# bblinn2017/inverse_path_tracer

Hardware: AMD Instinct MI355X
Metric: Msamples/sec fwd + grad-Msamples/sec, 512² Cornell 64spp, 1/2/4/8 GPU (higher is better)
Workload: dtype f32; 1 GPU; C2: CornellBox-Empty-CO.obj, 512x512, 64 spp, max_bounces=4; one frame per step tiled over the ranks as interleaved rows (fwd); adjoint dL/dKd of the rank's rows + RCCL all-reduce of the gradient (grad, --full); 3 frames in flight (consecutive steps round-robin over 3 HIP streams; one stream: secondary.serial); streams=3, width=512, height=512, spp=64, max_bounces=4, triangles=18, parallelism=interleaved row tiles x1

## Files before the change

include/ipt.h:

```cpp
#ifndef IPT_H
#define IPT_H
#include <stdint.h>

#ifdef __cplusplus
extern "C" {
#endif


int loadScene(float **poss, float **oris, float **scls, char **obj_fs, char **mtl_fs, int n,
              void **scenePtr);

void freeScene(void *scenePtr);

void createImage(void *scenePtr, char *img_file);

void createGraph(void *scenePtr, char *imgFile, float *data);

void getMaterials(void *scenePtr, float *materials);
void setMaterials(void *scenePtr, float *materials);


typedef struct ipt_params {
  int32_t width, height, spp, max_bounces;
  uint64_t seed;
  int32_t row_begin, row_end;
  int32_t row_step;
} ipt_params_t;

const char *ipt_last_error(void);
void ipt_clear_error(void);
int ipt_abi_version(void);
int ipt_device_count(void);
int ipt_selftest_math(uint64_t n, uint64_t seed, uint64_t *counts);
void ipt_debug_fail_launches(int n);
void ipt_debug_adju_ring(int pool_chunks, int lds_slots);

void ipt_legacy_config(int width, int height, int spp, int max_bounces, int64_t seed);

int ipt_load_scene(int n, const float *pos, const float *ori, const float *scl, const char **obj_files,
                   const char **mtl_files, void **scenePtr);
int ipt_load_scene_host(int n, const float *pos, const float *ori, const float *scl, const char **obj_files,
                        const char **mtl_files, void **scenePtr);
int ipt_scene_num_triangles(void *scene);
int ipt_scene_num_emissives(void *scene);
int ipt_scene_export_triangles(void *scene, float *out);
int ipt_scene_get_materials(void *scene, float *kd);
int ipt_scene_set_materials(void *scene, const float *kd);
int ipt_scene_camera(void *scene, float *out16);

#define IPT_ACCEL_AUTO 0
#define IPT_ACCEL_BRUTE 1
#define IPT_ACCEL_BVH 2
int ipt_scene_set_accel(void *scene, int mode);
int ipt_scene_bvh_info(void *scene, int32_t *info8);
int ipt_scene_export_bvh(void *scene, float *nodes, float *pairs, int32_t *big_idx);
int ipt_scene_export_wide(void *scene, float *wide);
int ipt_scene_shadow_masks(void *scene, uint32_t *masks);
int ipt_closest_hit_host(void *scene, int64_t n, const float *origins, const float *dirs, const int32_t *targets,
                         float *t, int32_t *idx);
int ipt_closest_hit_dev(void *scene, int64_t n, const float *origins_dev, const float *dirs_dev,
                        const int32_t *targets_dev, float *t_dev, int32_t *idx_dev, void *stream);
int ipt_shadow_hit_host(void *scene, int64_t n, const float *origins, const float *dirs, const int32_t *targets,
                        const int32_t *sources, float *t, int32_t *idx);

int ipt_render_samples_host(void *scene, const ipt_params_t *p, float *samples);
int ipt_render_host(void *scene, const ipt_params_t *p, float *hdr, uint8_t *ldr);
int ipt_adjoint_host(void *scene, const ipt_params_t *p, const float *adj , double *grad );
int ipt_graph_host(void *scene, const ipt_params_t *p, const uint8_t *target ,
                   double *acc , float *data );
int ipt_compress(int nT, const double *acc, float *data);

int ipt_render_dev(void *scene, const ipt_params_t *p, const float *kd_dev, float *hdr_dev, uint8_t *ldr_dev,
                   void *stream);
int ipt_render_samples_dev(void *scene, const ipt_params_t *p, const float *kd_dev, float *samples_dev,
                           void *stream);
int ipt_pixel_mean_dev(const float *samples_dev, int64_t npix, int spp, float *hdr_dev, uint8_t *ldr_dev,
                       void *stream);
int ipt_render_samples_sm_dev(void *scene, const ipt_params_t *p, const float *kd_dev, float *samples_dev,
                              void *stream);
int ipt_pixel_mean_sm_dev(const float *samples_dev, int64_t npix, int spp, float *hdr_dev, uint8_t *ldr_dev,
                          void *stream);
int ipt_adjoint_dev(void *scene, const ipt_params_t *p, const float *kd_dev, const float *adj_dev, double *grad_dev,
                    void *stream);
int ipt_graph_dev(void *scene, const ipt_params_t *p, const uint8_t *target_dev, double *acc_dev, void *stream);

int ipt_render_batch_dev(void *scene, const ipt_params_t *p, int n_scenes, uint64_t seed_stride, const float *kd_dev,
                         float *hdr_dev, void *stream);
int ipt_adjoint_batch_dev(void *scene, const ipt_params_t *p, int n_scenes, uint64_t seed_stride, const float *kd_dev,
                          const float *adj_dev, double *grad_dev, void *stream);

int ipt_scene_get_material_params(void *scene, float *kd, float *ks, float *ke, float *ns);
int ipt_scene_set_material_params(void *scene, const float *kd, const float *ks, const float *ke);
int ipt_render_mat_dev(void *scene, const ipt_params_t *p, const float *kd_dev, const float *ks_dev,
                       const float *ke_dev, float *hdr_dev, uint8_t *ldr_dev, void *stream);
int ipt_adjoint_mat_dev(void *scene, const ipt_params_t *p, const float *kd_dev, const float *ks_dev,
                        const float *ke_dev, const float *adj_dev, double *grad_dev, void *stream);
int ipt_adjoint_mat_host(void *scene, const ipt_params_t *p, const float *adj , double *grad );
int ipt_adjoint_mat_unbounded_dev(void *scene, const ipt_params_t *p, const float *kd_dev, const float *ks_dev,
                                  const float *ke_dev, const float *adj_dev, double *grad_dev, void *stream);
int ipt_adjoint_mat_unbounded_host(void *scene, const ipt_params_t *p, const float *adj ,
                                   double *grad );
int ipt_render_mat_batch_dev(void *scene, const ipt_params_t *p, int n_scenes, uint64_t seed_stride,
                             const float *kd_dev, const float *ks_dev, const float *ke_dev, float *hdr_dev,
                             void *stream);
int ipt_adjoint_mat_batch_dev(void *scene, const ipt_params_t *p, int n_scenes, uint64_t seed_stride,
                              const float *kd_dev, const float *ks_dev, const float *ke_dev, const float *adj_dev,
                              double *grad_dev, void *stream);

int ipt_camera_look_at(const float eye[3], const float look[3], const float up[3], float fov_deg, float aspect,
                       float *out16);
int ipt_scene_camera_bound(void *scene, float *bound);
int ipt_views_create(void *scene, int n_views, const float *cams , void **views);
void ipt_views_free(void *views);
int ipt_views_count(void *views);
int ipt_render_views_dev(void *scene, void *views, const ipt_params_t *p, uint64_t seed_stride, const float *kd_dev,
                         const float *ks_dev, const float *ke_dev, float *hdr_dev, void *stream);
int ipt_adjoint_views_dev(void *scene, void *views, const ipt_params_t *p, uint64_t seed_stride, const float *kd_dev,
                          const float *ks_dev, const float *ke_dev, const float *adj_dev, double *grad_dev,
                          void *stream);
int ipt_render_views_batch_dev(void *scene, void *views, const ipt_params_t *p, int n_sets, uint64_t seed_stride,
                               const float *kd_dev, const float *ks_dev, const float *ke_dev,
                               float *hdr_dev , void *stream);
int ipt_adjoint_views_batch_dev(void *scene, void *views, const ipt_params_t *p, int n_sets, uint64_t seed_stride,
                                const float *kd_dev, const float *ks_dev, const float *ke_dev,
                                const float *adj_dev ,
                                double *grad_dev , void *stream);
int ipt_render_views_batch_unbounded_dev(void *scene, void *views, const ipt_params_t *p, int n_sets,
                                         uint64_t seed_stride, const float *kd_dev, const float *ks_dev,
                                         const float *ke_dev,
                                         float *hdr_dev , void *stream);
int ipt_adjoint_views_batch_unbounded_dev(void *scene, void *views, const ipt_params_t *p, int n_sets,
                                          uint64_t seed_stride, const float *kd_dev, const float *ks_dev,
                                          const float *ke_dev,
                                          const float *adj_dev ,
                                          double *grad_dev ,
                                          void *stream);
int ipt_render_views_host(void *scene, void *views, const ipt_params_t *p, uint64_t seed_stride,
                          float *hdr );
int ipt_adjoint_views_host(void *scene, void *views, const ipt_params_t *p, uint64_t seed_stride,
                           const float *adj , double *grad );
int ipt_views_rays_host(void *scene, void *views, int view, const ipt_params_t *p, int64_t n,
                        const int64_t *sample_index, float *org , float *dir );

int ipt_png_write(const char *path, int width, int height, const uint8_t *rgb);
int ipt_png_read(const char *path, int *width, int *height, uint8_t *rgb, int64_t capacity);

#ifdef __cplusplus
}
#endif
#endif
```

inverse_path_tracer_amd/_native.py:

```python
from __future__ import annotations

import ctypes as C
import os

_HERE = os.path.dirname(os.path.abspath(__file__))
LIB_PATH = os.environ.get("IPT_AMD_LIB") or os.path.join(_HERE, "lib", "libipt_amd.so")
HEADER_PATH = os.path.join(os.path.dirname(_HERE), "include", "ipt.h")
TRI_EXPORT_STRIDE = 57
ACC_WIDTH = 8
ABI_VERSION = 5
ACCEL_AUTO, ACCEL_BRUTE, ACCEL_BVH = 0, 1, 2


class NativeError(RuntimeError):
    """A C-ABI call failed; the message is ipt_last_error()."""


class Params(C.Structure):

    _fields_ = [
        ("width", C.c_int32),
        ("height", C.c_int32),
        ("spp", C.c_int32),
        ("max_bounces", C.c_int32),
        ("seed", C.c_uint64),
        ("row_begin", C.c_int32),
        ("row_end", C.c_int32),
        ("row_step", C.c_int32),
    ]

    @property
    def rows(self) -> int:
        n = self.row_end - self.row_begin
        return max(0, -(-n // max(1, self.row_step)))


def make_params(width, height, spp, max_bounces=None, seed=0, row_begin=0, row_end=None, row_step=1) -> Params:
    return Params(int(width), int(height), int(spp), -1 if max_bounces is None else int(max_bounces),
                  int(seed) & 0xFFFFFFFFFFFFFFFF, int(row_begin), int(height if row_end is None else row_end),
                  int(row_step))


_lib = None

vp = C.c_void_p
fp = C.POINTER(C.c_float)
dp = C.POINTER(C.c_double)
u8p = C.POINTER(C.c_uint8)
pp = C.POINTER(Params)

SIGNATURES = {
    "loadScene": (C.c_int, [C.POINTER(fp), C.POINTER(fp), C.POINTER(fp), C.POINTER(C.c_char_p),
                            C.POINTER(C.c_char_p), C.c_int, C.POINTER(vp)]),
    "freeScene": (None, [vp]),
    "createImage": (None, [vp, C.c_char_p]),
    "createGraph": (None, [vp, C.c_char_p, fp]),
    "getMaterials": (None, [vp, fp]),
    "setMaterials": (None, [vp, fp]),
    "ipt_last_error": (C.c_char_p, []),
    "ipt_clear_error": (None, []),
    "ipt_abi_version": (C.c_int, []),
    "ipt_device_count": (C.c_int, []),
    "ipt_selftest_math": (C.c_int, [C.c_uint64, C.c_uint64, C.POINTER(C.c_uint64)]),
    "ipt_debug_fail_launches": (None, [C.c_int]),
    "ipt_debug_adju_ring": (None, [C.c_int, C.c_int]),
    "ipt_legacy_config": (None, [C.c_int, C.c_int, C.c_int, C.c_int, C.c_int64]),
    "ipt_load_scene": (C.c_int, [C.c_int, fp, fp, fp, C.POINTER(C.c_char_p), C.POINTER(C.c_char_p), C.POINTER(vp)]),
    "ipt_load_scene_host": (C.c_int, [C.c_int, fp, fp, fp, C.POINTER(C.c_char_p), C.POINTER(C.c_char_p),
                                      C.POINTER(vp)]),
    "ipt_scene_num_triangles": (C.c_int, [vp]),
    "ipt_scene_num_emissives": (C.c_int, [vp]),
    "ipt_scene_export_triangles": (C.c_int, [vp, fp]),
    "ipt_scene_camera": (C.c_int, [vp, fp]),
    "ipt_scene_get_materials": (C.c_int, [vp, fp]),
    "ipt_scene_set_materials": (C.c_int, [vp, fp]),
    "ipt_render_samples_host": (C.c_int, [vp, pp, fp]),
    "ipt_render_host": (C.c_int, [vp, pp, fp, u8p]),
    "ipt_adjoint_host": (C.c_int, [vp, pp, fp, dp]),
    "ipt_graph_host": (C.c_int, [vp, pp, u8p, dp, fp]),
    "ipt_compress": (C.c_int, [C.c_int, dp, fp]),
    "ipt_render_dev": (C.c_int, [vp, pp, vp, vp, vp, vp]),
    "ipt_render_samples_dev": (C.c_int, [vp, pp, vp, vp, vp]),
    "ipt_pixel_mean_dev": (C.c_int, [vp, C.c_int64, C.c_int, vp, vp, vp]),
    "ipt_render_samples_sm_dev": (C.c_int, [vp, pp, vp, vp, vp]),
    "ipt_pixel_mean_sm_dev": (C.c_int, [vp, C.c_int64, C.c_int, vp, vp, vp]),
    "ipt_adjoint_dev": (C.c_int, [vp, pp, vp, vp, vp, vp]),
    "ipt_graph_dev": (C.c_int, [vp, pp, vp, vp, vp]),
    "ipt_render_batch_dev": (C.c_int, [vp, pp, C.c_int, C.c_uint64, vp, vp, vp]),
    "ipt_adjoint_batch_dev": (C.c_int, [vp, pp, C.c_int, C.c_uint64, vp, vp, vp, vp]),
    "ipt_scene_get_material_params": (C.c_int, [vp, fp, fp, fp, fp]),
    "ipt_scene_set_material_params": (C.c_int, [vp, fp, fp, fp]),
    "ipt_render_mat_dev": (C.c_int, [vp, pp, vp, vp, vp, vp, vp, vp]),
    "ipt_adjoint_mat_dev": (C.c_int, [vp, pp, vp, vp, vp, vp, vp, vp]),
    "ipt_adjoint_mat_host": (C.c_int, [vp, pp, fp, dp]),
    "ipt_adjoint_mat_unbounded_dev": (C.c_int, [vp, pp, vp, vp, vp, vp, vp, vp]),
    "ipt_adjoint_mat_unbounded_host": (C.c_int, [vp, pp, fp, dp]),
    "ipt_render_mat_batch_dev": (C.c_int, [vp, pp, C.c_int, C.c_uint64, vp, vp, vp, vp, vp]),
    "ipt_adjoint_mat_batch_dev": (C.c_int, [vp, pp, C.c_int, C.c_uint64, vp, vp, vp, vp, vp, vp]),
    "ipt_camera_look_at": (C.c_int, [fp, fp, fp, C.c_float, C.c_float, fp]),
    "ipt_scene_camera_bound": (C.c_int, [vp, fp]),
    "ipt_views_create": (C.c_int, [vp, C.c_int, fp, C.POINTER(vp)]),
    "ipt_views_free": (None, [vp]),
    "ipt_views_count": (C.c_int, [vp]),
    "ipt_render_views_dev": (C.c_int, [vp, vp, pp, C.c_uint64, vp, vp, vp, vp, vp]),
    "ipt_adjoint_views_dev": (C.c_int, [vp, vp, pp, C.c_uint64, vp, vp, vp, vp, vp, vp]),
    "ipt_render_views_batch_dev": (C.c_int, [vp, vp, pp, C.c_int, C.c_uint64, vp, vp, vp, vp, vp]),
    "ipt_adjoint_views_batch_dev": (C.c_int, [vp, vp, pp, C.c_int, C.c_uint64, vp, vp, vp, vp, vp, vp]),
    "ipt_render_views_batch_unbounded_dev": (C.c_int, [vp, vp, pp, C.c_int, C.c_uint64, vp, vp, vp, vp, vp]),
    "ipt_adjoint_views_batch_unbounded_dev": (C.c_int, [vp, vp, pp, C.c_int, C.c_uint64, vp, vp, vp, vp, vp, vp]),
    "ipt_render_views_host":(C.c_int, [vp, vp, pp, C.c_uint64, fp]),
    "ipt_adjoint_views_host": (C.c_int, [vp, vp, pp, C.c_uint64, fp, dp]),
    "ipt_views_rays_host": (C.c_int, [vp, vp, C.c_int, pp, C.c_int64, C.POINTER(C.c_int64), fp, fp]),
    "ipt_scene_set_accel": (C.c_int, [vp, C.c_int]),
    "ipt_scene_bvh_info": (C.c_int, [vp, C.POINTER(C.c_int32)]),
    "ipt_scene_export_bvh": (C.c_int, [vp, fp, fp, C.POINTER(C.c_int32)]),
    "ipt_scene_export_wide": (C.c_int, [vp, fp]),
    "ipt_closest_hit_host": (C.c_int, [vp, C.c_int64, fp, fp, C.POINTER(C.c_int32), fp, C.POINTER(C.c_int32)]),
    "ipt_closest_hit_dev": (C.c_int, [vp, C.c_int64, vp, vp, vp, vp, vp, vp]),
    "ipt_scene_shadow_masks": (C.c_int, [vp, C.POINTER(C.c_uint32)]),
    "ipt_shadow_hit_host": (C.c_int, [vp, C.c_int64, fp, fp, C.POINTER(C.c_int32), C.POINTER(C.c_int32), fp,
                                      C.POINTER(C.c_int32)]),
    "ipt_png_write": (C.c_int, [C.c_char_p, C.c_int, C.c_int, u8p]),
    "ipt_png_read": (C.c_int, [C.c_char_p, C.POINTER(C.c_int), C.POINTER(C.c_int), u8p, C.c_int64]),
}


def lib():
    global _lib
    if _lib is None:
        if not os.path.exists(LIB_PATH):
            raise NativeError(
                "native library %s is missing: build it with `make -C inverse_path_tracer_amd/csrc` "
                "(there is no CPU fallback)" % LIB_PATH)
        L = C.CDLL(LIB_PATH)
        for name, (res, args) in SIGNATURES.items():
            f = getattr(L, name)
            f.restype = res
            f.argtypes = args
        v = L.ipt_abi_version()
        if v != ABI_VERSION:
            raise NativeError("%s has ABI %d, this binding needs %d: rebuild it" % (LIB_PATH, v, ABI_VERSION))
        _lib = L
    return _lib


def last_error() -> str:
    return (lib().ipt_last_error() or b"").decode(errors="replace")


def check(rc, what="native call"):
    if rc is not None and rc < 0:
        raise NativeError("%s failed: %s" % (what, last_error()))
    return rc


def device_count() -> int:
    return lib().ipt_device_count()
```

inverse_path_tracer_amd/csrc/capi.cpp:

```cpp
#include <cmath>
#include <cstdlib>
#include <algorithm>
#include <cstring>
#include <ctime>
#include <mutex>
#include <set>
#include <string>
#include <vector>

#include "../../include/ipt.h"
#include "gpu_api.h"
#include "png_io.h"
#include "scene_io.h"
#include "bvh.h"

using ipt::GpuScene;

namespace {

thread_local std::string g_err;

void fail(const std::string &e) { g_err = e; }

struct LegacyConfig {
  int width = 500, height = 500, spp = 100, max_bounces = -1;
  int64_t seed = -1;
} g_legacy;

ipt::RenderParams to_params(const ipt_params_t *p) {
  ipt::RenderParams r;
  r.width = p->width;
  r.height = p->height;
  r.spp = p->spp;
  r.max_bounces = p->max_bounces;
  r.seed = p->seed;
  r.row_begin = p->row_begin;
  r.row_end = p->row_end;
  r.row_step = p->row_step;
  return r;
}

ipt::RenderParams legacy_params() {
  ipt::RenderParams r;
  r.width = g_legacy.width;
  r.height = g_legacy.height;
  r.spp = g_legacy.spp;
  r.max_bounces = g_legacy.max_bounces;
  r.seed = g_legacy.seed >= 0 ? (uint64_t)g_legacy.seed : (uint64_t)time(nullptr);
  r.row_begin = 0;
  r.row_end = r.height;
  return r;
}

int gpu_status(int rc) {
  if (rc) fail(ipt::gpu_last_error());
  return rc;
}

GpuScene *as_scene(void *p) {
  if (!p) fail("null scene handle");
  return static_cast<GpuScene *>(p);
}

void compress(int nT, const double *acc, float *data) {
  const size_t sz = (size_t)(nT + 1) * nT;
  float *wts = data, *pix = data + sz, *lig = data + 4 * sz;
  std::vector<float> ws((size_t)nT);
  for (int dst = 0; dst <= nT; ++dst) {
    float total = 0.f;
    for (int src = 0; src < nT; ++src) {
      const double *e = acc + ((size_t)dst * nT + src) * 8;
      const float w = logf((float)e[0] + 1);
      ws[(size_t)src] = w;
      total += w;
      const float fs = (float)e[1];
      const float den = (fs != 0.f) ? fs : 1.f;
      for (int i = 0; i < 3; ++i) {
        pix[((size_t)dst * nT + src) * 3 + i] = (float)e[2 + i] / den;
        lig[((size_t)dst * nT + src) * 3 + i] = (float)e[5 + i] / den;
      }
    }
    for (int src = 0; src < nT; ++src)
      wts[(size_t)dst * nT + src] = (total != 0.f) ? ws[(size_t)src] / total : 0.f;
  }
}

}

extern "C" {

const char *ipt_last_error(void) { return g_err.c_str(); }
void ipt_clear_error(void) { g_err.clear(); }
int ipt_abi_version(void) { return 5; }
int ipt_device_count(void) { return ipt::gpu_device_count(); }
int ipt_selftest_math(uint64_t n, uint64_t seed, uint64_t *counts) {
  if (!counts) return -1;
  return gpu_status(ipt::gpu_selftest_math(n, seed, counts));
}
void ipt_debug_fail_launches(int n) { ipt::gpu_debug_fail_launches(n); }
void ipt_debug_adju_ring(int pool_chunks, int lds_slots) { ipt::gpu_debug_adju_ring(pool_chunks, lds_slots); }

void ipt_legacy_config(int width, int height, int spp, int max_bounces, int64_t seed) {
  g_legacy.width = width;
  g_legacy.height = height;
  g_legacy.spp = spp;
  g_legacy.max_bounces = max_bounces;
  g_legacy.seed = seed;
}

static int load_scene_impl(int n, const float *pos, const float *ori, const float *scl, const char **obj_files,
                           const char **mtl_files, void **scenePtr, bool device) {
  if (scenePtr) *scenePtr = nullptr;
  if (n < 0 || !scenePtr || (n > 0 && (!pos || !ori || !scl || !obj_files || !mtl_files))) {
    fail("ipt_load_scene: bad arguments");
    return -1;
  }
  std::vector<ipt::ObjectRecord> recs((size_t)n);
  for (int i = 0; i < n; ++i) {
    for (int k = 0; k < 3; ++k) {
      recs[(size_t)i].pos[k] = pos[3 * i + k];
      recs[(size_t)i].ori[k] = ori[3 * i + k];
      recs[(size_t)i].scl[k] = scl[3 * i + k];
    }
    if (!obj_files[i] || !mtl_files[i]) {
      fail("ipt_load_scene: null file name");
      return -1;
    }
    recs[(size_t)i].obj_file = obj_files[i];
    recs[(size_t)i].mtl_file = mtl_files[i];
  }
  ipt::HostScene host;
  std::string err;
  if (!ipt::build_scene(recs, &host, &err)) {
    fail(err);
    return -1;
  }
  GpuScene *s = device ? ipt::gpu_upload(host, &err) : ipt::gpu_host_only(host);
  if (!s) {
    fail(err);
    return -1;
  }
  *scenePtr = s;
  return host.nT;
}

int ipt_load_scene(int n, const float *pos, const float *ori, const float *scl, const char **obj_files,
                   const char **mtl_files, void **scenePtr) {
  return load_scene_impl(n, pos, ori, scl, obj_files, mtl_files, scenePtr, true);
}
int ipt_load_scene_host(int n, const float *pos, const float *ori, const float *scl, const char **obj_files,
                        const char **mtl_files, void **scenePtr) {
  return load_scene_impl(n, pos, ori, scl, obj_files, mtl_files, scenePtr, false);
}

int loadScene(float **poss, float **oris, float **scls, char **obj_fs, char **mtl_fs, int n, void **scenePtr) {
  if (n < 0 || !poss || !oris || !scls) {
    if (scenePtr) *scenePtr = nullptr;
    fail("loadScene: bad arguments");
    return -1;
  }
  std::vector<float> pos((size_t)n * 3), ori((size_t)n * 3), scl((size_t)n * 3);
  for (int i = 0; i < n; ++i)
    for (int k = 0; k < 3; ++k) {
      pos[(size_t)(3 * i + k)] = poss[i][k];
      ori[(size_t)(3 * i + k)] = oris[i][k];
      scl[(size_t)(3 * i + k)] = scls[i][k];
    }
  return ipt_load_scene(n, pos.data(), ori.data(), scl.data(), const_cast<const char **>(obj_fs),
                        const_cast<const char **>(mtl_fs), scenePtr);
}

void freeScene(void *scenePtr) { ipt::gpu_free(static_cast<GpuScene *>(scenePtr)); }

int ipt_scene_num_triangles(void *scene) {
  GpuScene *s = as_scene(scene);
  return s ? ipt::gpu_host(s).nT : -1;
}
int ipt_scene_num_emissives(void *scene) {
  GpuScene *s = as_scene(scene);
  return s ? ipt::gpu_host(s).nE : -1;
}
int ipt_scene_export_triangles(void *scene, float *out) {
  GpuScene *s = as_scene(scene);
  if (!s || !out) return -1;
  ipt::export_triangles(ipt::gpu_host(s), out);
  return 0;
}
int ipt_scene_camera(void *scene, float *out16) {
  GpuScene *s = as_scene(scene);
  if (!s || !out16) return -1;
  std::memcpy(out16, ipt::gpu_host(s).cam, 16 * sizeof(float));
  return 0;
}

int ipt_scene_bvh_info(void *scene, int32_t *info8) {
  GpuScene *s = as_scene(scene);
  if (!s || !info8) return -1;
  const ipt::HostScene &h = ipt::gpu_host(s);
  info8[0] = (int32_t)h.bvh_nodes.size();
  info8[1] = (int32_t)h.bvh_pairs.size();
  info8[2] = h.bvh_depth;
  info8[3] = ipt::gpu_accel_in_use(s);
  info8[4] = (int32_t)h.bvh_big_pairs.size();
  info8[5] = (int32_t)h.bvh_wide.size();
  info8[6] = h.bvh_wdepth;
  info8[7] = (int32_t)h.bvh_wtris.size();
  if (h.bvh_nodes.empty()) fail("no BVH: " + h.bvh_status);
  return h.bvh_nodes.empty() ? 0 : 1;
}
int ipt_scene_export_bvh(void *scene, float *nodes, float *pairs, int32_t *big_idx) {
  GpuScene *s = as_scene(scene);
  if (!s) return -1;
  const ipt::HostScene &h = ipt::gpu_host(s);
  if (big_idx && !h.bvh_big_idx.empty())
    std::memcpy(big_idx, h.bvh_big_idx.data(), h.bvh_big_idx.size() * sizeof(int32_t));
  if (nodes && !h.bvh_nodes.empty()) std::memcpy(nodes, h.bvh_nodes.data(), h.bvh_nodes.size() * sizeof(ipt::BvhNode));
  if (pairs && !h.bvh_pairs.empty()) std::memcpy(pairs, h.bvh_pairs.data(), h.bvh_pairs.size() * sizeof(ipt::BvhPair));
  return 0;
}
int ipt_scene_export_wide(void *scene, float *wide) {
  GpuScene *s = as_scene(scene);
  if (!s) return -1;
  const ipt::HostScene &h = ipt::gpu_host(s);
  if (wide && !h.bvh_wide.empty()) std::memcpy(wide, h.bvh_wide.data(), h.bvh_wide.size() * sizeof(ipt::WideNode));
  return 0;
}
int ipt_scene_shadow_masks(void *scene, uint32_t *masks) {
  GpuScene *s = as_scene(scene);
  if (!s || !masks) return -1;
  const std::vector<uint32_t> m = ipt::shadow_occluder_masks(ipt::gpu_host(s));
  std::memcpy(masks, m.data(), m.size() * sizeof(uint32_t));
  return 0;
}
int ipt_scene_set_accel(void *scene, int mode) {
  GpuScene *s = as_scene(scene);
  if (!s) return -1;
  return gpu_status(ipt::gpu_set_accel(s, mode));
}
static bool probe_ids_ok(GpuScene *s, int64_t n, const int32_t *targets, const int32_t *sources, const char *who) {
  const ipt::HostScene &h = ipt::gpu_host(s);
  for (int64_t i = 0; i < n; ++i) {
    if (targets && targets[i] >= 0 &&
        std::find(h.emit_tri.begin(), h.emit_tri.end(), targets[i]) == h.emit_tri.end()) {
      fail(std::string(who) + ": target " + std::to_string(targets[i]) + " is not an emitter triangle");
      return false;
    }
    if (sources && (sources[i] < -1 || sources[i] >= h.nT)) {
      fail(std::string(who) + ": source " + std::to_string(sources[i]) + " outside [-1, nT)");
      return false;
    }
  }
  return true;
// ... 521 lines not shown
```

inverse_path_tracer_amd/csrc/gpu_api.h:

```cpp
#pragma once
#include <stdint.h>

#include <string>

#include "../../include/ipt.h"
#include "scene_io.h"

namespace ipt {

struct GpuScene;

GpuScene *gpu_upload(const HostScene &host, std::string *err);
GpuScene *gpu_host_only(const HostScene &host);
bool gpu_on_device(const GpuScene *s);
void gpu_free(GpuScene *s);
const HostScene &gpu_host(const GpuScene *s);
HostScene &gpu_host_mut(GpuScene *s);
int gpu_set_kd(GpuScene *s, const float *kd_host);

int gpu_render_samples(GpuScene *s, const RenderParams &p, const float *kd_dev, float *samples_dev,
                       void *stream);
int gpu_pixel_mean(const float *samples_dev, int64_t npix, int spp, float *hdr_dev, uint8_t *ldr_dev,
                   void *stream);
int gpu_render_samples_sm(GpuScene *s, const RenderParams &p, const float *kd_dev, float *samples_dev,
                          void *stream);
int gpu_pixel_mean_sm(const float *samples_dev, int64_t npix, int spp, float *hdr_dev, uint8_t *ldr_dev,
                      void *stream);
int gpu_render(GpuScene *s, const RenderParams &p, const float *kd_dev, float *hdr_dev, uint8_t *ldr_dev,
               void *stream);
int gpu_adjoint(GpuScene *s, const RenderParams &p, const float *kd_dev, const float *adj_dev,
                double *grad_dev, void *stream);
int gpu_graph(GpuScene *s, const RenderParams &p, const uint8_t *target_dev, double *acc_dev, void *stream);

int gpu_set_material_params(GpuScene *s, const float *kd, const float *ks, const float *ke);
int gpu_render_mat(GpuScene *s, const RenderParams &p, const float *kd_dev, const float *ks_dev, const float *ke_dev,
                   float *hdr_dev, uint8_t *ldr_dev, void *stream);
int gpu_adjoint_mat(GpuScene *s, const RenderParams &p, const float *kd_dev, const float *ks_dev, const float *ke_dev,
                    const float *adj_dev, double *grad_dev, void *stream);
int gpu_adjoint_mat_host(GpuScene *s, const RenderParams &p, const float *adj, double *grad);
int gpu_adjoint_mat_unbounded(GpuScene *s, const RenderParams &p, const float *kd_dev, const float *ks_dev,
                              const float *ke_dev, const float *adj_dev, double *grad_dev, void *stream);
int gpu_adjoint_mat_unbounded_host(GpuScene *s, const RenderParams &p, const float *adj, double *grad);
int gpu_render_mat_batch(GpuScene *s, const RenderParams &p, const float *kd_dev, const float *ks_dev,
                         const float *ke_dev, float *hdr_dev, void *stream);
int gpu_adjoint_mat_batch(GpuScene *s, const RenderParams &p, const float *kd_dev, const float *ks_dev,
                          const float *ke_dev, const float *adj_dev, double *grad_dev, void *stream);

struct GpuViews;
GpuViews *gpu_views_create(GpuScene *s, int n, const float *cams);
void gpu_views_free(GpuViews *v);
int gpu_views_count(const GpuViews *v);
float gpu_camera_bound(const GpuScene *s);
int gpu_render_views(GpuScene *s, const GpuViews *v, RenderParams p, const float *kd_dev, const float *ks_dev,
                     const float *ke_dev, float *hdr_dev, void *stream);
int gpu_adjoint_views(GpuScene *s, const GpuViews *v, RenderParams p, const float *kd_dev, const float *ks_dev,
                      const float *ke_dev, const float *adj_dev, double *grad_dev, void *stream);
int gpu_render_views_batch(GpuScene *s, const GpuViews *v, RenderParams p, int n_sets, const float *kd_dev,
                           const float *ks_dev, const float *ke_dev, float *hdr_dev, void *stream);
int gpu_adjoint_views_batch(GpuScene *s, const GpuViews *v, RenderParams p, int n_sets, const float *kd_dev,
                            const float *ks_dev, const float *ke_dev, const float *adj_dev, double *grad_dev,
                            void *stream);
int gpu_render_views_batch_unbounded(GpuScene *s, const GpuViews *v, RenderParams p, int n_sets, const float *kd_dev,
                                     const float *ks_dev, const float *ke_dev, float *hdr_dev, void *stream);
int gpu_adjoint_views_batch_unbounded(GpuScene *s, const GpuViews *v, RenderParams p, int n_sets, const float *kd_dev,
                                      const float *ks_dev, const float *ke_dev, const float *adj_dev,
                                      double *grad_dev, void *stream);
int gpu_render_views_host(GpuScene *s, const GpuViews *v, const RenderParams &p, float *hdr);
int gpu_adjoint_views_host(GpuScene *s, const GpuViews *v, const RenderParams &p, const float *adj, double *grad);
int gpu_views_rays_host(GpuScene *s, const GpuViews *v, int view, RenderParams p, int64_t n, const int64_t *index,
                        float *org, float *dir);

int gpu_render_samples_host(GpuScene *s, const RenderParams &p, float *samples);
int gpu_render_host(GpuScene *s, const RenderParams &p, float *hdr, uint8_t *ldr);
int gpu_adjoint_host(GpuScene *s, const RenderParams &p, const float *adj, double *grad);
int gpu_graph_host(GpuScene *s, const RenderParams &p, const uint8_t *target, double *acc);

int gpu_set_accel(GpuScene *s, int mode);
int gpu_accel_in_use(const GpuScene *s);
int gpu_closest_hit(GpuScene *s, int64_t n, const float *org_dev, const float *dir_dev, const int *targets_dev,
                    const int *sources_dev, float *t_dev, int *idx_dev, void *stream);
int gpu_closest_hit_host(GpuScene *s, int64_t n, const float *org, const float *dir, const int *targets,
                         const int *sources, float *t, int *idx);

int gpu_device_count();
int gpu_selftest_math(uint64_t n, uint64_t seed, uint64_t *counts);
void gpu_debug_fail_launches(int n);
void gpu_debug_adju_ring(int pool_chunks, int lds_slots);
const char *gpu_last_error();
void gpu_set_error(const std::string &e);

}
```

inverse_path_tracer_amd/csrc/ipt_device.h:

```cpp
#pragma once
#include <hip/hip_runtime.h>
#include <stdint.h>

#include "scene_layout.h"

namespace ipt {
namespace dev {

typedef __attribute__((address_space(3))) float lds_f32;
typedef __attribute__((address_space(3))) double lds_f64;
typedef __attribute__((address_space(1))) float gbl_f32;
typedef __attribute__((address_space(1))) double gbl_f64;
typedef float v4f __attribute__((ext_vector_type(4)));
typedef __attribute__((address_space(3))) v4f lds_v4;
typedef __attribute__((address_space(1))) v4f gbl_v4;

constexpr float kMinDotUp = 0x1.a36e30p-14f;
constexpr float kEpsUp = 0x1.47ae16p-7f;
constexpr float kPRR = 0.9f;
constexpr float kPiF = 3.14159265358979323846f;
constexpr float kInvPiF = (float)(1.0 / 3.14159265358979323846);
constexpr double kPi = 3.14159265358979323846;

#ifndef IPT_DIV_CONST
// ... 924 lines not shown
  const float s2 = fmaf(qz, T.e2[2], fmaf(qy, T.e2[1], fmaf(qx, T.e2[0], T.e2[3])));
  const bool ok = !(fabsf(denom) < kMinDotUp) && t >= kEpsUp && !(s0 > 0.f) && !(s1 > 0.f) && !(s2 > 0.f);
  return ok ? t : __builtin_inff();
}

template <bool SHADOW>
__device__ __forceinline__ void coop_traverse(const CoopView &C, V3 gp, V3 gd, float &gt, int &gi) {
  const int lane = (int)__lane_id();
  const int g = lane >> 3, j = lane & 7;
  const int target = gi;
  const SlabRay r = slab_ray(gp, gd);
  const int oct = (gd.x < 0.f ? 1 : 0) | (gd.y < 0.f ? 2 : 0) | (gd.z < 0.f ? 4 : 0);
  uint32_t *stk = C.stk + g * C.stride;
  int node = 0, sp = 0;
#ifdef IPT_BVH_STATS
  uint32_t st_nodes = 0, st_leaves = 0;
#endif
  for (;;) {
    if (node >= 0) {
#ifdef IPT_BVH_STATS
      ++st_nodes;
#endif
      float4 a, b;
      uint32_t rw;
      if (C.wn_lds) {
        const lds_f32 *pw = (const lds_f32 *)C.wn + 4 * (2 * (8 * node + oct) + 1) + 3;
        const lds_v4 *q = (const lds_v4 *)C.wn + 2 * (8 * node + j);
        rw = __float_as_uint(*pw);
        const v4f qa = q[0], qb = q[1];
        a = make_float4(qa.x, qa.y, qa.z, qa.w);
        b = make_float4(qb.x, qb.y, qb.z, qb.w);
      } else {
        const gbl_f32 *pw = (const gbl_f32 *)C.wn + 4 * (2 * (8 * node + oct) + 1) + 3;
        const gbl_v4 *q = (const gbl_v4 *)C.wn + 2 * (8 * node + j);
        rw = __float_as_uint(*pw);
        const v4f qa = q[0], qb = q[1];
        a = make_float4(qa.x, qa.y, qa.z, qa.w);
        b = make_float4(qb.x, qb.y, qb.z, qb.w);
      }
      const uint32_t rj = (rw >> (3 * j)) & 7u;
      const int ref = __float_as_int(b.z);
      const float tx0 = fmaf(a.x, r.ix.x, r.ox.x), tx1 = fmaf(a.w, r.ix.x, r.ox.x);
      const float ty0 = fmaf(a.y, r.iy.x, r.oy.x), ty1 = fmaf(b.x, r.iy.x, r.oy.x);
      const float tz0 = fmaf(a.z, r.iz.x, r.oz.x), tz1 = fmaf(b.y, r.iz.x, r.oz.x);
      const float en = fmaxf(fmaxf(fminf(tx0, tx1), fminf(ty0, ty1)), fmaxf(fminf(tz0, tz1), 0.f));
      const float ex = fminf(fminf(fmaxf(tx0, tx1), fmaxf(ty0, ty1)), fminf(fmaxf(tz0, tz1), gt));
      const bool h = en <= ex && ref != kWideEmpty;
      const uint32_t hm = group_or_u32(h ? 1u << rj : 0u);
      if (hm == 0) {
        node = sp > 0 ? (int)stk[--sp] : kBvhDone;
      } else {
        const uint32_t f = (uint32_t)__builtin_ctz(hm);
        const int nx = group_min_i32(h && rj == f ? ref : 0x7fffffff);
        const uint32_t others = hm & (hm - 1u);
        if ((others >> rj) & 1u) stk[sp + __popc(others >> (rj + 1))] = (uint32_t)ref;
        sp += __popc(others);
        node = nx;
      }
    } else {
#ifdef IPT_BVH_STATS
      ++st_leaves;
#endif
      const int code = ~node;
      const int first = code >> 4, cnt = (code & 15) + 1;
#ifdef IPT_BVH_STATS
      if (j == 0) atomicAdd(&g_bvh_stats[4], (unsigned long long)cnt);
#endif
      for (int base = 0; base < cnt; base += 8) {
        float tj = __builtin_inff();
        int ij = 0x7fffffff;
        if (base + j < cnt) {
          const TriIsect &T = C.wt[first + base + j];
          tj = tri_accept_t(T, gp, gd);
          ij = __float_as_int(T.pad[0]);
        }
        group_lexmin(tj, ij);
        const bool take = (tj < gt) | ((tj == gt) & (ij < gi));
        gt = take ? tj : gt;
        gi = take ? ij : gi;
      }
      node = (SHADOW && gi != target) ? kBvhDone : (sp > 0 ? (int)stk[--sp] : kBvhDone);
    }
    if (node == kBvhDone) break;
  }
#ifdef IPT_BVH_STATS
  if (j == 0) {
    atomicAdd(&g_bvh_stats[0], 1ull);
    atomicAdd(&g_bvh_stats[1], (unsigned long long)st_nodes);
    atomicAdd(&g_bvh_stats[2], (unsigned long long)st_leaves);
    if (SHADOW && gi != target) atomicAdd(&g_bvh_stats[3], 1ull);
  }
#endif
}

template <bool SHADOW>
__device__ __forceinline__ void coop_cast(const CoopView &C, bool need, V3 p, V3 d, float &bt, int &bi) {
  const int lane = (int)__lane_id();
  const int g = lane >> 3;
  uint64_t M = __ballot(need);
#ifdef IPT_BVH_STATS
  if (M && lane == (int)__builtin_ctzll(__ballot(1))) atomicAdd(&g_bvh_stats[5], 1ull);
#endif
  while (M) {
#ifdef IPT_BVH_STATS
    if (lane == (int)__builtin_ctzll(__ballot(1))) atomicAdd(&g_bvh_stats[6], 1ull);
#endif
    uint64_t Mr = M;
    int src = -1;
#pragma unroll
    for (int k = 0; k < 8; ++k) {
      if (Mr) {
        const int idx = __builtin_ctzll(Mr);
        Mr &= Mr - 1;
        src = (g == k) ? idx : src;
      }
    }
    const uint64_t taken = M & ~Mr;
    M = Mr;
    const int sa = (src < 0 ? lane : src) << 2;
    const V3 gp = mk(bperm_f(sa, p.x), bperm_f(sa, p.y), bperm_f(sa, p.z));
    const V3 gd = mk(bperm_f(sa, d.x), bperm_f(sa, d.y), bperm_f(sa, d.z));
    float gt = bperm_f(sa, bt);
    int gi = __builtin_amdgcn_ds_bpermute(sa, bi);
    if (src >= 0) {
      coop_traverse<SHADOW>(C, gp, gd, gt, gi);
    }
    const int ra = (8 * lane_rank64(taken)) << 2;
    const float rt = bperm_f(ra, gt);
    const int ri = __builtin_amdgcn_ds_bpermute(ra, gi);
    if ((taken >> lane) & 1ull) {
      bt = rt;
      bi = ri;
    }
  }
}

__device__ __forceinline__ V3 shading_normal(const TriGeom &g, V3 q) {
  if (g.flags & GEOM_AXIS_FLAT) return mk(g.vn[0][0], g.vn[0][1], g.vn[0][2]);
  const V3 v0 = mk(g.v[0][0], g.v[0][1], g.v[0][2]);
  const V3 v1 = mk(g.v[1][0], g.v[1][1], g.v[1][2]);
  const V3 v2 = mk(g.v[2][0], g.v[2][1], g.v[2][2]);
  const V3 c0 = cross3(sub(v1, q), sub(v2, q));
  const V3 c1 = cross3(sub(v2, q), sub(v0, q));
  const V3 c2 = cross3(sub(v0, q), sub(v1, q));
  const float w0 = (0.5f * sqrtf(dot3(c0, c0))) / g.area;
  const float w1 = (0.5f * sqrtf(dot3(c1, c1))) / g.area;
  const float w2 = (0.5f * sqrtf(dot3(c2, c2))) / g.area;
  const V3 n = mk(fmaf(g.vn[2][0], w2, fmaf(g.vn[1][0], w1, g.vn[0][0] * w0)),
                  fmaf(g.vn[2][1], w2, fmaf(g.vn[1][1], w1, g.vn[0][1] * w0)),
                  fmaf(g.vn[2][2], w2, fmaf(g.vn[1][2], w1, g.vn[0][2] * w0)));
  return unit(n);
}

__device__ __forceinline__ V3 camera_local(float u0, float u1, float cf, float rf, int W, int H, float rcW, float rcH) {
  const float nx = 2.f * (cf + u0), ny = 2.f * (rf + u1);
  const float x = (rcW != 0.f ? nx * rcW : div_inrange(nx, (float)W)) - 1.f;
  const float y = 1.f - (rcH != 0.f ? ny * rcH : div_inrange(ny, (float)H));
  return unit_in_range(mk(x, y, 1.f));
}
__device__ __forceinline__ V3 rotate3(const float *R0, const float *R1, const float *R2, V3 h) {
  return mk(fmaf(R0[2], h.z, fmaf(R0[1], h.y, R0[0] * h.x)), fmaf(R1[2], h.z, fmaf(R1[1], h.y, R1[0] * h.x)),
            fmaf(R2[2], h.z, fmaf(R2[1], h.y, R2[0] * h.x)));
}
__device__ __forceinline__ V3 camera_w0(const float *cam, V3 v) {
  return mk(fmaf(cam[3], 0.f, v.x), fmaf(cam[7], 0.f, v.y), fmaf(cam[11], 0.f, v.z));
}
__device__ __forceinline__ void camera_ray_f(const float *cam, const float *org, Rng &st, float rf, float cf, int W, int H,
                                             float rcW, float rcH, V3 &p, V3 &d) {
  const float u0 = uniform(st), u1 = uniform(st);
  const V3 d0 = camera_local(u0, u1, cf, rf, W, H, rcW, rcH);
  p = mk(org[0], org[1], org[2]);
  d = unit(camera_w0(cam, rotate3(cam, cam + 4, cam + 8, d0)));
}
__device__ __forceinline__ void camera_ray(const float *cam, const float *org, Rng &st, int r, int c, int W, int H,
                                           float rcW, float rcH, V3 &p, V3 &d) {
  camera_ray_f(cam, org, st, (float)r, (float)c, W, H, rcW, rcH, p, d);
}

__device__ inline float phong(float shin, V3 nrm, V3 w, V3 wi) {
  const float dn = dot3(nrm, wi);
  const V3 refl = mk(fmaf(2.f * dn, nrm.x, -wi.x), fmaf(2.f * dn, nrm.y, -wi.y), fmaf(2.f * dn, nrm.z, -wi.z));
  const float pw = pow_f(dot3(refl, w), shin);
  const float mx = pw > 0.f ? pw : 0.f;
  return (float)((((double)(shin + 2.f)) / 2.0 / kPi) * (double)mx);
}

}
}
```

inverse_path_tracer_amd/csrc/ipt_hip.hip:

```cpp
#include <hip/hip_runtime.h>

#include <algorithm>
#include <atomic>
#include <cmath>
#include <cstdio>
#include <cstdlib>
#include <cstring>
#include <mutex>
#include <string>
#include <type_traits>
#include <vector>

#include "bvh.h"
#include "gpu_api.h"
#include "ipt_device.h"

namespace ipt {

static thread_local std::string g_gpu_err;
void gpu_set_error(const std::string &e) { g_gpu_err = e; }
const char *gpu_last_error() { return g_gpu_err.c_str(); }
static std::atomic<int> g_fail_launches{0};
void gpu_debug_fail_launches(int n) { g_fail_launches.store(n > 0 ? n : 0); }
static std::atomic<int> g_adju_pool{0}, g_adju_lds{0};
void gpu_debug_adju_ring(int pool_chunks, int lds_slots) {
  g_adju_pool.store(pool_chunks > 0 ? std::min(pool_chunks, 63) : 0);
  g_adju_lds.store(lds_slots > 0 ? lds_slots : 0);
}

#define HIP_TRY(expr)                                                                        \
  do {                                                                                       \
    hipError_t e_ = (expr);                                                                  \
    if (e_ != hipSuccess) {                                                                  \
      gpu_set_error(std::string(#expr) + ": " + hipGetErrorString(e_));                      \
      return -1;                                                                             \
    }                                                                                        \
  } while (0)

enum { MODE_FWD = 0, MODE_ADJ = 1, MODE_GRAPH = 2, MODE_ADJU = 3, MODE_FWDM = 4, MODE_ADJW = 5 };
template <int MODE>
constexpr bool is_badj() {
  return MODE == MODE_ADJ || MODE == MODE_ADJW;
}
template <int MODE>
constexpr bool is_adj() {
  return is_badj<MODE>() || MODE == MODE_ADJU;
}
template <int MODE>
constexpr bool is_fwd() {
  return MODE == MODE_FWD || MODE == MODE_FWDM;
}
constexpr int kBlock = 256;
constexpr int kRecSD = 3;
constexpr int kRecFieldsDiffuse = 3;
constexpr int kRecFieldsSpec = kRecFieldsDiffuse + 2;
constexpr int kMaxAdjTris = 65535;
constexpr int kEdgeW = 8;
constexpr int kEdgeL = 5;
__host__ __device__ inline size_t graph_lds_doubles(int nT, int nE) {
  return (size_t)(nT + 1) * nT * kEdgeL + (size_t)(nT + 1) * (nE > 0 ? nE : 0) * 3;
}
__host__ __device__ inline size_t mat_lds_doubles(int grad_slots, int nE, bool spec) {
  return (size_t)grad_slots * 3 * (spec ? 2 : 1) + (size_t)(nE > 0 ? nE : 0) * 3;
}
constexpr int kCarryWords = 9;
__host__ __device__ inline size_t mat_carry_bytes(bool bvh) {
  return bvh ? 0 : (size_t)kCarryWords * kBlock * sizeof(uint32_t);
}
constexpr int kMaxAdjBounces = 62;
#ifndef IPT_CHAIN_DPP
#define IPT_CHAIN_DPP 1
#endif
#ifndef IPT_ADJU_SHIFTED_CHAIN
#define IPT_ADJU_SHIFTED_CHAIN 0
#endif
#ifndef IPT_ADJU_RING
#define IPT_ADJU_RING 63
#endif
constexpr int kPoolSlots = 16, kPoolMaxChunks = 4;
#ifndef IPT_ADJU_POOL_MB
#define IPT_ADJU_POOL_MB 64
#endif
#ifndef IPT_ADJU_LDS_CAP
#define IPT_ADJU_LDS_CAP (31 * 1024)
#endif
#ifndef IPT_ADJU_LDS_SLOTS
#define IPT_ADJU_LDS_SLOTS 8
#endif
#ifndef IPT_ADJU_LDS_SLOTS_BVH
#define IPT_ADJU_LDS_SLOTS_BVH 6
#endif
#ifndef IPT_ADJU_LDS_SLOTS_FIXED
#define IPT_ADJU_LDS_SLOTS_FIXED -1
#endif
constexpr int kAdjuRing = IPT_ADJU_RING;
#ifndef IPT_ADJU_SUB
#define IPT_ADJU_SUB 0
#endif
constexpr int kSub = IPT_ADJU_SUB;
constexpr int kMrEnt = kSub > 0 ? (kAdjuRing + kSub - 1) / kSub : 1;
#ifndef IPT_DYN_CHUNKS
#define IPT_DYN_CHUNKS 1
#endif
#ifndef IPT_DYN_CHUNKS_PER_WAVE
#define IPT_DYN_CHUNKS_PER_WAVE 32
#endif
#ifndef IPT_DYN_MIN_CHUNK
#define IPT_DYN_MIN_CHUNK 128
#endif
constexpr int kMaxTableTris = 512;
#ifndef IPT_LDS_GRAD_KB
#define IPT_LDS_GRAD_KB 12
#endif
constexpr int kLdsGradBytes = IPT_LDS_GRAD_KB * 1024;
#ifndef IPT_BVH_MIN_TRIS
#define IPT_BVH_MIN_TRIS 64
#endif
constexpr int kBvhMinTris = IPT_BVH_MIN_TRIS;
#ifndef IPT_BVH_LDS_KB
#define IPT_BVH_LDS_KB 32
#endif
constexpr int kBvhLdsNodeBytes = IPT_BVH_LDS_KB * 1024;

struct TraceArgs {
  int W, H, spp, max_bounces;
  uint64_t seed;
  uint64_t n_samples;
  int nT, nE;
  int lds_edges;
  int sample_major;
  int kd_tables;
  const float *kdpi_g;
  int small_pairs;
  uint64_t npix;
  int row0, row_step;
  int idx32;
  uint64_t m_spp, m_W, m_npix;
  int bvh_nbig;
  const float4 *bvh_wide;
  const TriIsect *bvh_wtris;
  int bvh_wide_lds, coop_stride;
  int bvh_big_lds;
  float root_box[6];
  float tree_sphere[4];
  const float4 *src_cull;
  const TriPair *bvh_big;
  const int32_t *bvh_big_idx;
  const PairBox2 *bvh_big_boxes;
  int grad_slots;
  const int *grad_map;
  const int *slot_tri;
  float cam[16];
  float cam_org[3];
  const double *emit_pmfr;
  float rc_spp;
  float rc_W, rc_H;
  int rec_cap;
  int rec_lds;
  float *grec;
  uint64_t grec_stride;
  int pool_chunks;
  float *mring;
  int nscenes, bps;
  uint64_t seed_stride, out_stride, adj_stride;
  uint32_t chunk;
  uint32_t chunk_small, chunk_big_n;
  uint32_t mat_stride;
  uint32_t *chunk_ctr;
  uint32_t grabs;
  const PairBox2 *pboxes;
  const uint32_t *pomask;
  const uint32_t *big_pomask;
  int fused;
  uint32_t group;
  uint32_t mean_off, mean_wstride;
  int nslots;
  uint8_t *ldr;
};
static_assert(alignof(TraceArgs) == 8, "TraceArgs sits right after the ten 8-B scene pointers in the kernarg segment");
static_assert(offsetof(TraceArgs, chunk_ctr) == offsetof(TraceArgs, mat_stride) + sizeof(uint32_t), "mat_stride fills the padding");

__device__ __forceinline__ uint32_t udiv32(uint32_t n, uint64_t m, uint32_t d) {
  return d == 1u ? n : (uint32_t)__umul64hi(m, (uint64_t)n);
}

__device__ __forceinline__ void item_split(const TraceArgs &a, uint64_t w, uint64_t &lp, uint64_t &sj) {
  if (a.idx32) {
    if (a.sample_major) {
      const uint32_t q = udiv32((uint32_t)w, a.m_npix, (uint32_t)a.npix);
      sj = q;
      lp = (uint32_t)w - q * (uint32_t)a.npix;
    } else {
      const uint32_t q = udiv32((uint32_t)w, a.m_spp, (uint32_t)a.spp);
      lp = q;
      sj = (uint32_t)w - q * (uint32_t)a.spp;
    }
  } else if (a.sample_major) {
    sj = w / a.npix;
    lp = w - sj * a.npix;
  } else {
    lp = w / (uint64_t)a.spp;
    sj = w - lp * (uint64_t)a.spp;
  }
}
__device__ __forceinline__ void local_rc(const TraceArgs &a, uint64_t lp, int &r, int &c) {
  uint64_t lr;
  if (a.idx32) {
    const uint32_t q = udiv32((uint32_t)lp, a.m_W, (uint32_t)a.W);
    lr = q;
    c = (int)((uint32_t)lp - q * (uint32_t)a.W);
  } else {
    lr = lp / (uint64_t)a.W;
    c = (int)(lp - lr * (uint64_t)a.W);
  }
  r = a.row0 + (int)lr * a.row_step;
}

#ifndef IPT_BF_BIG
#define IPT_BF_BIG 2
#endif
#ifndef IPT_BF_TAIL
#define IPT_BF_TAIL 4
#endif
#ifndef IPT_CTR_STRIDE
#define IPT_CTR_STRIDE 32
#endif
constexpr int kCtrStride = IPT_CTR_STRIDE;
constexpr int kViewFloats = 20;
template <bool BVH>
constexpr bool kGuided() {
  return BVH || IPT_BF_BIG > 1;
}
template <bool GUIDED>
__device__ __forceinline__ void chunk_range(const TraceArgs &a, uint64_t g, uint64_t units, uint64_t &start,
                                            uint64_t &end) {
  const uint64_t nb = a.chunk_big_n;
  uint64_t len;
  if (!GUIDED || g < nb) {
    start = g * a.chunk;
    len = a.chunk;
  } else {
    start = nb * a.chunk + (g - nb) * a.chunk_small;
    len = a.chunk_small;
  }
  end = start + len < units ? start + len : units;
}

__device__ __forceinline__ void grab_failed(uint32_t *word, uint32_t c, uint32_t grabs) {
  if (c + 1u == grabs) __hip_atomic_store(word, 0u, __ATOMIC_RELAXED, __HIP_MEMORY_SCOPE_AGENT);
}

__device__ __forceinline__ uint64_t item_pixel(const TraceArgs &a, uint64_t w) {
  uint64_t lp, sj;
  item_split(a, w, lp, sj);
  int r, c;
  local_rc(a, lp, r, c);
  if (a.idx32) return (uint32_t)r * (uint32_t)a.W + (uint32_t)c;
  return (uint64_t)r * (uint64_t)a.W + (uint64_t)c;
}

using namespace dev;
typedef __attribute__((address_space(3))) uint32_t lds_u32;

__device__ __forceinline__ void item_ray_ls(const TraceArgs &a, uint64_t seed, uint64_t lp, uint64_t sj, Rng &st, V3 &p,
                                            V3 &d, int &r, int &c) {
  local_rc(a, lp, r, c);
  uint64_t g;
  if (a.idx32) {
    const uint32_t pixel = (uint32_t)r * (uint32_t)a.W + (uint32_t)c;
    g = (uint64_t)pixel * (uint32_t)a.spp + sj;
  } else {
    g = ((uint64_t)r * (uint64_t)a.W + (uint64_t)c) * (uint64_t)a.spp + sj;
  }
  rng_init(st, seed + g);
  camera_ray(a.cam, a.cam_org, st, r, c, a.W, a.H, a.rc_W, a.rc_H, p, d);
}
__device__ __forceinline__ void item_ray(const TraceArgs &a, uint64_t seed, uint64_t w, Rng &st, V3 &p, V3 &d, int &r,
                                         int &c) {
  uint64_t lp, sj;
  item_split(a, w, lp, sj);
  item_ray_ls(a, seed, lp, sj, st, p, d, r, c);
}

#ifndef IPT_INPHASE_REFILL
#define IPT_INPHASE_REFILL 1
#endif
#ifndef IPT_INPHASE_MERGE
#define IPT_INPHASE_MERGE 1
#endif
#ifndef IPT_INPHASE_PACK
#define IPT_INPHASE_PACK 0
#endif
template <int MODE, bool BVH>
constexpr bool kInphase() {
  return IPT_INPHASE_REFILL && MODE == MODE_FWDM && !BVH;
}
constexpr int kEntryWords = 4;
static inline uint32_t fused_entry_words(uint32_t group, bool bvh) {
  return (IPT_INPHASE_REFILL && !bvh) ? kEntryWords * group : 0u;
}
__device__ __forceinline__ void pixel_entry(const TraceArgs &a, uint64_t seed, uint64_t lp, uint32_t e[kEntryWords]) {
  int r, c;
  local_rc(a, lp, r, c);
  uint64_t g0;
  if (a.idx32) {
    const uint32_t pixel = (uint32_t)r * (uint32_t)a.W + (uint32_t)c;
    g0 = (uint64_t)pixel * (uint32_t)a.spp;
  } else {
    g0 = ((uint64_t)r * (uint64_t)a.W + (uint64_t)c) * (uint64_t)a.spp;
  }
  g0 += seed;
  e[0] = (uint32_t)g0;
  e[1] = (uint32_t)(g0 >> 32);
  e[2] = __float_as_uint((float)c);
  e[3] = __float_as_uint((float)r);
}
#ifndef IPT_REFILL_ABLATE
#define IPT_REFILL_ABLATE 0
#endif

#ifndef IPT_MIN_BLOCKS_FWD
#define IPT_MIN_BLOCKS_FWD 5
#endif
#ifndef IPT_MIN_BLOCKS_ADJ
#define IPT_MIN_BLOCKS_ADJ 5
#endif
#ifndef IPT_MIN_BLOCKS_ADJU
#define IPT_MIN_BLOCKS_ADJU 5
#endif
#ifndef IPT_MIN_BLOCKS_ADJW
#define IPT_MIN_BLOCKS_ADJW 6
#endif
#ifndef IPT_ADJW_LANE_LDS
#define IPT_ADJW_LANE_LDS 1
#endif
#ifndef IPT_MIN_BLOCKS_GRAPH
#define IPT_MIN_BLOCKS_GRAPH 0
#endif
#ifndef IPT_MIN_BLOCKS_BVH
#define IPT_MIN_BLOCKS_BVH 4
#endif
#ifndef IPT_MIN_BLOCKS_BVH_ADJ
#define IPT_MIN_BLOCKS_BVH_ADJ 2
#endif
#ifndef IPT_MIN_BLOCKS_BVH_ADJU
#define IPT_MIN_BLOCKS_BVH_ADJU 4
#endif
#ifndef IPT_MIN_BLOCKS_BVH_FWD
#define IPT_MIN_BLOCKS_BVH_FWD 5
#endif
template <int MODE, bool BVH>
constexpr int min_blocks() {
  return BVH ? (MODE == MODE_ADJU ? IPT_MIN_BLOCKS_BVH_ADJU
                                  : (is_adj<MODE>() ? IPT_MIN_BLOCKS_BVH_ADJ
                                                    : (is_fwd<MODE>() ? IPT_MIN_BLOCKS_BVH_FWD : IPT_MIN_BLOCKS_BVH)))
             : (is_fwd<MODE>() ? IPT_MIN_BLOCKS_FWD
                                : (MODE == MODE_ADJU   ? IPT_MIN_BLOCKS_ADJU
                                   : MODE == MODE_ADJW ? IPT_MIN_BLOCKS_ADJW
                                                       : (is_adj<MODE>() ? IPT_MIN_BLOCKS_ADJ : IPT_MIN_BLOCKS_GRAPH)));
}
#ifndef IPT_GRAPH_LDS_KB
#define IPT_GRAPH_LDS_KB 64
#endif
#ifndef IPT_ADJ_PIXEL_MAJOR
#define IPT_ADJ_PIXEL_MAJOR 1
#endif
#ifndef IPT_GRAPH_PIXEL_MAJOR
#define IPT_GRAPH_PIXEL_MAJOR 1
#endif
#define IPT_TRACE_BOUNDS __attribute__((amdgpu_flat_work_group_size(1, kBlock), amdgpu_waves_per_eu(min_blocks<MODE, BVH>() ? min_blocks<MODE, BVH>() : 1)))
#ifdef IPT_PHASE_TIMING
constexpr int kPhaseWords = 26;
__device__ unsigned long long g_phase_cycles[kPhaseWords];
#define PHASE_LANES(i, cond)                             \
  {                                                      \
    const uint64_t b_ = __ballot(cond);                  \
    if (b_) {                                            \
      tacc[i] += (uint64_t)__popcll(b_);                 \
      tacc[(i) + 1] += 1;                                \
    }                                                    \
  }
#define SUBPHASE_BEGIN const uint64_t ts_ = __builtin_amdgcn_s_memtime();
#define SUBPHASE_END(i) tacc[i] += __builtin_amdgcn_s_memtime() - ts_;
#define PHASE(i)                                     \
  {                                                  \
    const uint64_t tn_ = __builtin_amdgcn_s_memtime(); \
    tacc[i] += tn_ - tp_;                            \
    tp_ = tn_;                                       \
  }
#else
#define PHASE(i)
#define SUBPHASE_BEGIN
#define SUBPHASE_END(i)
#define PHASE_LANES(i, cond)
#endif

__device__ __forceinline__ int cast_bf(const TriPair *__restrict__ pairs, const f2 *e3, int nT, V3 p, V3 d, float &t) {
  if (e3) return closest_hit_pairs_small(pairs, e3, nT, p, d, t);
  return closest_hit_pairs(pairs, nT, p, d, t);
}

__device__ __forceinline__ float small_table_entry(const TriPair *__restrict__ pairs, int i) {
  const int j = i / kE3Floats, k = i % kE3Floats, h = k & 1;
  return pairs[j].f[9 + 4 * (k >> 1)][h];
}

__host__ __device__ inline size_t bvh_lds_offset(size_t base) { return (base + 15) & ~(size_t)15; }
constexpr int kEmitLdsMax = 16;
__host__ __device__ inline size_t emit_lds_bytes(int nE) {
  return nE > 0 && nE <= kEmitLdsMax ? (size_t)nE * sizeof(TriIsect) : 0;
}
__host__ __device__ inline size_t big_lds_bytes(int nbig) {
  return IPT_PATH_CULL && nbig > 0 ? 12 + (size_t)nbig * (sizeof(TriPair) + 2 * sizeof(int32_t)) : 0;
}
__device__ __forceinline__ float *big_lds_copy(const TraceArgs &a, float *at, float *base, int tid, int nthr,
                                               BvhView &bv) {
  if (!(IPT_PATH_CULL && a.bvh_nbig > 0 && a.bvh_big_lds)) return at;
  float *pl = at + ((4 - (int)((at - base) & 3)) & 3);
  const float *g = reinterpret_cast<const float *>(a.bvh_big);
  for (int i = tid; i < 36 * a.bvh_nbig; i += nthr) pl[i] = g[i];
  int32_t *il = reinterpret_cast<int32_t *>(pl + 36 * a.bvh_nbig);
  for (int i = tid; i < 2 * a.bvh_nbig; i += nthr) il[i] = a.bvh_big_idx[i];
  bv.big_lds = pl;
  return at + big_lds_bytes(a.bvh_nbig) / sizeof(float);
}

template <int CTRL, int ROW, int BANK>
__device__ __forceinline__ int dpp0(int v) {
  return __builtin_amdgcn_update_dpp(0, v, CTRL, ROW, BANK, true);
}
__device__ __forceinline__ int wave_scan_add(int v) {
  int s = v + dpp0<0x111, 0xf, 0xf>(v);
  s += dpp0<0x112, 0xf, 0xf>(v);
  s += dpp0<0x113, 0xf, 0xf>(v);
  s += dpp0<0x114, 0xf, 0xe>(s);
  s += dpp0<0x118, 0xf, 0xc>(s);
  s += dpp0<0x142, 0xa, 0xf>(s);
  s += dpp0<0x143, 0xc, 0xf>(s);
  return s;
}
__device__ __forceinline__ uint32_t wave_scan_max(uint32_t v) {
  v = max(v, (uint32_t)dpp0<0x111, 0xf, 0xf>((int)v));
  v = max(v, (uint32_t)dpp0<0x112, 0xf, 0xf>((int)v));
  v = max(v, (uint32_t)dpp0<0x114, 0xf, 0xf>((int)v));
  v = max(v, (uint32_t)dpp0<0x118, 0xf, 0xf>((int)v));
  v = max(v, (uint32_t)dpp0<0x142, 0xa, 0xf>((int)v));
  v = max(v, (uint32_t)dpp0<0x143, 0xc, 0xf>((int)v));
  return v;
}

struct TraceKernArgs {
  TraceArgs a;
  const TriIsect *isect;
  const TriPair *pairs;
  const TriGeom *geom;
  const TriMat *mat;
  const float *kd;
  const int *emit_tri;
  const float *emit_cdf;
  const float *emit_pmf;
  float *out_samples;
  const float *adj;
  double *grad;
  const uint8_t *target;
  double *edges;
};
static_assert(offsetof(TraceKernArgs, isect) == sizeof(TraceArgs), "pointers follow TraceArgs");
template <typename T>
__device__ __forceinline__ T karg(size_t off) {
#if defined(__HIP_DEVICE_COMPILE__)
  typedef __attribute__((address_space(4))) const char cst_char;
  typedef __attribute__((address_space(4))) const T cst_t;
  const cst_char *k = (const cst_char *)__builtin_amdgcn_kernarg_segment_ptr();
  asm volatile("" : "+s"(k));
  return *(const cst_t *)(k + off);
#else
  (void)off;
  return T();
#endif
}
template <int MODE, bool SPEC, bool BVH>
__global__ IPT_TRACE_BOUNDS void trace_kernel(
    const TraceArgs a, const TriIsect *__restrict__ isect, const TriPair *__restrict__ pairs,
    const TriGeom *__restrict__ geom, const TriMat *__restrict__ mat, const float *__restrict__ kd,
    const int *__restrict__ emit_tri, const float *__restrict__ emit_cdf, const float *__restrict__ emit_pmf,
    float *__restrict__ out_samples, const float *__restrict__ adj, double *__restrict__ grad,
    const uint8_t *__restrict__ target, double *__restrict__ edges) {
  constexpr bool MATG = false;
  constexpr bool MATB = false;
  constexpr bool VIEWS = false;
  constexpr bool VSETS = false;
  const int *const tri_emit = nullptr;
#include "trace_body.h"
}

template <int MODE, bool SPEC, bool BVH>
__global__ IPT_TRACE_BOUNDS void trace_fwd_mat_kernel(
    const TraceArgs a, const TriIsect *__restrict__ isect, const TriPair *__restrict__ pairs,
    const TriGeom *__restrict__ geom, const TriMat *__restrict__ mat, const float *__restrict__ kd,
    const int *__restrict__ emit_tri, const float *__restrict__ emit_cdf, const float *__restrict__ emit_pmf,
    float *__restrict__ out_samples, const float *__restrict__ adj, double *__restrict__ grad,
    const uint8_t *__restrict__ target, double *__restrict__ edges) {
  static_assert(is_fwd<MODE>(), "forward instances only");
  constexpr bool MATG = false;
  constexpr bool MATB = true;
  constexpr bool VIEWS = false;
  constexpr bool VSETS = false;
  const int *const tri_emit = nullptr;
#include "trace_body.h"
}

template <bool SPEC, bool BVH>
__global__ __attribute__((amdgpu_flat_work_group_size(1, kBlock),
                          amdgpu_waves_per_eu(min_blocks<MODE_ADJ, BVH>()))) void
trace_mat_kernel(const TraceArgs a, const TriIsect *__restrict__ isect, const TriPair *__restrict__ pairs,
                 const TriGeom *__restrict__ geom, const TriMat *__restrict__ mat, const float *__restrict__ kd,
                 const int *__restrict__ emit_tri, const float *__restrict__ emit_cdf,
                 const float *__restrict__ emit_pmf, float *__restrict__ out_samples, const float *__restrict__ adj,
                 double *__restrict__ grad, const uint8_t *__restrict__ target, double *__restrict__ edges,
                 const int *__restrict__ tri_emit) {
  constexpr int MODE = MODE_ADJ;
  constexpr bool MATG = true;
  constexpr bool MATB = false;
  constexpr bool VIEWS = false;
  constexpr bool VSETS = false;
#include "trace_body.h"
}

template <bool SPEC, bool BVH>
__global__ __attribute__((amdgpu_flat_work_group_size(1, kBlock),
                          amdgpu_waves_per_eu(min_blocks<MODE_ADJU, BVH>()))) void
trace_matu_kernel(const TraceArgs a, const TriIsect *__restrict__ isect, const TriPair *__restrict__ pairs,
                  const TriGeom *__restrict__ geom, const TriMat *__restrict__ mat, const float *__restrict__ kd,
                  const int *__restrict__ emit_tri, const float *__restrict__ emit_cdf,
                  const float *__restrict__ emit_pmf, float *__restrict__ out_samples, const float *__restrict__ adj,
                  double *__restrict__ grad, const uint8_t *__restrict__ target, double *__restrict__ edges,
                  const int *__restrict__ tri_emit) {
  constexpr int MODE = MODE_ADJU;
  constexpr bool MATG = true;
  constexpr bool MATB = false;
  constexpr bool VIEWS = false;
  constexpr bool VSETS = false;
#include "trace_body.h"
}

template <int MODE, bool SPEC, bool BVH>
__global__ IPT_TRACE_BOUNDS void trace_fwd_views_kernel(
    const TraceArgs a, const TriIsect *__restrict__ isect, const TriPair *__restrict__ pairs,
    const TriGeom *__restrict__ geom, const TriMat *__restrict__ mat, const float *__restrict__ kd,
    const int *__restrict__ emit_tri, const float *__restrict__ emit_cdf, const float *__restrict__ emit_pmf,
    float *__restrict__ out_samples, const float *__restrict__ adj, double *__restrict__ grad,
    const uint8_t *__restrict__ target, double *__restrict__ edges, const float *__restrict__ views) {
  static_assert(is_fwd<MODE>(), "forward instances only");
  constexpr bool MATG = false;
  constexpr bool MATB = false;
  constexpr bool VIEWS = true;
  constexpr bool VSETS = false;
  const int *const tri_emit = nullptr;
#include "trace_body.h"
}
template <bool SPEC, bool BVH>
__global__ __attribute__((amdgpu_flat_work_group_size(1, kBlock),
                          amdgpu_waves_per_eu(min_blocks<MODE_ADJ, BVH>()))) void
trace_mat_views_kernel(const TraceArgs a, const TriIsect *__restrict__ isect, const TriPair *__restrict__ pairs,
                       const TriGeom *__restrict__ geom, const TriMat *__restrict__ mat,
                       const float *__restrict__ kd, const int *__restrict__ emit_tri,
                       const float *__restrict__ emit_cdf, const float *__restrict__ emit_pmf,
                       float *__restrict__ out_samples, const float *__restrict__ adj, double *__restrict__ grad,
                       const uint8_t *__restrict__ target, double *__restrict__ edges,
                       const int *__restrict__ tri_emit, const float *__restrict__ views) {
  constexpr int MODE = MODE_ADJ;
  constexpr bool MATG = true;
  constexpr bool MATB = false;
  constexpr bool VIEWS = true;
  constexpr bool VSETS = false;
#include "trace_body.h"
}

template <int MODE, bool SPEC, bool BVH>
__global__ IPT_TRACE_BOUNDS void trace_fwd_views_batch_kernel(
    const TraceArgs a, const TriIsect *__restrict__ isect, const TriPair *__restrict__ pairs,
    const TriGeom *__restrict__ geom, const TriMat *__restrict__ mat, const float *__restrict__ kd,
    const int *__restrict__ emit_tri, const float *__restrict__ emit_cdf, const float *__restrict__ emit_pmf,
    float *__restrict__ out_samples, const float *__restrict__ adj, double *__restrict__ grad,
    const uint8_t *__restrict__ target, double *__restrict__ edges, const float *__restrict__ views,
    const int nviews) {
  static_assert(is_fwd<MODE>(), "forward instances only");
  constexpr bool MATG = false;
  constexpr bool MATB = false;
  constexpr bool VIEWS = true;
  constexpr bool VSETS = true;
  const int *const tri_emit = nullptr;
#include "trace_body.h"
}
template <bool SPEC, bool BVH>
__global__ __attribute__((amdgpu_flat_work_group_size(1, kBlock),
                          amdgpu_waves_per_eu(min_blocks<MODE_ADJ, BVH>()))) void
trace_mat_views_batch_kernel(const TraceArgs a, const TriIsect *__restrict__ isect, const TriPair *__restrict__ pairs,
                             const TriGeom *__restrict__ geom, const TriMat *__restrict__ mat,
                             const float *__restrict__ kd, const int *__restrict__ emit_tri,
                             const float *__restrict__ emit_cdf, const float *__restrict__ emit_pmf,
                             float *__restrict__ out_samples, const float *__restrict__ adj,
                             double *__restrict__ grad, const uint8_t *__restrict__ target,
                             double *__restrict__ edges, const int *__restrict__ tri_emit,
                             const float *__restrict__ views, const int nviews) {
  constexpr int MODE = MODE_ADJ;
  constexpr bool MATG = true;
  constexpr bool MATB = false;
  constexpr bool VIEWS = true;
  constexpr bool VSETS = true;
#include "trace_body.h"
}

template <bool SPEC, bool BVH>
__global__ __attribute__((amdgpu_flat_work_group_size(1, kBlock),
                          amdgpu_waves_per_eu(min_blocks<MODE_ADJU, BVH>()))) void
trace_matu_views_batch_kernel(const TraceArgs a, const TriIsect *__restrict__ isect, const TriPair *__restrict__ pairs,
                              const TriGeom *__restrict__ geom, const TriMat *__restrict__ mat,
                              const float *__restrict__ kd, const int *__restrict__ emit_tri,
                              const float *__restrict__ emit_cdf, const float *__restrict__ emit_pmf,
                              float *__restrict__ out_samples, const float *__restrict__ adj,
                              double *__restrict__ grad, const uint8_t *__restrict__ target,
                              double *__restrict__ edges, const int *__restrict__ tri_emit,
                              const float *__restrict__ views, const int nviews) {
  constexpr int MODE = MODE_ADJU;
  constexpr bool MATG = true;
  constexpr bool MATB = false;
  constexpr bool VIEWS = true;
  constexpr bool VSETS = true;
#include "trace_body.h"
}

__global__ __launch_bounds__(kBlock) void view_rays_kernel(const float *__restrict__ views, int view, int W, int H,
                                                           int spp, float rcW, float rcH, uint64_t seed, int64_t n,
                                                           const int64_t *__restrict__ index,
                                                           float *__restrict__ org, float *__restrict__ dir) {
  const int64_t i = (int64_t)blockIdx.x * kBlock + threadIdx.x;
  if (i >= n) return;
  const uint64_t g = (uint64_t)index[i], pixel = g / (uint64_t)spp;
  const float *cam = views + (size_t)view * kViewFloats;
  Rng st;
  rng_init(st, seed + g);
  V3 p, d;
  camera_ray(cam, cam + 16, st, (int)(pixel / (uint64_t)W), (int)(pixel % (uint64_t)W), W, H, rcW, rcH, p, d);
  org[3 * i] = p.x, org[3 * i + 1] = p.y, org[3 * i + 2] = p.z;
  dir[3 * i] = d.x, dir[3 * i + 1] = d.y, dir[3 * i + 2] = d.z;
}

__global__ __launch_bounds__(kBlock) void pack_mat_kernel(const TriMat *__restrict__ src, const float *__restrict__ ks,
                                                          const float *__restrict__ ke,
                                                          const int *__restrict__ tri_emit, int nT,
                                                          TriMat *__restrict__ out) {
  const int i = blockIdx.x * kBlock + threadIdx.x;
  if (i >= nT) return;
  const size_t row = (size_t)blockIdx.y * (size_t)nT + (size_t)i;
  TriMat m = src[i];
  if (ks) {
    const bool lobe = (m.flags & MAT_HAS_KS) != 0;
    for (int c = 0; c < 3; ++c) m.ks[c] = lobe ? ks[3 * row + c] : 0.f;
  }
  if (ke) {
    const bool em = tri_emit[i] >= 0;
    for (int c = 0; c < 3; ++c) m.ke[c] = em ? ke[3 * row + c] : 0.f;
  }
  out[row] = m;
}

__global__ __launch_bounds__(kBlock) void replicate_kernel(const float *__restrict__ src, int n, size_t total,
                                                           float *__restrict__ out) {
  const size_t i = (size_t)blockIdx.x * kBlock + threadIdx.x;
  if (i < total) out[i] = src[i % (size_t)n];
}

__global__ __launch_bounds__(kBlock) void pixel_mean_sm_kernel(const float *__restrict__ samples, int64_t npix,
                                                               int spp, float *__restrict__ hdr,
                                                               uint8_t *__restrict__ ldr) {
  const int64_t px = (int64_t)blockIdx.x * kBlock + threadIdx.x;
  if (px >= npix) return;
  samples += (size_t)blockIdx.y * (size_t)npix * spp * 3;
  hdr += (size_t)blockIdx.y * (size_t)npix * 3;
  if (ldr) ldr += (size_t)blockIdx.y * (size_t)npix * 3;
  float tx = 0.f, ty = 0.f, tz = 0.f;
  const float fs = (float)spp;
  if ((spp & (spp - 1)) == 0 && spp <= (1 << 24)) {
    const float rc = 1.0f / fs;
    int i = 0;
    for (; i + 16 <= spp; i += 16) {
      float v[48];
#pragma unroll
      for (int u = 0; u < 16; ++u) {
        const float *s = samples + ((int64_t)(i + u) * npix + px) * 3;
        v[3 * u] = s[0];
        v[3 * u + 1] = s[1];
        v[3 * u + 2] = s[2];
      }
#pragma unroll
      for (int u = 0; u < 16; ++u) {
        tx += v[3 * u] * rc;
        ty += v[3 * u + 1] * rc;
        tz += v[3 * u + 2] * rc;
      }
    }
    for (; i < spp; ++i) {
      const float *s = samples + ((int64_t)i * npix + px) * 3;
      tx += s[0] * rc;
      ty += s[1] * rc;
      tz += s[2] * rc;
    }
  } else {
    for (int i = 0; i < spp; ++i) {
      const float *s = samples + ((int64_t)i * npix + px) * 3;
      tx += s[0] / fs;
      ty += s[1] / fs;
      tz += s[2] / fs;
    }
  }
  hdr[px * 3] = tx;
  hdr[px * 3 + 1] = ty;
  hdr[px * 3 + 2] = tz;
  if (ldr) {
    ldr[px * 3] = (uint8_t)(255.f * tx / (1 + tx));
    ldr[px * 3 + 1] = (uint8_t)(255.f * ty / (1 + ty));
    ldr[px * 3 + 2] = (uint8_t)(255.f * tz / (1 + tz));
  }
}

__global__ __launch_bounds__(kBlock) void pixel_mean_kernel(const float *__restrict__ samples, int64_t npix,
                                                            int spp, float *__restrict__ hdr,
                                                            uint8_t *__restrict__ ldr) {
  const int64_t px = (int64_t)blockIdx.x * kBlock + threadIdx.x;
  if (px >= npix) return;
  const float *s = samples + px * spp * 3;
  float tx = 0.f, ty = 0.f, tz = 0.f;
  const float fs = (float)spp;
  for (int i = 0; i < spp; ++i) {
    tx += s[3 * i] / fs;
    ty += s[3 * i + 1] / fs;
    tz += s[3 * i + 2] / fs;
  }
  hdr[px * 3] = tx;
  hdr[px * 3 + 1] = ty;
  hdr[px * 3 + 2] = tz;
  if (ldr) {
    ldr[px * 3] = (uint8_t)(255.f * tx / (1 + tx));
    ldr[px * 3 + 1] = (uint8_t)(255.f * ty / (1 + ty));
    ldr[px * 3 + 2] = (uint8_t)(255.f * tz / (1 + tz));
  }
}

static std::vector<double> pmf_reciprocals(const std::vector<float> &pmf) {
  std::vector<double> r(pmf.size(), 0.0);
  for (size_t e = 0; e < pmf.size(); ++e) {
    int ex = 0;
    const double m = std::frexp((double)pmf[e], &ex);
    if (pmf[e] > 0.f && m == 0.5 && ex > -1000) r[e] = std::ldexp(1.0, 1 - ex);
  }
  return r;
}

enum { KIND_TRACE = 0, KIND_MATG = 1, KIND_FWDB = 2, KIND_VFWD = 3, KIND_VMAT = 4, KIND_VBFWD = 5, KIND_VBMAT = 6 };
constexpr int kKindLast = KIND_VBMAT;
constexpr bool kind_views(int kind) { return kind == KIND_VFWD || kind == KIND_VMAT; }
constexpr bool kind_view_sets(int kind) { return kind == KIND_VBFWD || kind == KIND_VBMAT; }
constexpr bool inst_valid(int mode, int kind) {
  return kind == KIND_TRACE  ? mode >= MODE_FWD && mode <= MODE_ADJW
         : kind == KIND_MATG ? mode == MODE_ADJ || mode == MODE_ADJU
         : kind == KIND_VMAT ? mode == MODE_ADJ
         : kind == KIND_VBMAT ? mode == MODE_ADJ || mode == MODE_ADJU
                             : mode == MODE_FWD || mode == MODE_FWDM;
}
constexpr int inst_slot(int mode, bool spec, bool bvh, int kind) {
  return (kind == KIND_MATG   ? (mode == MODE_ADJU ? 36 : 24)
          : kind == KIND_FWDB ? 28 + (mode == MODE_FWDM ? 4 : 0)
          : kind == KIND_VFWD ? 40 + (mode == MODE_FWDM ? 4 : 0)
          : kind == KIND_VMAT ? 48
          : kind == KIND_VBFWD ? 52 + (mode == MODE_FWDM ? 4 : 0)
          : kind == KIND_VBMAT ? (mode == MODE_ADJU ? 64 : 60)
                              : mode * 4) +
         (spec ? 2 : 0) + (bvh ? 1 : 0);
}
constexpr int inst_slot_count() {
  bool seen[128] = {};
  int n = 0;
  for (int kind = KIND_TRACE; kind <= kKindLast; ++kind)
    for (int mode = MODE_FWD; mode <= MODE_ADJW; ++mode)
      for (int sb = 0; sb < 4 && inst_valid(mode, kind); ++sb) {
        const int slot = inst_slot(mode, (sb & 2) != 0, (sb & 1) != 0, kind);
        if (slot < 0 || slot >= 128 || seen[slot]) return -1;
        seen[slot] = true;
        n = slot + 1 > n ? slot + 1 : n;
      }
  return n;
}
constexpr int kInstSlots = inst_slot_count();
static_assert(kInstSlots > 0, "two instances share a slot of GpuScene::inst (inst_slot)");

struct InstCache {
  int grid = 0;
  size_t grid_lds = 0;
  size_t pick_base = 0;
  size_t pick_tail = 0;
  int pick_opt = -1;
};

struct GpuScene {
  HostScene host;
  int device = 0;
  bool on_device = false;
  TriIsect *isect = nullptr;
  TriPair *pairs = nullptr;
  TriGeom *geom = nullptr;
  TriMat *mat = nullptr;
  float *kd = nullptr;
  int *emit_tri = nullptr;
  float *emit_cdf = nullptr, *emit_pmf = nullptr;
  double *emit_pmfr = nullptr;
  bool has_ks = false;
  TriPair *big_pairs = nullptr;
  int32_t *big_idx = nullptr;
  PairBox2 *big_boxes = nullptr;
  float4 *wide = nullptr;
  float4 *src_cull = nullptr;
  TriIsect *wtris = nullptr;
  PairBox2 *pboxes = nullptr;
  uint32_t *pomask = nullptr;
  uint32_t *big_pomask = nullptr;
  int accel = IPT_ACCEL_AUTO;
  size_t adju_base = 0;
  int adju_nl = 0;
  size_t matu_base = 0;
  int matu_nl = 0;
  size_t vbmatu_base = 0;
  int vbmatu_nl = 0;
  int *grad_map = nullptr, *slot_tri = nullptr;
  int *tri_emit = nullptr;
  InstCache inst[kInstSlots];
  struct Counters {
    hipStream_t stream;
    int words;
    uint32_t *dev;
  };
  std::vector<Counters> counters;
  std::vector<uint32_t *> counters_retired;
  std::mutex counters_mu;
};

#ifdef IPT_PHASE_TIMING
extern "C" int ipt_debug_phase_cycles(unsigned long long *out) {
  if (hipMemcpyFromSymbol(out, HIP_SYMBOL(g_phase_cycles), kPhaseWords * sizeof(unsigned long long)) != hipSuccess)
    return -1;
  unsigned long long z[kPhaseWords] = {};
  return hipMemcpyToSymbol(HIP_SYMBOL(g_phase_cycles), z, sizeof z) == hipSuccess ? 0 : -1;
}
#endif

#ifdef IPT_BVH_STATS
extern "C" int ipt_debug_bvh_stats(unsigned long long *out) {
  if (hipMemcpyFromSymbol(out, HIP_SYMBOL(g_bvh_stats), kBvhStats * sizeof(unsigned long long)) != hipSuccess)
    return -1;
  unsigned long long z[kBvhStats] = {0};
  return hipMemcpyToSymbol(HIP_SYMBOL(g_bvh_stats), z, sizeof z) == hipSuccess ? 0 : -1;
}
#endif

const HostScene &gpu_host(const GpuScene *s) { return s->host; }
HostScene &gpu_host_mut(GpuScene *s) { return s->host; }

template <typename T>
static int upload(T **dst, const std::vector<T> &v) {
  const size_t n = std::max<size_t>(v.size(), 1) * sizeof(T);
  HIP_TRY(hipMalloc(reinterpret_cast<void **>(dst), n));
  if (!v.empty()) HIP_TRY(hipMemcpy(*dst, v.data(), v.size() * sizeof(T), hipMemcpyHostToDevice));
  return 0;
}

template <typename T>
static int upload_as_f4(float4 **dst, const std::vector<T> &v) {
  static_assert(sizeof(T) % sizeof(float4) == 0, "record is not a whole number of float4");
  HIP_TRY(hipMalloc(reinterpret_cast<void **>(dst), std::max<size_t>(v.size(), 1) * sizeof(T)));
  if (!v.empty()) HIP_TRY(hipMemcpy(*dst, v.data(), v.size() * sizeof(T), hipMemcpyHostToDevice));
  return 0;
}

static std::vector<float4> src_cull_f4(const HostScene &host) {
  std::vector<float4> v(host.bvh_src_cull.size() / 4);
  for (size_t i = 0; i < v.size(); ++i)
    v[i] = make_float4(host.bvh_src_cull[4 * i], host.bvh_src_cull[4 * i + 1], host.bvh_src_cull[4 * i + 2],
                       host.bvh_src_cull[4 * i + 3]);
  return v;
}

GpuScene *gpu_upload(const HostScene &host, std::string *err) {
  GpuScene *s = new GpuScene();
  s->host = host;
  if (hipGetDevice(&s->device) != hipSuccess) {
    *err = "no HIP device available";
    delete s;
    return nullptr;
  }
  std::vector<TriPair> pairs((host.isect.size() + 1) / 2);
  pack_pairs(host.isect.data(), (int)host.isect.size(), pairs.data());
  std::vector<TriGeom> geom(host.geom);
  geom.resize((size_t)host.nT + 1, TriGeom());
  for (int i = 0; i < 3; ++i)
    for (int j = 0; j < 3; ++j) geom[(size_t)host.nT].R[i][j] = host.cam[4 * i + j];
  if (upload(&s->isect, host.isect) || upload(&s->pairs, pairs) || upload(&s->geom, geom) || upload(&s->mat, host.mat) ||
      upload(&s->kd, host.kd) || upload(&s->emit_tri, host.emit_tri) || upload(&s->emit_cdf, host.emit_cdf) ||
      upload(&s->emit_pmf, host.emit_pmf) || upload(&s->emit_pmfr, pmf_reciprocals(host.emit_pmf)) ||
      upload(&s->big_pairs, host.bvh_big_pairs) || upload(&s->big_idx, host.bvh_big_idx) ||
      upload(&s->big_boxes, host.bvh_big_boxes) ||
      upload_as_f4(&s->wide, host.bvh_wide) || upload(&s->src_cull, src_cull_f4(host)) ||
      upload(&s->wtris, host.bvh_wtris) || upload(&s->pboxes, pair_boxes(host)) ||
      upload(&s->pomask, shadow_occluder_masks(host)) ||
      upload(&s->big_pomask, host.bvh_big_idx.empty()
                                 ? std::vector<uint32_t>()
                                 : shadow_occluder_masks(host, std::vector<int>(host.bvh_big_idx.begin(),
                                                                                host.bvh_big_idx.end())))) {
    *err = gpu_last_error();
    gpu_free(s);
    return nullptr;
  }
  for (const TriMat &m : host.mat) s->has_ks |= (m.flags & MAT_HAS_KS) != 0;
  {
    std::vector<int> te((size_t)host.nT, -1);
    for (int e = 0; e < host.nE; ++e) te[(size_t)host.emit_tri[(size_t)e]] = e;
    if (upload(&s->tri_emit, te)) {
      *err = gpu_last_error();
      gpu_free(s);
      return nullptr;
    }
  }
  {
    hipMemPool_t pool;
    if (hipDeviceGetDefaultMemPool(&pool, s->device) == hipSuccess) {
      uint64_t keep = ~0ull;
      (void)hipMemPoolSetAttribute(pool, hipMemPoolAttrReleaseThreshold, &keep);
    }
  }
  if ((size_t)host.nT * 3 * sizeof(double) > (size_t)kLdsGradBytes) {
    const int slots = kLdsGradBytes / (3 * (int)sizeof(double));
    std::vector<int> order(host.nT), map(host.nT, -1), inv(slots);
    for (int i = 0; i < host.nT; ++i) order[i] = i;
    std::stable_sort(order.begin(), order.end(),
                     [&](int x, int y) { return host.geom[(size_t)x].area > host.geom[(size_t)y].area; });
    for (int k = 0; k < slots; ++k) {
      map[(size_t)order[(size_t)k]] = k;
      inv[(size_t)k] = order[(size_t)k];
    }
    if (upload(&s->grad_map, map) || upload(&s->slot_tri, inv)) {
      *err = gpu_last_error();
      gpu_free(s);
      return nullptr;
    }
  }
  s->on_device = true;
  return s;
}

GpuScene *gpu_host_only(const HostScene &host) {
  GpuScene *s = new GpuScene();
  s->host = host;
  return s;
}
bool gpu_on_device(const GpuScene *s) { return s->on_device; }

void gpu_free(GpuScene *s) {
  if (!s) return;
  if (!s->on_device) {
    delete s;
    return;
  }
  (void)hipFree(s->isect);
  (void)hipFree(s->pairs);
  (void)hipFree(s->geom);
  (void)hipFree(s->mat);
  (void)hipFree(s->kd);
  (void)hipFree(s->emit_tri);
  (void)hipFree(s->emit_cdf);
  (void)hipFree(s->emit_pmf);
  (void)hipFree(s->emit_pmfr);
  (void)hipFree(s->big_pairs);
  (void)hipFree(s->big_idx);
  (void)hipFree(s->big_boxes);
  (void)hipFree(s->wide);
  (void)hipFree(s->src_cull);
  (void)hipFree(s->wtris);
  (void)hipFree(s->pboxes);
  (void)hipFree(s->pomask);
  (void)hipFree(s->big_pomask);
  (void)hipFree(s->grad_map);
  (void)hipFree(s->slot_tri);
  (void)hipFree(s->tri_emit);
  for (auto &c : s->counters) (void)hipFree(c.dev);
  for (uint32_t *p : s->counters_retired) (void)hipFree(p);
  delete s;
}

int gpu_set_kd(GpuScene *s, const float *kd_host) {
  std::memcpy(s->host.kd.data(), kd_host, s->host.kd.size() * sizeof(float));
  if (!s->on_device) return 0;
  HIP_TRY(hipMemcpy(s->kd, kd_host, s->host.kd.size() * sizeof(float), hipMemcpyHostToDevice));
  return 0;
}

int gpu_device_count() {
  int n = 0;
  if (hipGetDeviceCount(&n) != hipSuccess) return 0;
  return n;
}

static int check_params(const GpuScene *s, const RenderParams &p) {
  if (!s->on_device) {
    gpu_set_error("scene was loaded host-only (ipt_load_scene_host); it cannot be rendered");
    return -1;
  }
  if (p.width <= 0 || p.height <= 0 || p.spp <= 0 || p.row_begin < 0 || p.row_end > p.height ||
      p.row_begin > p.row_end || p.row_step < 1) {
    gpu_set_error("invalid render parameters (width/height/spp > 0, 0 <= row_begin <= row_end <= height, row_step >= 1)");
    return -1;
  }
  if ((uint64_t)p.width * (uint64_t)p.height * (uint64_t)p.spp >= (1ull << 40)) {
    gpu_set_error("too many samples (width*height*spp must be < 2^40)");
    return -1;
  }
  if (s->host.nT <= 0) {
    gpu_set_error("scene has no triangles");
    return -1;
  }
  if (p.nscenes < 1) {
    gpu_set_error("scene batch needs n_scenes >= 1");
    return -1;
  }
  return 0;
}

#ifndef IPT_DEBUG_GRID
#define IPT_DEBUG_GRID 0
#endif
template <int MODE, bool SPEC, bool BVH, int KIND>
constexpr auto kernel_of() {
  if constexpr (KIND == KIND_VBMAT) {
    static_assert(MODE == MODE_ADJ || MODE == MODE_ADJU, "the view sets' adjoint is the material adjoint, MODE_ADJ or MODE_ADJU");
    if constexpr (MODE == MODE_ADJU) return &trace_matu_views_batch_kernel<SPEC, BVH>;
    else return &trace_mat_views_batch_kernel<SPEC, BVH>;
  } else if constexpr (KIND == KIND_VBFWD) {
    static_assert(is_fwd<MODE>(), "the view sets' forward: forward instances only");
    return &trace_fwd_views_batch_kernel<MODE, SPEC, BVH>;
  } else if constexpr (KIND == KIND_VMAT) {
    static_assert(MODE == MODE_ADJ, "the views' adjoint is the bounded material adjoint");
    return &trace_mat_views_kernel<SPEC, BVH>;
  } else if constexpr (KIND == KIND_VFWD) {
    static_assert(is_fwd<MODE>(), "the views' forward: forward instances only");
    return &trace_fwd_views_kernel<MODE, SPEC, BVH>;
  } else if constexpr (KIND == KIND_MATG) {
    static_assert(MODE == MODE_ADJ || MODE == MODE_ADJU, "the material adjoint is MODE_ADJ or MODE_ADJU");
    if constexpr (MODE == MODE_ADJU) return &trace_matu_kernel<SPEC, BVH>;
    else return &trace_mat_kernel<SPEC, BVH>;
  } else if constexpr (KIND == KIND_FWDB) {
    static_assert(is_fwd<MODE>(), "the batch forward: forward instances only");
    return &trace_fwd_mat_kernel<MODE, SPEC, BVH>;
  } else {
    return &trace_kernel<MODE, SPEC, BVH>;
  }
}
constexpr const char *kernel_name(int mode, int kind) {
  return kind == KIND_VBFWD  ? "trace_fwd_views_batch_kernel"
         : kind == KIND_VBMAT ? (mode == MODE_ADJU ? "trace_matu_views_batch_kernel" : "trace_mat_views_batch_kernel")
         : kind == KIND_VFWD ? "trace_fwd_views_kernel"
         : kind == KIND_VMAT ? "trace_mat_views_kernel"
         : kind == KIND_MATG ? (mode == MODE_ADJU ? "trace_matu_kernel" : "trace_mat_kernel")
         : kind == KIND_FWDB ? "trace_fwd_mat_kernel"
                             : "trace_kernel";
}
template <int MODE, bool SPEC, bool BVH, int KIND>
static int resident_grid(GpuScene *s, size_t lds_bytes, int *grid) {
  InstCache &c = s->inst[inst_slot(MODE, SPEC, BVH, KIND)];
  if (c.grid == 0 || c.grid_lds != lds_bytes) {
    int per_cu = 0, cus = 0;
    HIP_TRY(hipOccupancyMaxActiveBlocksPerMultiprocessor(&per_cu, kernel_of<MODE, SPEC, BVH, KIND>(), kBlock, lds_bytes));
    HIP_TRY(hipDeviceGetAttribute(&cus, hipDeviceAttributeMultiprocessorCount, s->device));
    if (per_cu <= 0) {
      gpu_set_error("trace kernel cannot be resident (LDS request too large?)");
      return -1;
    }
    c.grid = per_cu * cus;
    c.grid_lds = lds_bytes;
    if (IPT_DEBUG_GRID)
      std::fprintf(stderr, "[ipt] %s<%d,%d,%d>: %zu B LDS/block, %d blocks/CU x %d CUs\n", kernel_name(MODE, KIND), MODE,
                   (int)SPEC, (int)BVH, lds_bytes, per_cu, cus);
  }
  *grid = c.grid;
  return 0;
}

static void camera_origin(const float *cam, float *org) {
  for (int i = 0; i < 3; ++i) {
    const float *M = cam + 4 * i;
    org[i] = std::fmaf(M[3], 1.f, std::fmaf(M[2], 0.f, std::fmaf(M[1], 0.f, M[0] * 0.f)));
  }
}

static TraceArgs make_args(const GpuScene *s, const RenderParams &p);
static TraceArgs make_args_scene(const GpuScene *s) {
  RenderParams p;
  p.width = p.height = p.spp = 1;
  p.max_bounces = 0;
  p.seed = 0;
  p.row_begin = 0;
  p.row_end = 1;
  return make_args(s, p);
}
static TraceArgs make_args(const GpuScene *s, const RenderParams &p) {
  TraceArgs a = TraceArgs();
  a.W = p.width;
  a.H = p.height;
  a.spp = p.spp;
  a.max_bounces = p.max_bounces < 0 ? -1 : p.max_bounces;
  a.seed = p.seed;
  const int rows = band_rows(p);
  a.n_samples = (uint64_t)rows * p.width * p.spp;
  a.nT = s->host.nT;
  a.nE = s->host.nE;
  a.kd_tables = s->host.nT <= kMaxTableTris ? 1 : 0;
  a.small_pairs = s->host.nT <= 2 * kSmallPairs ? 1 : 0;
  a.npix = (uint64_t)rows * p.width;
  a.row0 = p.row_begin;
  a.row_step = p.row_step > 1 ? p.row_step : 1;
  const uint64_t total = (uint64_t)p.height * p.width * p.spp;
  a.idx32 = total <= 0xffffffffull ? 1 : 0;
  a.m_spp = p.spp > 1 ? ~0ull / (uint64_t)p.spp + 1 : 0;
  a.m_W = p.width > 1 ? ~0ull / (uint64_t)p.width + 1 : 0;
  a.m_npix = a.npix > 1 ? ~0ull / a.npix + 1 : 0;
  for (int k = 0; k < 6; ++k) a.root_box[k] = s->host.bvh_root_box[k];
  for (int k = 0; k < 4; ++k) a.tree_sphere[k] = s->host.bvh_sphere[k];
  a.src_cull = s->src_cull;
  std::memcpy(a.cam, s->host.cam, sizeof a.cam);
  a.emit_pmfr = s->emit_pmfr;
  camera_origin(a.cam, a.cam_org);
  a.rec_cap = p.max_bounces >= 0 ? p.max_bounces + 1 : 0;
  a.pboxes = s->pboxes;
  a.pomask = s->host.nE > 0 ? s->pomask : nullptr;
  a.nscenes = p.nscenes > 1 ? p.nscenes : 1;
  a.bps = 1;
  a.seed_stride = p.seed_stride;
  a.out_stride = a.n_samples * 3;
  a.adj_stride = (uint64_t)p.width * p.height * 3;
  a.rc_spp = (p.spp > 0 && p.spp <= (1 << 24) && (p.spp & (p.spp - 1)) == 0) ? 1.0f / (float)p.spp : 0.f;
  a.rc_W = (p.width > 0 && (p.width & (p.width - 1)) == 0) ? 1.0f / (float)p.width : 0.f;
  a.rc_H = (p.height > 0 && (p.height & (p.height - 1)) == 0) ? 1.0f / (float)p.height : 0.f;
  return a;
}

static bool use_bvh(const GpuScene *s) {
  if (s->host.bvh_nodes.empty()) return false;
  if (s->accel == IPT_ACCEL_BVH) return true;
  if (s->accel == IPT_ACCEL_BRUTE) return false;
  return s->host.nT >= kBvhMinTris;
}

constexpr size_t kLaneWsBytes = (size_t)6 * kBlock * sizeof(uint32_t);

static size_t bvh_lds(const GpuScene *s, TraceArgs &a, size_t base, bool stage = true, bool big_copy = true,
                      bool lane_words = false) {
  const size_t nw = s->host.bvh_wide.size();
  a.bvh_wide = s->wide;
  a.bvh_wtris = s->wtris;
  a.bvh_wide_lds = (stage && nw * kWideF4 * sizeof(float4) <= (size_t)kBvhLdsNodeBytes) ? (int)nw : 0;
  a.bvh_big_lds = big_copy && IPT_PATH_CULL ? 1 : 0;
  a.big_pomask = (IPT_SHADOW_PO && s->host.nE > 0 && !s->host.bvh_big_idx.empty()) ? s->big_pomask : nullptr;
  a.coop_stride = 7 * s->host.bvh_wdepth + 8;
  a.bvh_nbig = (int)s->host.bvh_big_pairs.size();
  a.bvh_big = s->big_pairs;
  a.bvh_big_idx = s->big_idx;
  a.bvh_big_boxes = s->big_boxes;
  const size_t head = bvh_lds_offset(base) + (size_t)a.bvh_wide_lds * kWideF4 * sizeof(float4) +
                      (size_t)a.bvh_nbig * 6 * sizeof(float) + (a.bvh_big_lds ? big_lds_bytes(a.bvh_nbig) : 0) +
                      emit_lds_bytes(s->host.nE);
  return head + (size_t)(kBlock / 64) * 8 * a.coop_stride * sizeof(uint32_t) + (lane_words ? kLaneWsBytes : 0);
}

static size_t table_bytes(const TraceArgs &a) {
  return (a.kd_tables ? (size_t)6 * a.nT * sizeof(float) : 0) +
         (a.small_pairs ? (size_t)kE3Floats * ((a.nT + 1) / 2) * sizeof(float) + 12 + (size_t)a.nT * kIsectLdsFloats * sizeof(float) +
                              (IPT_PATH_CULL ? (size_t)((a.nT + 1) / 2) * sizeof(TriPair) : 0) +
                              (IPT_SHADOW_PO && a.pomask ? (size_t)a.nT * a.nE * sizeof(uint32_t) : 0)
                        : 0);
}

struct StreamScratch {
  void *p = nullptr;
  hipStream_t st = nullptr;
  int alloc(size_t bytes, hipStream_t stream) {
    st = stream;
    HIP_TRY(hipMallocAsync(&p, std::max<size_t>(bytes, 16), st));
    return 0;
  }
  ~StreamScratch() {
    if (p) (void)hipFreeAsync(p, st);
  }
};

static int stream_counters(GpuScene *s, hipStream_t st, int words, uint32_t **out, void **scratch) {
  const size_t bytes = (size_t)words * sizeof(uint32_t);
  hipStreamCaptureStatus cap = hipStreamCaptureStatusNone;
  HIP_TRY(hipStreamIsCapturing(st, &cap));
  if (cap != hipStreamCaptureStatusNone) {
    HIP_TRY(hipMallocAsync(scratch, bytes, st));
    HIP_TRY(hipMemsetAsync(*scratch, 0, bytes, st));
    *out = (uint32_t *)*scratch;
    return 0;
  }
  std::lock_guard<std::mutex> lk(s->counters_mu);
  GpuScene::Counters *c = nullptr;
  for (auto &e : s->counters)
    if (e.stream == st) c = &e;
  if (c && c->words < words) {
    s->counters_retired.push_back(c->dev);
    c->dev = nullptr;
    c->words = 0;
  }
  if (!c || c->dev == nullptr) {
    const int w = std::max(words, 16);
    uint32_t *dev = nullptr;
    HIP_TRY(hipMalloc(reinterpret_cast<void **>(&dev), (size_t)w * sizeof(uint32_t)));
    HIP_TRY(hipMemsetAsync(dev, 0, (size_t)w * sizeof(uint32_t), st));
    if (c) {
      c->dev = dev;
      c->words = w;
    } else {
      s->counters.push_back({st, w, dev});
      c = &s->counters.back();
    }
  }
  *out = c->dev;
  return 0;
}

#ifndef IPT_GUIDED_TAIL
#define IPT_GUIDED_TAIL 4
#endif

static uint32_t launch_grabs(bool guided, uint64_t units, uint64_t c, uint64_t small, uint64_t nb, uint64_t rw) {
  const uint64_t chunks = guided ? nb + (units - nb * c + small - 1) / small : (units + c - 1) / c;
  return (uint32_t)((chunks > rw ? chunks - rw : 0) + rw);
}
#ifndef IPT_DYN_SMALL_CHUNK
#define IPT_DYN_SMALL_CHUNK 64
#endif

struct LaunchIO {
  const float *kd = nullptr;
  float *out = nullptr;
  const float *adj = nullptr;
  double *grad = nullptr;
  const uint8_t *target = nullptr;
  double *edges = nullptr;
  const TriMat *mat = nullptr;
  const float *views = nullptr;
  int nviews = 0;
  hipStream_t stream = nullptr;
  size_t tail = 0;
};

template <int MODE, bool SPEC, bool BVH, int KIND>
static int launch_inst(GpuScene *s, const TraceArgs &a, size_t lds, const LaunchIO &io) {
  const hipStream_t st = io.stream;
  int grid = 0;
  if (lds > 160 * 1024) {
    gpu_set_error("LDS footprint of the launch exceeds 160 KiB");
    return -1;
  }
  if (resident_grid<MODE, SPEC, BVH, KIND>(s, lds, &grid)) return -1;
  if (a.n_samples == 0) return 0;
  TraceArgs b = a;
  if (a.nscenes > 1) {
    b.bps = std::max(1, grid / a.nscenes);
    grid = b.bps * a.nscenes;
  }
  b.chunk = 0;
  b.chunk_ctr = nullptr;
  StreamScratch cap_ctr;
  if (IPT_DYN_CHUNKS) {
    const uint64_t waves = (uint64_t)(a.nscenes > 1 ? b.bps : grid) * (kBlock / 64);
    uint64_t c = (a.n_samples / (waves * IPT_DYN_CHUNKS_PER_WAVE) + 63) / 64 * 64;
    c = std::min<uint64_t>(std::max<uint64_t>(c, IPT_DYN_MIN_CHUNK), 4096);
    uint64_t units = a.n_samples, small = std::min<uint64_t>(c, IPT_DYN_SMALL_CHUNK);
    if (a.fused) {
      c = a.chunk;
      while (c > 1 && (a.npix + c - 1) / c < waves && (c / 2) * (uint64_t)a.spp >= 64) c /= 2;
      b.group = std::min<uint32_t>(a.group, (uint32_t)c);
      small = std::min<uint64_t>(c, std::max<uint64_t>(1, 64 / (uint64_t)a.spp));
      units = a.npix;
    }
    if (!BVH) {
      small = c;
      c *= IPT_BF_BIG;
    }
    b.chunk = (uint32_t)c;
    b.chunk_small = (uint32_t)small;
    const uint64_t rw = waves;
    constexpr bool guided = kGuided<BVH>();
    const uint64_t tail = guided ? rw * (uint64_t)(BVH ? IPT_GUIDED_TAIL : IPT_BF_TAIL) * small : 0;
    const uint64_t nb = guided ? (units > tail ? (units - tail) / c : 0) : 0;
    b.chunk_big_n = (uint32_t)nb;
    b.grabs = launch_grabs(guided, units, c, small, nb, rw);
    cap_ctr.st = st;
    const int words = a.nscenes * kCtrStride;
    if (stream_counters(s, st, words, &b.chunk_ctr, &cap_ctr.p)) return -1;
  }
  StreamScratch grec, mring;
  if (MODE == MODE_ADJU) {
    const size_t fields = SPEC ? kRecFieldsSpec : kRecFieldsDiffuse;
    const size_t waves = (size_t)grid * (kBlock / 64), chunk = (size_t)kPoolSlots * fields * sizeof(float);
    b.pool_chunks = (int)std::max<size_t>(16, std::min<size_t>(63, ((size_t)IPT_ADJU_POOL_MB << 20) / (waves * chunk)));
    if (g_adju_pool.load() > 0) b.pool_chunks = g_adju_pool.load();
    b.grec_stride = (uint64_t)b.pool_chunks * kPoolSlots * fields;
    b.rec_cap = std::min(kAdjuRing, a.rec_lds + kPoolMaxChunks * kPoolSlots);
    if (grec.alloc(waves * b.grec_stride * sizeof(float), st)) return -1;
    b.grec = (float *)grec.p;
    if (kSub > 0) {
      if (mring.alloc(waves * (size_t)kMrEnt * 64 * 3 * sizeof(float), st)) return -1;
      b.mring = (float *)mring.p;
    }
  }
  if (g_fail_launches.load() > 0 && g_fail_launches.fetch_sub(1) > 0) {
    gpu_set_error("launch failed on request (ipt_debug_fail_launches)");
    return -1;
  }
  if (IPT_DEBUG_GRID)
    std::fprintf(stderr,
                 "[ipt] launch %s<%d,%d,%d> grid=%d lds=%zu bps=%d chunk=%u chunk_small=%u chunk_big_n=%u grabs=%u group=%u "
                 "rec_cap=%d rec_lds=%d pool_chunks=%d grec_stride=%llu grad_slots=%d bvh_wide_lds=%d bvh_big_lds=%d "
                 "coop_stride=%d mean_off=%u mean_wstride=%u nslots=%d mat_stride=%u kd_tables=%d small_pairs=%d "
                 "sample_major=%d\n",
                 kernel_name(MODE, KIND), MODE, (int)SPEC, (int)BVH, grid, lds, b.bps, b.chunk, b.chunk_small,
                 b.chunk_big_n, b.grabs, b.group, b.rec_cap, b.rec_lds, b.pool_chunks, (unsigned long long)b.grec_stride,
                 b.grad_slots, b.bvh_wide_lds, b.bvh_big_lds, b.coop_stride, b.mean_off, b.mean_wstride, b.nslots,
                 b.mat_stride, b.kd_tables, b.small_pairs, b.sample_major);
  auto enqueue = [&](auto... trailing) {
    hipLaunchKernelGGL((kernel_of<MODE, SPEC, BVH, KIND>()), dim3(grid), dim3(kBlock), lds, st, b, s->isect, s->pairs,
                       s->geom, io.mat ? io.mat : s->mat, io.kd ? io.kd : s->kd, s->emit_tri, s->emit_cdf, s->emit_pmf,
                       io.out, io.adj, io.grad, io.target, io.edges, trailing...);
  };
  if constexpr (KIND == KIND_VBMAT) enqueue(s->tri_emit, io.views, io.nviews);
  else if constexpr (KIND == KIND_VBFWD) enqueue(io.views, io.nviews);
  else if constexpr (KIND == KIND_VMAT) enqueue(s->tri_emit, io.views);
  else if constexpr (KIND == KIND_VFWD) enqueue(io.views);
  else if constexpr (KIND == KIND_MATG) enqueue(s->tri_emit);
  else enqueue();
  HIP_TRY(hipGetLastError());
  return 0;
}

__global__ __launch_bounds__(kBlock) void kdpi_kernel(const float *__restrict__ kd, int n, float *__restrict__ out) {
  const int i = blockIdx.x * kBlock + threadIdx.x;
  if (i < n) out[i] = kd[i] / kPiF;
}

template <int MODE, bool SPEC, int KIND>
static int launch_bvh_pick(GpuScene *s, TraceArgs &a, size_t *lds, size_t tail) {
  InstCache &c = s->inst[inst_slot(MODE, SPEC, false, KIND)];
  const bool opt[4][2] = {{true, true}, {true, false}, {false, true}, {false, false}};
  const size_t base = *lds;
  if (c.pick_opt < 0 || c.pick_base != base || c.pick_tail != tail) {
    int best = -1, best_per_cu = 0;
    for (int k = 0; k < 4; ++k) {
      TraceArgs b = a;
      const size_t l = bvh_lds_offset(bvh_lds(s, b, base, opt[k][0], opt[k][1], is_fwd<MODE>())) + tail;
      if (l > 160 * 1024) continue;
      int per_cu = 0;
      HIP_TRY(hipOccupancyMaxActiveBlocksPerMultiprocessor(&per_cu, kernel_of<MODE, SPEC, true, KIND>(), kBlock, l));
      if (per_cu > best_per_cu) {
        best = k;
        best_per_cu = per_cu;
      }
    }
    if (best < 0) {
      gpu_set_error("BVH trace kernel cannot be resident (LDS request too large?)");
      return -1;
    }
    c.pick_opt = best;
    c.pick_base = base;
    c.pick_tail = tail;
  }
  const int k = c.pick_opt;
  *lds = bvh_lds(s, a, base, opt[k][0], opt[k][1], is_fwd<MODE>());
  return 0;
}

template <int MODE, int KIND = KIND_TRACE>
static int launch(GpuScene *s, TraceArgs a, size_t lds, const LaunchIO &io) {
  const hipStream_t st = io.stream;
  const int msets = kind_views(KIND) ? 1 : kind_view_sets(KIND) ? a.nscenes / io.nviews : a.nscenes;
  a.mat_stride = (io.mat && msets > 1) ? (uint32_t)a.nT : 0u;
  if constexpr (is_fwd<MODE>() && KIND == KIND_TRACE) {
    if (a.mat_stride) return launch<MODE, KIND_FWDB>(s, a, lds, io);
  }
  StreamScratch kdpi;
  if (MODE != MODE_GRAPH && !a.kd_tables && a.n_samples > 0) {
    const int n = 3 * s->host.nT * msets;
    if (kdpi.alloc((size_t)n * sizeof(float), st)) return -1;
    hipLaunchKernelGGL(kdpi_kernel, dim3((n + kBlock - 1) / kBlock), dim3(kBlock), 0, st, io.kd ? io.kd : s->kd, n,
                       (float *)kdpi.p);
    HIP_TRY(hipGetLastError());
    a.kdpi_g = (const float *)kdpi.p;
  }
  auto run = [&](auto spec, auto bvh) {
    constexpr bool SPEC = decltype(spec)::value, BVH = decltype(bvh)::value;
    if constexpr (BVH) {
      if (launch_bvh_pick<MODE, SPEC, KIND>(s, a, &lds, io.tail)) return -1;
    }
    if (io.tail) {
      a.mean_off = (uint32_t)bvh_lds_offset(lds);
      lds = a.mean_off + io.tail;
    }
    return launch_inst<MODE, SPEC, BVH, KIND>(s, a, lds, io);
  };
  constexpr std::true_type yes;
  constexpr std::false_type no;
  if constexpr (MODE == MODE_ADJW) return run(no, no);
  else if (use_bvh(s)) return s->has_ks ? run(yes, yes) : run(no, yes);
  else return s->has_ks ? run(yes, no) : run(no, no);
}

int gpu_render_samples(GpuScene *s, const RenderParams &p, const float *kd_dev, float *samples_dev, void *stream) {
  if (check_params(s, p)) return -1;
  const TraceArgs a = make_args(s, p);
  LaunchIO io;
  io.kd = kd_dev, io.out = samples_dev, io.stream = (hipStream_t)stream;
  return launch<MODE_FWD>(s, a, table_bytes(a), io);
}

int gpu_pixel_mean(const float *samples_dev, int64_t npix, int spp, float *hdr_dev, uint8_t *ldr_dev, void *stream) {
  if (npix <= 0) return 0;
  const int blocks = (int)((npix + kBlock - 1) / kBlock);
  hipLaunchKernelGGL(pixel_mean_kernel, dim3(blocks), dim3(kBlock), 0, (hipStream_t)stream, samples_dev, npix, spp,
                     hdr_dev, ldr_dev);
  HIP_TRY(hipGetLastError());
  return 0;
}

template <int KIND = KIND_TRACE>
static int render_samples_sm(GpuScene *s, const RenderParams &p, const float *kd_dev, float *samples_dev,
                             void *stream, const TriMat *mat_dev, const float *views_dev = nullptr,
                             int nviews = 0) {
  if (check_params(s, p)) return -1;
  TraceArgs a = make_args(s, p);
  a.sample_major = 1;
  LaunchIO io;
  io.kd = kd_dev, io.out = samples_dev, io.mat = mat_dev, io.views = views_dev, io.nviews = nviews;
  io.stream = (hipStream_t)stream;
  return launch<MODE_FWD, KIND>(s, a, table_bytes(a), io);
}
int gpu_render_samples_sm(GpuScene *s, const RenderParams &p, const float *kd_dev, float *samples_dev,
                          void *stream) {
  return render_samples_sm(s, p, kd_dev, samples_dev, stream, nullptr);
}

static int pixel_mean_sm_sets(const float *samples_dev, int64_t npix, int spp, int nsets, float *hdr_dev,
                              uint8_t *ldr_dev, void *stream) {
  if (npix <= 0 || nsets <= 0) return 0;
  const int blocks = (int)((npix + kBlock - 1) / kBlock);
  hipLaunchKernelGGL(pixel_mean_sm_kernel, dim3(blocks, nsets), dim3(kBlock), 0, (hipStream_t)stream, samples_dev,
                     npix, spp, hdr_dev, ldr_dev);
  HIP_TRY(hipGetLastError());
  return 0;
}

int gpu_pixel_mean_sm(const float *samples_dev, int64_t npix, int spp, float *hdr_dev, uint8_t *ldr_dev,
                      void *stream) {
  return pixel_mean_sm_sets(samples_dev, npix, spp, 1, hdr_dev, ldr_dev, stream);
}

#ifndef IPT_FUSED_MEAN
#define IPT_FUSED_MEAN 1
#endif
#ifndef IPT_FUSED_GRAB_SAMPLES
#define IPT_FUSED_GRAB_SAMPLES 256
#endif
#ifndef IPT_FUSED_WAVE_BYTES
#define IPT_FUSED_WAVE_BYTES 6144
#endif
struct FusedShape {
  int slots, group, per_grab;
};
#ifndef IPT_FUSED_BVH
#define IPT_FUSED_BVH 0
#endif
#ifndef IPT_FUSED_BVH_WAVE_BYTES
#define IPT_FUSED_BVH_WAVE_BYTES 3072
#endif
static FusedShape fused_shape(const RenderParams &p, bool bvh) {
  const FusedShape none = {0, 0, 0};
  if (!IPT_FUSED_MEAN || !IPT_DYN_CHUNKS) return none;
  if ((uint64_t)p.width * (uint64_t)p.height * (uint64_t)p.spp > 0xffffffffull || p.spp > 256) return none;
  int bytes = IPT_FUSED_WAVE_BYTES;
  if (bvh) {
    if (!IPT_FUSED_BVH) return none;
    bytes = IPT_FUSED_BVH_WAVE_BYTES;
  }
  const int slots = std::min(16, bytes / (12 * p.spp));
  const bool long_paths = p.max_bounces < 0 || p.max_bounces > 8;
  const int cap = slots / (long_paths ? 4 : 2);
  if (cap < 1) return none;
  int g = 1;
  while (2 * g <= cap && 2 * g * p.spp <= 256) g *= 2;
  if (g * p.spp < 32) return none;
  const int per_grab = std::min(8, (IPT_FUSED_GRAB_SAMPLES + g * p.spp - 1) / (g * p.spp));
  return {slots, g, per_grab};
}

template <int KIND = KIND_TRACE>
static int render_impl(GpuScene *s, const RenderParams &p, const float *kd_dev, float *hdr_dev, uint8_t *ldr_dev,
                       void *stream, const TriMat *mat_dev, const float *views_dev = nullptr, int nviews = 0) {
  if (check_params(s, p)) return -1;
  const int64_t npix = (int64_t)band_rows(p) * p.width;
  const int sets = p.nscenes > 1 ? p.nscenes : 1;
  const FusedShape fs = fused_shape(p, use_bvh(s));
  if (fs.group > 0) {
    TraceArgs a = make_args(s, p);
    a.fused = 1;
    a.group = (uint32_t)fs.group;
    a.chunk = (uint32_t)(fs.group * fs.per_grab);
    a.nslots = fs.slots;
    a.mean_wstride = (uint32_t)(((2 * fs.slots + 3) & ~3) + fused_entry_words((uint32_t)fs.group, use_bvh(s)) +
                                3 * fs.slots * p.spp + 3) & ~3u;
    a.ldr = ldr_dev;
    a.out_stride = (uint64_t)npix * 3;
    LaunchIO io;
    io.kd = kd_dev, io.out = hdr_dev, io.mat = mat_dev, io.views = views_dev, io.nviews = nviews;
    io.stream = (hipStream_t)stream;
    io.tail = (size_t)(kBlock / 64) * a.mean_wstride * sizeof(float);
    return launch<MODE_FWDM, KIND>(s, a, table_bytes(a), io);
  }
  StreamScratch ws;
  if (ws.alloc((size_t)sets * npix * p.spp * 3 * sizeof(float), (hipStream_t)stream)) return -1;
  if (render_samples_sm<KIND>(s, p, kd_dev, (float *)ws.p, stream, mat_dev, views_dev, nviews)) return -1;
  return pixel_mean_sm_sets((const float *)ws.p, npix, p.spp, sets, hdr_dev, ldr_dev, stream);
}
int gpu_render(GpuScene *s, const RenderParams &p, const float *kd_dev, float *hdr_dev, uint8_t *ldr_dev,
               void *stream) {
  return render_impl(s, p, kd_dev, hdr_dev, ldr_dev, stream, nullptr);
}

int gpu_set_material_params(GpuScene *s, const float *kd, const float *ks, const float *ke) {
  HostScene &h = s->host;
  if (kd) std::memcpy(h.kd.data(), kd, h.kd.size() * sizeof(float));
  std::vector<char> em((size_t)h.nT, 0);
  for (int e : h.emit_tri) em[(size_t)e] = 1;
  for (int i = 0; i < h.nT; ++i) {
    TriMat &m = h.mat[(size_t)i];
    for (int c = 0; c < 3; ++c) {
      if (ks) m.ks[c] = (m.flags & MAT_HAS_KS) ? ks[3 * i + c] : 0.f;
      if (ke) m.ke[c] = em[(size_t)i] ? ke[3 * i + c] : 0.f;
    }
  }
  if (!s->on_device) return 0;
  if (kd) HIP_TRY(hipMemcpy(s->kd, h.kd.data(), h.kd.size() * sizeof(float), hipMemcpyHostToDevice));
  if (ks || ke) HIP_TRY(hipMemcpy(s->mat, h.mat.data(), h.mat.size() * sizeof(TriMat), hipMemcpyHostToDevice));
  return 0;
}

static int pack_materials(GpuScene *s, const float *ks_dev, const float *ke_dev, int sets, hipStream_t st,
                          StreamScratch &buf, const TriMat **mat) {
  *mat = nullptr;
  if (!ks_dev && !ke_dev) return 0;
  const int nT = s->host.nT;
  if (buf.alloc((size_t)sets * nT * sizeof(TriMat), st)) return -1;
  hipLaunchKernelGGL(pack_mat_kernel, dim3((nT + kBlock - 1) / kBlock, sets), dim3(kBlock), 0, st, s->mat, ks_dev,
                     ke_dev, s->tri_emit, nT, (TriMat *)buf.p);
  HIP_TRY(hipGetLastError());
  *mat = (const TriMat *)buf.p;
  return 0;
}

static int batch_kd(GpuScene *s, const float **kd_dev, int sets, hipStream_t st, StreamScratch &buf) {
  if (*kd_dev || sets <= 1) return 0;
  const int n = 3 * s->host.nT;
  const size_t total = (size_t)sets * n;
  if (buf.alloc(total * sizeof(float), st)) return -1;
  hipLaunchKernelGGL(replicate_kernel, dim3((unsigned)((total + kBlock - 1) / kBlock)), dim3(kBlock), 0, st, s->kd, n,
                     total, (float *)buf.p);
  HIP_TRY(hipGetLastError());
  *kd_dev = (const float *)buf.p;
  return 0;
}

struct LaunchMaterials {
  StreamScratch tab, kdrep;
  const TriMat *mat = nullptr;
  int fill(GpuScene *s, const float **kd_dev, const float *ks_dev, const float *ke_dev, int sets, void *stream) {
    if (batch_kd(s, kd_dev, sets, (hipStream_t)stream, kdrep)) return -1;
    return pack_materials(s, ks_dev, ke_dev, sets, (hipStream_t)stream, tab, &mat);
  }
};

static int check_sets(int n_scenes) {
  if (n_scenes > 65535) {
    gpu_set_error("material overrides: at most 65535 material sets per launch");
    return -1;
  }
  return 0;
}

static int render_mat_impl(GpuScene *s, const RenderParams &p, const float *kd_dev, const float *ks_dev,
                           const float *ke_dev, float *hdr_dev, uint8_t *ldr_dev, void *stream) {
  const int sets = p.nscenes > 1 ? p.nscenes : 1;
  LaunchMaterials m;
  if (m.fill(s, &kd_dev, ks_dev, ke_dev, sets, stream)) return -1;
  return render_impl(s, p, kd_dev, hdr_dev, ldr_dev, stream, m.mat);
}

int gpu_render_mat(GpuScene *s, const RenderParams &p, const float *kd_dev, const float *ks_dev, const float *ke_dev,
                   float *hdr_dev, uint8_t *ldr_dev, void *stream) {
  if (check_params(s, p)) return -1;
  if (p.nscenes > 1) {
    gpu_set_error("material overrides do not support the scene batch (n_scenes > 1)");
    return -1;
  }
  return render_mat_impl(s, p, kd_dev, ks_dev, ke_dev, hdr_dev, ldr_dev, stream);
}

int gpu_render_mat_batch(GpuScene *s, const RenderParams &p, const float *kd_dev, const float *ks_dev,
                         const float *ke_dev, float *hdr_dev, void *stream) {
  if (check_params(s, p) || check_sets(p.nscenes)) return -1;
  if (p.max_bounces < 0 || p.max_bounces > kMaxAdjBounces) {
    gpu_set_error("material batch: give max_bounces in 0..62 (the unbounded estimator is not supported; one material set: ipt_adjoint_mat_unbounded_dev)");
    return -1;
  }
  if (s->host.nT > kMaxAdjTris) {
    gpu_set_error("material batch supports at most 65535 triangles");
    return -1;
  }
  return render_mat_impl(s, p, kd_dev, ks_dev, ke_dev, hdr_dev, nullptr, stream);
}

static TraceArgs adjoint_args(const GpuScene *s, const RenderParams &p) {
  TraceArgs a = make_args(s, p);
  a.sample_major = IPT_ADJ_PIXEL_MAJOR ? 0 : 1;
  if (s->grad_map) {
    a.grad_slots = kLdsGradBytes / (3 * (int)sizeof(double));
    a.grad_map = s->grad_map;
    a.slot_tri = s->slot_tri;
  } else {
    a.grad_slots = s->host.nT;
  }
  return a;
}

template <int KIND>
static int ring_lds_slots(GpuScene *s, size_t base, size_t per, bool bvh, size_t *cached_base, int *cached_nl,
                          int *rec_lds) {
  int nl = bvh ? IPT_ADJU_LDS_SLOTS_BVH : IPT_ADJU_LDS_SLOTS;
  if (IPT_ADJU_LDS_SLOTS_FIXED >= 0) {
    nl = IPT_ADJU_LDS_SLOTS_FIXED;
  } else if (!bvh) {
    if (*cached_base != base) {
      auto occ = [&](size_t bytes, int *o) {
        return s->has_ks ? hipOccupancyMaxActiveBlocksPerMultiprocessor(o, kernel_of<MODE_ADJU, true, false, KIND>(), kBlock, bytes)
                         : hipOccupancyMaxActiveBlocksPerMultiprocessor(o, kernel_of<MODE_ADJU, false, false, KIND>(), kBlock, bytes);
      };
      int occ0 = 0, best = 0;
      HIP_TRY(occ(base, &occ0));
      for (int k = nl; k > 0 && best == 0; --k) {
        int o = 0;
        HIP_TRY(occ(base + k * per, &o));
        if (o >= occ0 && base + k * per <= IPT_ADJU_LDS_CAP) best = k;
      }
      *cached_base = base;
      *cached_nl = best;
    }
    nl = *cached_nl;
  }
// ... 208 lines not shown
    gpu_set_error("ipt_views_rays_host: view outside [0, n_views)");
    return -1;
  }
  const uint64_t total = (uint64_t)p.width * (uint64_t)p.height * (uint64_t)p.spp;
  for (int64_t i = 0; i < n; ++i)
    if (index[i] < 0 || (uint64_t)index[i] >= total) {
      gpu_set_error("ipt_views_rays_host: a sample index outside [0, width*height*spp)");
      return -1;
    }
  if (n <= 0) return 0;
  const TraceArgs a = make_args(s, p);
  struct Buf {
    void *p = nullptr;
    ~Buf() {
      if (p) (void)hipFree(p);
    }
  } ix, o, d;
  const size_t n3 = (size_t)n * 3 * sizeof(float);
  HIP_TRY(hipMalloc(&ix.p, (size_t)n * sizeof(int64_t)));
  HIP_TRY(hipMalloc(&o.p, n3));
  HIP_TRY(hipMalloc(&d.p, n3));
  HIP_TRY(hipMemcpy(ix.p, index, (size_t)n * sizeof(int64_t), hipMemcpyHostToDevice));
  hipLaunchKernelGGL(view_rays_kernel, dim3((unsigned)((n + kBlock - 1) / kBlock)), dim3(kBlock), 0, nullptr, v->dev,
                     view, p.width, p.height, p.spp, a.rc_W, a.rc_H, p.seed, n, (const int64_t *)ix.p, (float *)o.p,
                     (float *)d.p);
  HIP_TRY(hipGetLastError());
  HIP_TRY(hipMemcpy(org, o.p, n3, hipMemcpyDeviceToHost));
  HIP_TRY(hipMemcpy(dir, d.p, n3, hipMemcpyDeviceToHost));
  return 0;
}

static size_t matu_lds_base(const GpuScene *s, const TraceArgs &a, size_t *per) {
  *per = (size_t)(s->has_ks ? kRecFieldsSpec : kRecFieldsDiffuse) * kBlock * sizeof(float);
  return mat_lds_doubles(a.grad_slots, s->host.nE, s->has_ks) * sizeof(double) + table_bytes(a) +
         mat_carry_bytes(use_bvh(s)) + (size_t)kBlock * sizeof(uint32_t);
}

template <int KIND>
static int matu_ring(GpuScene *s, TraceArgs &a, size_t *cached_base, int *cached_nl, size_t *lds) {
  size_t per = 0;
  const size_t base = matu_lds_base(s, a, &per);
  a.rec_cap = kAdjuRing;
  if (ring_lds_slots<KIND>(s, base, per, use_bvh(s), cached_base, cached_nl, &a.rec_lds)) return -1;
  a.rec_lds = (int)std::min<size_t>((size_t)a.rec_lds, (160 * 1024 - base) / per);
  *lds = base + (size_t)a.rec_lds * per;
  return 0;
}

static int check_unbounded(const RenderParams &p) {
  if (p.max_bounces >= 0) {
    gpu_set_error("unbounded material adjoint: max_bounces must be -1 (no bounce cap); ipt_adjoint_mat_dev takes max_bounces in 0..62");
    return -1;
  }
  return 0;
}
int gpu_adjoint_mat_unbounded(GpuScene *s, const RenderParams &p, const float *kd_dev, const float *ks_dev,
                              const float *ke_dev, const float *adj_dev, double *grad_dev, void *stream) {
  if (check_unbounded(p) || check_params(s, p)) return -1;
  if (p.nscenes > 1) {
    gpu_set_error("unbounded material adjoint: the scene batch (n_scenes > 1) is not supported");
    return -1;
  }
  if (s->host.nT > kMaxAdjTris) {
    gpu_set_error("adjoint supports at most 65535 triangles");
    return -1;
  }
  TraceArgs a = adjoint_args(s, p);
  size_t per = 0, lds = 0;
  if (matu_lds_base(s, a, &per) + per > 160 * 1024) {
    gpu_set_error("unbounded material adjoint: the Kd/Ks/Ke bins and the scene's LDS tables plus one record slot per lane exceed 160 KiB");
    return -1;
  }
  if (matu_ring<KIND_MATG>(s, a, &s->matu_base, &s->matu_nl, &lds)) return -1;
  LaunchMaterials m;
  if (m.fill(s, &kd_dev, ks_dev, ke_dev, 1, stream)) return -1;
  LaunchIO io;
  io.kd = kd_dev, io.adj = adj_dev, io.grad = grad_dev, io.mat = m.mat, io.stream = (hipStream_t)stream;
  return launch<MODE_ADJU, KIND_MATG>(s, a, lds, io);
}

static int view_sets_unbounded_params(GpuScene *s, const GpuViews *v, RenderParams &p, int n_sets) {
  if (p.max_bounces >= 0) {
    gpu_set_error("unbounded views batch: max_bounces must be -1 (no bounce cap); ipt_render_views_batch_dev and ipt_adjoint_views_batch_dev take max_bounces in 0..62");
    return -1;
  }
  if (n_sets < 1) {
    gpu_set_error("unbounded views batch: n_sets must be >= 1");
    return -1;
  }
  if ((int64_t)n_sets * v->n > 65535) {
    gpu_set_error("unbounded views batch: at most 65535 (material set, view) pairs per launch (n_sets * n_views)");
    return -1;
  }
  if (s->host.nT > kMaxAdjTris) {
    gpu_set_error("unbounded views batch supports at most 65535 triangles");
    return -1;
  }
  if (v->scene != s) {
    gpu_set_error("views: the handle was created for another scene");
    return -1;
  }
  p.nscenes = n_sets * v->n;
  if (check_params(s, p)) return -1;
  size_t per = 0;
  const size_t base = matu_lds_base(s, adjoint_args(s, p), &per);
  if (base + per > 160 * 1024) {
    gpu_set_error("unbounded views batch: the Kd/Ks/Ke bins and the scene's LDS tables plus one record slot per lane exceed 160 KiB");
    return -1;
  }
  return 0;
}

int gpu_render_views_batch_unbounded(GpuScene *s, const GpuViews *v, RenderParams p, int n_sets, const float *kd_dev,
                                     const float *ks_dev, const float *ke_dev, float *hdr_dev, void *stream) {
  if (view_sets_unbounded_params(s, v, p, n_sets)) return -1;
  LaunchMaterials m;
  if (m.fill(s, &kd_dev, ks_dev, ke_dev, n_sets, stream)) return -1;
  return render_impl<KIND_VBFWD>(s, p, kd_dev, hdr_dev, nullptr, stream, m.mat, v->dev, v->n);
}

int gpu_adjoint_views_batch_unbounded(GpuScene *s, const GpuViews *v, RenderParams p, int n_sets, const float *kd_dev,
                                      const float *ks_dev, const float *ke_dev, const float *adj_dev,
                                      double *grad_dev, void *stream) {
  if (view_sets_unbounded_params(s, v, p, n_sets)) return -1;
  TraceArgs a = adjoint_args(s, p);
  size_t lds = 0;
  if (matu_ring<KIND_VBMAT>(s, a, &s->vbmatu_base, &s->vbmatu_nl, &lds)) return -1;
  LaunchMaterials m;
  if (m.fill(s, &kd_dev, ks_dev, ke_dev, n_sets, stream)) return -1;
  LaunchIO io;
  io.kd = kd_dev, io.adj = adj_dev, io.grad = grad_dev, io.mat = m.mat, io.views = v->dev, io.nviews = v->n;
  io.stream = (hipStream_t)stream;
  return launch<MODE_ADJU, KIND_VBMAT>(s, a, lds, io);
}

#ifndef IPT_ADJW_MIN_SAMPLES
#define IPT_ADJW_MIN_SAMPLES (8ull << 20)
#endif
int gpu_adjoint(GpuScene *s, const RenderParams &p, const float *kd_dev, const float *adj_dev, double *grad_dev,
                void *stream) {
  if (check_params(s, p)) return -1;
  if (p.max_bounces > kMaxAdjBounces) {
    gpu_set_error("adjoint requires max_bounces <= 62 (vertex records live in LDS); -1 = unbounded");
    return -1;
  }
  const bool unbounded = p.max_bounces < 0;
  if (s->host.nT > kMaxAdjTris) {
    gpu_set_error("adjoint supports at most 65535 triangles");
    return -1;
  }
  TraceArgs a = adjoint_args(s, p);
  const size_t fields = (size_t)(s->has_ks ? kRecFieldsSpec : kRecFieldsDiffuse);
  const size_t per = fields * kBlock * sizeof(float);
  const size_t base = (size_t)a.grad_slots * 3 * sizeof(double) + table_bytes(a) +
                      (size_t)kBlock * sizeof(uint32_t);
  if (unbounded) {
    a.rec_cap = kAdjuRing;
    if (ring_lds_slots<KIND_TRACE>(s, base, per, use_bvh(s), &s->adju_base, &s->adju_nl, &a.rec_lds)) return -1;
  }
  const size_t lds = base + (size_t)(unbounded ? a.rec_lds : a.rec_cap) * per;
  if (lds > 160 * 1024) {
    gpu_set_error(unbounded ? "unbounded adjoint: the scene's LDS tables plus one record slot per lane exceed 160 KiB"
                            : "adjoint LDS footprint exceeds 160 KiB; lower max_bounces");
    return -1;
  }
  LaunchIO io;
  io.kd = kd_dev, io.adj = adj_dev, io.grad = grad_dev, io.stream = (hipStream_t)stream;
  if (unbounded) return launch<MODE_ADJU>(s, a, lds, io);
  const size_t lane_words = IPT_ADJW_LANE_LDS ? kLaneWsBytes : 0;
  bool wide = !use_bvh(s) && !s->has_ks && 6 * (lds + lane_words) <= 160 * 1024 &&
              (uint64_t)a.n_samples * (uint64_t)std::max(1, a.nscenes) >= IPT_ADJW_MIN_SAMPLES;
  if (const char *e = std::getenv("IPT_ADJW")) wide = std::atoi(e) != 0 && !use_bvh(s) && !s->has_ks;
  if (wide) return launch<MODE_ADJW>(s, a, lds + lane_words, io);
  return launch<MODE_ADJ>(s, a, lds, io);
}

int gpu_graph(GpuScene *s, const RenderParams &p, const uint8_t *target_dev, double *acc_dev, void *stream) {
  if (check_params(s, p)) return -1;
  TraceArgs a = make_args(s, p);
  const size_t bins = graph_lds_doubles(s->host.nT, s->host.nE) * sizeof(double);
  a.lds_edges = bins <= (size_t)IPT_GRAPH_LDS_KB * 1024 ? 1 : 0;
  a.kd_tables = 0;
  a.sample_major = IPT_GRAPH_PIXEL_MAJOR ? 0 : 1;
  LaunchIO io;
  io.target = target_dev, io.edges = acc_dev, io.stream = (hipStream_t)stream;
  return launch<MODE_GRAPH>(s, a, (a.lds_edges ? bins : 0) + table_bytes(a), io);
}

__device__ __forceinline__ uint64_t mix64(uint64_t z) {
  z += 0x9e3779b97f4a7c15ull;
  z = (z ^ (z >> 30)) * 0xbf58476d1ce4e5b9ull;
  z = (z ^ (z >> 27)) * 0x94d049bb133111ebull;
  return z ^ (z >> 31);
}
__device__ __forceinline__ float rand_exp_float(uint64_t r, int emin, int emax) {
  const int e = emin + (int)((r >> 23) % (uint64_t)(emax - emin + 1));
  const uint32_t m = (uint32_t)r & 0x7fffffu;
  const uint32_t sgn = (uint32_t)(r >> 63) << 31;
  return __uint_as_float(sgn | ((uint32_t)(e + 127) << 23) | m);
}
__global__ __launch_bounds__(kBlock) void math_selftest_kernel(uint64_t n, uint64_t seed,
                                                               unsigned long long *counts) {
  unsigned long long c[8] = {0, 0, 0, 0, 0, 0, 0, 0};
  const uint64_t stride = (uint64_t)gridDim.x * kBlock;
  for (uint64_t i = (uint64_t)blockIdx.x * kBlock + threadIdx.x; i < n; i += stride) {
    const uint64_t r0 = mix64(seed ^ (i * 8 + 0)), r1 = mix64(seed ^ (i * 8 + 1)), r2 = mix64(seed ^ (i * 8 + 2));
    const uint64_t r3 = mix64(seed ^ (i * 8 + 3)), r4 = mix64(seed ^ (i * 8 + 4));
    {
      const float x = fabsf(rand_exp_float(r0, -96, 127));
      c[0] += __float_as_uint(sqrt_core(x)) != __float_as_uint(sqrtf(x));
    }
    {
      const int e = -767 + (int)((r1 >> 52) % 1768u);
      const double x = __longlong_as_double((long long)(((uint64_t)(e + 1023) << 52) | (r1 & 0xfffffffffffffull)));
      c[1] += __double_as_longlong(dsqrt_core(x)) != __double_as_longlong(sqrt(x));
    }
    {
      const float a = rand_exp_float(r2, -100, 60);
      const float b = rand_exp_float(r3, -60, 60);
      const float q = a / b;
      if (fabsf(q) >= 0x1p-120f && fabsf(q) <= 0x1p120f)
        c[2] += __float_as_uint(div_inrange(a, b)) != __float_as_uint(q);
    }
    {
      const float a = rand_exp_float(r4, -40, 20);
      const float b = (r0 & 1 ? 1.f : -1.f) * (kMinDotUp + (1.f - kMinDotUp) * (float)(r3 >> 40) * 0x1p-24f);
      c[3] += __float_as_uint(div_inrange(a, b)) != __float_as_uint(a / b);
    }
    {
      V3 v;
      float comp[3];
      for (int k = 0; k < 3; ++k) {
        const uint64_t rk = mix64(r4 ^ (uint64_t)(k + 11));
        const int kind = (int)(rk & 15);
        if (kind == 0) comp[k] = 0.f;
        else if (kind == 1) comp[k] = (rk & 16) ? -0.f : 0.f;
        else if (kind == 2) comp[k] = rand_exp_float(rk, -149 + 23, -85);
        else if (kind == 3) comp[k] = rand_exp_float(rk, 25, 35);
        else if (kind == 4) comp[k] = rand_exp_float(rk, -6, -2);
        else comp[k] = rand_exp_float(rk, -30, 3);
      }
      v = mk(comp[0], comp[1], comp[2]);
      const V3 u = unit(v), w = unit_ieee(v);
      c[5] += (__float_as_uint(u.x) != __float_as_uint(w.x)) || (__float_as_uint(u.y) != __float_as_uint(w.y)) ||
              (__float_as_uint(u.z) != __float_as_uint(w.z));
      const float n2 = dot3(v, v);
      const uint32_t m = min(min((__float_as_uint(v.x) << 1) - 1u, (__float_as_uint(v.y) << 1) - 1u),
                             (__float_as_uint(v.z) << 1) - 1u);
      const bool fast = n2 >= 0x1p-6f && n2 <= 0x1p60f && m >= ((0x25u << 24) - 1u);
      c[6] += fast;
      if (fast) {
        const float sq = sqrtf(n2);
        const V3 q = div3_core(v, sq);
        c[4] += (__float_as_uint(q.x) != __float_as_uint(v.x / sq)) || (__float_as_uint(q.y) != __float_as_uint(v.y / sq)) ||
                (__float_as_uint(q.z) != __float_as_uint(v.z / sq));
      }
    }
    {
      const int W = 1 + (int)(r0 % 65536u), cc = (int)(r1 % (uint64_t)W);
      const float u0 = (float)(uint32_t)r2 * 2.3283064e-10f + 1.1641532e-10f;
      const float a = 2.f * ((float)cc + u0);
      c[7] += __float_as_uint(div_inrange(a, (float)W)) != __float_as_uint(a / (float)W);
    }
  }
  for (int k = 0; k < 8; ++k)
    if (c[k]) atomicAdd(&counts[k], c[k]);
}

int gpu_selftest_math(uint64_t n, uint64_t seed, uint64_t *counts_host) {
  unsigned long long *d = nullptr;
  HIP_TRY(hipMalloc(reinterpret_cast<void **>(&d), 8 * sizeof(unsigned long long)));
  int rc = 0;
  if (hipMemset(d, 0, 8 * sizeof(unsigned long long)) != hipSuccess) rc = -1;
  if (!rc) {
    hipLaunchKernelGGL(math_selftest_kernel, dim3(2048), dim3(kBlock), 0, 0, n, seed, d);
    if (hipGetLastError() != hipSuccess || hipDeviceSynchronize() != hipSuccess) rc = -1;
  }
  if (!rc && hipMemcpy(counts_host, d, 8 * sizeof(unsigned long long), hipMemcpyDeviceToHost) != hipSuccess) rc = -1;
  (void)hipFree(d);
  if (rc) gpu_set_error("math self-test failed to run");
  return rc;
}

__device__ __forceinline__ uint32_t probe_allow(const uint32_t *masks, const int *emit_tri, int nE, int nT, int src,
                                                int target) {
  if (!masks || src < 0 || src >= nT) return 0xffffffffu;
  for (int e = 0; e < nE; ++e)
    if (emit_tri[e] == target) return masks[src * nE + e];
  return 0xffffffffu;
}

template <bool BVH>
__global__ __launch_bounds__(kBlock) void closest_hit_kernel(const TriIsect *__restrict__ isect,
                                                             const TriPair *__restrict__ pairs, const TraceArgs a,
                                                             int small, int64_t n, const float *__restrict__ org,
                                                             const float *__restrict__ dir,
                                                             const int *__restrict__ targets,
                                                             const int *__restrict__ sources,
                                                             const int *__restrict__ emit_tri, float *__restrict__ t_out,
                                                             int *__restrict__ i_out) {
  extern __shared__ double lds[];
  const int tid = threadIdx.x;
  const int nT = a.nT;
  const int nP = (nT + 1) >> 1;
  float *lds_e3 = reinterpret_cast<float *>(lds);
  const f2 *e3 = nullptr;
  if (small) {
    for (int i = tid; i < kE3Floats * nP; i += kBlock) lds_e3[i] = small_table_entry(pairs, i);
    e3 = reinterpret_cast<const f2 *>(lds_e3);
  }
  float *lds_is = lds_e3 + kE3Floats * nP;
  lds_is += (4 - (int)((lds_is - lds_e3) & 3)) & 3;
  float *lds_pr = lds_is + kIsectLdsFloats * nT;
  if (!BVH && small) {
    const float *g = reinterpret_cast<const float *>(isect);
    for (int i = tid; i < kIsectLdsFloats * nT; i += kBlock) lds_is[i] = g[i];
    if (IPT_PATH_CULL) {
      const float *gp = reinterpret_cast<const float *>(pairs);
      for (int i = tid; i < 36 * nP; i += kBlock) lds_pr[i] = gp[i];
    }
  }
  BvhView bv;
  bv.isect = isect;
  bv.big = nullptr;
  bv.big_idx = nullptr;
// ... 245 lines not shown
```

inverse_path_tracer_amd/csrc/scene_layout.h:

```cpp
#pragma once
#include <stdint.h>

namespace ipt {

struct TriIsect {
  float c[3];
  float n[3];
  float e0[4];
  float e1[4];
  float e2[4];
  float pad[2];
};
static_assert(sizeof(TriIsect) == 80, "TriIsect layout");

struct TriPair {
  float f[18][2];
};
static_assert(sizeof(TriPair) == 144, "TriPair layout");
inline void pack_pairs(const TriIsect *t, int nT, TriPair *out) {
  for (int j = 0; 2 * j < nT; ++j) {
    for (int h = 0; h < 2; ++h) {
      const int i = 2 * j + h;
      float src[18] = {0.f};
      if (i < nT) {
        const TriIsect &T = t[i];
        const float v[18] = {T.c[0], T.c[1], T.c[2], T.n[0], T.n[1], T.n[2], T.e0[0], T.e0[1], T.e0[2],
                             T.e0[3], T.e1[0], T.e1[1], T.e1[2], T.e1[3], T.e2[0], T.e2[1], T.e2[2], T.e2[3]};
        for (int k = 0; k < 18; ++k) src[k] = v[k];
      }
      for (int k = 0; k < 18; ++k) out[j].f[k][h] = src[k];
    }
  }
}

struct TriGeom {
  float v[3][3];
  float vn[3][3];
  float area;
  float R[3][3];
  uint32_t flags;
  float pad[3];
};
static_assert(sizeof(TriGeom) == 128, "TriGeom layout");

enum : uint32_t { GEOM_AXIS_FLAT = 1u };

enum : uint32_t { MAT_HAS_KS = 1u, MAT_SPECULAR = 2u };

struct TriMat {
  float ks[3];
  float shininess;
  float ke[3];
  uint32_t flags;
};
static_assert(sizeof(TriMat) == 32, "TriMat layout");

struct BvhNode {
  float q[4][4];
};
static_assert(sizeof(BvhNode) == 64, "BvhNode layout");
constexpr int kBvhLeafPairBits = 4;
constexpr int kBvhMaxDepth = 32;
struct BvhPair {
  float f[18][2];
  int32_t idx[2];
  int32_t pad[2];
};
static_assert(sizeof(BvhPair) == 160, "BvhPair layout");

struct WideNode {
  float s[8][8];
};
static_assert(sizeof(WideNode) == 256, "WideNode layout");
constexpr int32_t kWideEmpty = (int32_t)0x80000000;

struct PairBox2 {
  float f[6][2];
};
static_assert(sizeof(PairBox2) == 48, "PairBox2 layout");

struct DevScene {
  int nT, nE;
  const TriIsect *isect;
  const TriGeom *geom;
  const TriMat *mat;
  const float *kd;
  const int *emit_tri;
  const float *emit_cdf;
  const float *emit_pmf;
  float cam[16];
};

struct RenderParams;
inline int band_rows(const RenderParams &p);
struct RenderParams {
  int width, height, spp;
  int max_bounces;
  uint64_t seed;
  int row_begin, row_end;
  int row_step = 1;
  int nscenes = 1;
  uint64_t seed_stride = 0;
};
inline int band_rows(const RenderParams &p) {
  const int n = p.row_end - p.row_begin;
  return n <= 0 ? 0 : (p.row_step <= 1 ? n : (n + p.row_step - 1) / p.row_step);
}

}
```

inverse_path_tracer_amd/csrc/trace_body.h:

```cpp
  extern __shared__ double lds[];
  const int tid = threadIdx.x;
  const int set = a.nscenes > 1 ? (int)(blockIdx.x % (uint32_t)a.nscenes) : 0;
  const uint32_t sblock = a.nscenes > 1 ? blockIdx.x / (uint32_t)a.nscenes : blockIdx.x;
  const uint32_t sgrid = a.nscenes > 1 ? (uint32_t)a.bps : gridDim.x;
  const uint64_t seed = a.seed + (uint64_t)set * a.seed_stride;
  int mset = 0, view = set;
  if (VSETS) {
    const int nviews = karg<int>(sizeof(TraceKernArgs) + (MATG ? sizeof(void *) : 0) + sizeof(const float *));
    mset = set / nviews;
    view = set - mset * nviews;
  }
  if (a.nscenes > 1) {
    if (!VIEWS) kd += (size_t)set * 3 * a.nT;
    else if (VSETS) kd += (size_t)mset * 3 * a.nT;
    if (!VIEWS && (MATG || MATB)) mat += (size_t)set * a.mat_stride;
    else if (VSETS) mat += (size_t)mset * a.mat_stride;
    if (is_fwd<MODE>()) out_samples += (size_t)set * a.out_stride;
  }
  const float *kdpi_g = a.kdpi_g ? a.kdpi_g + (VIEWS ? (VSETS ? (size_t)mset * 3 * a.nT : (size_t)0) : (size_t)set * 3 * a.nT) : nullptr;
  constexpr int nthr = kBlock;
  const int nT = a.nT, nE = a.nE;
  const int vmax = a.rec_cap;
  double *lds_acc = lds;
  int n_acc = 0;
  if (is_adj<MODE>()) {
    n_acc = a.grad_slots * 3;
    if (MATG) n_acc = (int)mat_lds_doubles(a.grad_slots, nE, SPEC);
  } else if (MODE == MODE_GRAPH && a.lds_edges) {
    n_acc = (int)graph_lds_doubles(nT, nE);
  }
  float *tab = reinterpret_cast<float *>(lds + n_acc);
  if (a.kd_tables) {
    for (int i = tid; i < 3 * nT; i += nthr) {
      const float v = kd[i];
      tab[i] = v;
      tab[3 * nT + i] = v / kPiF;
    }
  }
  const lds_f32 *tab_l = (const lds_f32 *)tab;
  const gbl_f32 *kd_g = (const gbl_f32 *)kd;
  auto kd3 = [&](int t) -> V3 {
    if (a.kd_tables) return mk(tab_l[3 * t], tab_l[3 * t + 1], tab_l[3 * t + 2]);
    return mk(kd_g[3 * t], kd_g[3 * t + 1], kd_g[3 * t + 2]);
  };
  auto ke3 = [&](int t) -> V3 {
    const gbl_f32 *q = (const gbl_f32 *)mat + (size_t)t * (sizeof(TriMat) / sizeof(float)) + offsetof(TriMat, ke) / sizeof(float);
    return mk(q[0], q[1], q[2]);
  };
  auto kdpi3 = [&](int t) -> V3 {
    if (a.kd_tables) return mk(tab_l[3 * nT + 3 * t], tab_l[3 * nT + 3 * t + 1], tab_l[3 * nT + 3 * t + 2]);
    const gbl_f32 *q = (const gbl_f32 *)kdpi_g + 3 * t;
    return mk(q[0], q[1], q[2]);
  };
  const f2 *e3 = nullptr;
  float *lds_e3 = tab + (a.kd_tables ? 6 * nT : 0);
  const int nP = (nT + 1) >> 1;
  if (a.small_pairs) {
    for (int i = tid; i < kE3Floats * nP; i += nthr) lds_e3[i] = small_table_entry(pairs, i);
    e3 = reinterpret_cast<const f2 *>(lds_e3);
  }
  float *lds_is = lds_e3 + (a.small_pairs ? kE3Floats * nP : 0);
  lds_is += (4 - (int)((lds_is - reinterpret_cast<float *>(lds)) & 3)) & 3;
  if (kIsectLdsFloats != 0 && a.small_pairs) {
    const float *g = reinterpret_cast<const float *>(isect);
    for (int i = tid; i < kIsectLdsFloats * nT; i += nthr) lds_is[i] = g[i];
  }
  float *lds_pr = lds_is + (a.small_pairs ? kIsectLdsFloats * nT : 0);
  if (a.small_pairs && IPT_PATH_CULL) {
    const float *g = reinterpret_cast<const float *>(pairs);
    for (int i = tid; i < 36 * nP; i += nthr) lds_pr[i] = g[i];
  }
  uint32_t *lds_po = reinterpret_cast<uint32_t *>(lds_pr + (a.small_pairs && IPT_PATH_CULL ? 36 * nP : 0));
  const bool po = a.small_pairs && IPT_SHADOW_PO && a.pomask;
  if (po)
    for (int i = tid; i < nT * nE; i += nthr) lds_po[i] = a.pomask[i];
  float *lds_rec = a.small_pairs ? reinterpret_cast<float *>(lds_po) + (po ? nT * nE : 0) : lds_e3;
  constexpr bool kCarryLds = MATG && MODE == MODE_ADJU && !BVH;
  lds_u32 *carry_ws = nullptr;
  if (kCarryLds) {
    carry_ws = (lds_u32 *)lds_rec;
    lds_rec += kCarryWords * kBlock;
  }
  if (is_adj<MODE>()) lds_rec += kBlock;
  BvhView bv;
  bv.isect = isect;
  bv.big = nullptr;
  bv.big_idx = nullptr;
  bv.big_e3 = nullptr;
  bv.nbig = 0;
  bv.big_boxes = nullptr;
  bv.big_lds = nullptr;
  bv.emit_is = nullptr;
  constexpr bool kLaneLds = (BVH && is_fwd<MODE>()) || (!BVH && MODE == MODE_ADJW && IPT_ADJW_LANE_LDS);
  lds_u32 *lane_ws = nullptr;
  if (!BVH && kLaneLds)
    lane_ws = (lds_u32 *)(lds_rec + (size_t)vmax * kRecFieldsDiffuse * kBlock);
  CoopView cv;
  cv.wn = nullptr;
  cv.wn_lds = false;
  cv.wt = a.bvh_wtris;
  cv.stk = nullptr;
  cv.stride = a.coop_stride;
  for (int k = 0; k < 6; ++k) cv.root[k] = a.root_box[k];
  for (int k = 0; k < 4; ++k) cv.sphere[k] = a.tree_sphere[k];
  if (BVH) {
    const size_t rec_words = is_badj<MODE>()    ? (size_t)vmax * (SPEC ? kRecFieldsSpec : kRecFieldsDiffuse) * kBlock
                             : MODE == MODE_ADJU ? (size_t)a.rec_lds * (SPEC ? kRecFieldsSpec : kRecFieldsDiffuse) * kBlock
                                                 : 0;
    char *base = reinterpret_cast<char *>(lds);
    const size_t off = bvh_lds_offset((size_t)(reinterpret_cast<char *>(lds_rec + rec_words) - base));
    float4 *lw = reinterpret_cast<float4 *>(base + off);
    cv.wn = a.bvh_wide;
    if (a.bvh_wide_lds > 0) {
      for (int i = tid; i < kWideF4 * a.bvh_wide_lds; i += nthr) lw[i] = a.bvh_wide[i];
      cv.wn = lw;
      cv.wn_lds = true;
    }
    float *be3 = reinterpret_cast<float *>(lw + kWideF4 * a.bvh_wide_lds);
    for (int i = tid; i < 6 * a.bvh_nbig; i += nthr) {
      const int j = i / 6, kf = (i % 6) >> 1, h = i & 1;
      be3[i] = a.bvh_big[j].f[9 + 4 * kf][h];
    }
    bv.big = a.bvh_big;
    bv.big_idx = a.bvh_big_idx;
    bv.big_boxes = a.bvh_big_boxes;
    bv.big_e3 = reinterpret_cast<const f2 *>(be3);
    bv.nbig = a.bvh_nbig;
    float *after = big_lds_copy(a, be3 + 6 * a.bvh_nbig, reinterpret_cast<float *>(lds), tid, nthr, bv);
    if (emit_lds_bytes(nE)) {
      for (int i = tid; i < 20 * nE; i += nthr) after[i] = reinterpret_cast<const float *>(isect)[20 * emit_tri[i / 20] + i % 20];
      bv.emit_is = after;
      after += 20 * nE;
    }
    cv.stk = reinterpret_cast<uint32_t *>(after) + (tid >> 6) * 8 * a.coop_stride;
    if (kLaneLds) lane_ws = (lds_u32 *)(reinterpret_cast<uint32_t *>(after) + (kBlock / 64) * 8 * a.coop_stride);
  }
  for (int i = tid; i < n_acc; i += nthr) lds_acc[i] = 0.0;
  __syncthreads();
  auto bins_add = [&](bool in_lds, double *glob, size_t off, int n, const double *v) {
    if (in_lds) {
      lds_f64 *b = (lds_f64 *)lds_acc + off;
      for (int i = 0; i < n; ++i) __hip_atomic_fetch_add(b + i, v[i], __ATOMIC_RELAXED, __HIP_MEMORY_SCOPE_WORKGROUP);
    } else {
      gbl_f64 *b = (gbl_f64 *)glob + off;
      for (int i = 0; i < n; ++i) __hip_atomic_fetch_add(b + i, v[i], __ATOMIC_RELAXED, __HIP_MEMORY_SCOPE_AGENT);
    }
  };

  gbl_f32 *upool = nullptr;
  if (MODE == MODE_ADJU)
    upool = (gbl_f32 *)a.grec + ((size_t)blockIdx.x * (kBlock / 64) + (tid >> 6)) * a.grec_stride;
  gbl_f32 *umr = nullptr;
  if (MODE == MODE_ADJU && kSub > 0)
    umr = (gbl_f32 *)a.mring + ((size_t)blockIdx.x * (kBlock / 64) + (tid >> 6)) * (kMrEnt * 64 * 3) + (tid & 63) * 3;
  {
  const uint32_t wave = __builtin_amdgcn_readfirstlane((sblock * kBlock + tid) >> 6);
  const uint32_t nwaves = (sgrid * kBlock) >> 6;
  const TraceArgs &ar = a;
  const bool dyn = a.chunk != 0;
  uint64_t next, end;
  if (dyn) {
    chunk_range<kGuided<BVH>()>(ar, wave, ar.n_samples, next, end);
  } else {
    next = (ar.n_samples * wave) / nwaves;
    end = (ar.n_samples * (wave + 1)) / nwaves;
  }
  bool exhausted = !dyn;
  uint32_t glp = 0, gnp = 0, gslots = 0, fj = 0, sdone = 0;
  uint64_t pl0 = 0, pl1 = 0;
  uint32_t sfree = MODE == MODE_FWDM ? (a.nslots >= 32 ? ~0u : (1u << a.nslots) - 1u) : 0u;
  bool started = false;

  bool active = false;
  Rng st;
  V3 p = mk(0.f, 0.f, 0.f), d = p;
  V3 L = p, Le_r = p, Ld = p, M = mk(1.f, 1.f, 1.f);
  auto set_le = [&](V3 v) {
    if (kLaneLds) {
      ((lds_f32 *)lane_ws)[3 * kBlock + tid] = v.x;
      ((lds_f32 *)lane_ws)[4 * kBlock + tid] = v.y;
      ((lds_f32 *)lane_ws)[5 * kBlock + tid] = v.z;
    } else {
      Le_r = v;
    }
  };
  auto le = [&]() -> V3 {
    if (kLaneLds)
      return mk(((lds_f32 *)lane_ws)[3 * kBlock + tid], ((lds_f32 *)lane_ws)[4 * kBlock + tid],
                ((lds_f32 *)lane_ws)[5 * kBlock + tid]);
    return Le_r;
  };
  V3 Scar = mk(0.f, 0.f, 0.f), Mlo = mk(1.f, 1.f, 1.f);
  int rhi = 0, rslot = 0;
  constexpr bool kTri0Carry = MATG && MODE == MODE_ADJU;
  static_assert(!kTri0Carry || kSub == 0, "the unbounded material adjoint has no sub-chunked sweep (IPT_ADJU_SUB)");
  int tri0_r = 0;
  auto carry_at = [&](int f, int l) -> lds_u32 * {
    asm volatile("" : "+v"(l));
    return carry_ws + f * kBlock + l;
  };
  auto carry_put3 = [&](int f, V3 v) {
    lds_f32 *w = (lds_f32 *)carry_at(f, tid);
    w[0] = v.x;
    w[kBlock] = v.y;
    w[2 * kBlock] = v.z;
  };
  auto carry_get3 = [&](int f, int l) -> V3 {
    const lds_f32 *w = (const lds_f32 *)carry_at(f, (tid & ~63) + l);
    return mk(w[0], w[kBlock], w[2 * kBlock]);
  };
  int usub = 0;
  auto pending = [&]() { return MODE == MODE_ADJU && kSub > 0 && usub > 0; };
  constexpr uint32_t kNoChunks = 0x00ffffffu;
  uint32_t ctab = kNoChunks | ((uint32_t)vmax << 24);
  uint64_t pfree = MODE == MODE_ADJU ? (a.pool_chunks >= 64 ? ~0ull : (1ull << a.pool_chunks) - 1ull) : 0ull;
  auto vcap_of = [&]() { return (int)(ctab >> 24); };
  float weight = 1.f;
  V3 pix = p;
  int k = 0, dst = 0;
  int ptri_r = -1;
  uint64_t witem_r = 0;
  auto set_item = [&](uint64_t w) {
    if (kLaneLds) {
      lane_ws[tid] = (uint32_t)w;
      lane_ws[kBlock + tid] = (uint32_t)(w >> 32);
    } else if (kCarryLds) {
      lds_u32 *q = carry_at(7, tid);
      q[0] = (uint32_t)w;
      q[kBlock] = (uint32_t)(w >> 32);
// ... 140 lines not shown
              pixel_entry(a, seed, glp + (uint32_t)lane, e);
              lds_u32 *w = fused_entries(a) + kEntryWords * lane;
#pragma unroll
              for (int i = 0; i < kEntryWords; ++i) w[i] = e[i];
            }
          }
          if (kInph) {
            __builtin_amdgcn_fence(__ATOMIC_RELEASE, "wavefront");
            __builtin_amdgcn_wave_barrier();
          }
        } else {
          exhausted = true;
        }
      }
    } else if (next >= end && !exhausted) {
      uint32_t c = 0;
      if (lane == 0) c = atomicAdd(a.chunk_ctr + (size_t)set * kCtrStride, 1u);
      c = (uint32_t)__shfl((int)c, 0);
      uint64_t start, stop;
      chunk_range<kGuided<BVH>()>(a, nwaves + c, a.n_samples, start, stop);
      if (start < a.n_samples) {
        next = start;
        end = stop;
      } else {
        exhausted = true;
        if (lane == 0) grab_failed(a.chunk_ctr + (size_t)set * kCtrStride, c, a.grabs);
      }
    }
    const bool wants = !active && !pending();
    const uint64_t need = __ballot(wants);
#ifdef IPT_PHASE_TIMING
    const uint64_t act0_ = ~need;
#endif
    if (MODE == MODE_FWDM) {
      const uint32_t fn = gnp * (uint32_t)a.spp;
      if (need && fj < fn) {
        const uint32_t rank =
            __builtin_amdgcn_mbcnt_hi((uint32_t)(need >> 32), __builtin_amdgcn_mbcnt_lo((uint32_t)need, 0u));
        if (!active && fj + rank < fn) {
          const uint32_t j = fj + rank;
          const uint32_t s = (gnp & (gnp - 1u)) == 0u ? j >> __builtin_ctz(gnp) : j / gnp;
          const uint32_t q = j - s * gnp;
          if (IPT_REFILL_ABLATE && !BVH) {
            uint64_t g = (uint64_t)(glp * (uint32_t)a.spp + j);
            if (IPT_REFILL_ABLATE < 2) {
              int r, c;
              local_rc(a, glp + q, r, c);
              g = (uint64_t)((uint32_t)r * (uint32_t)a.W + (uint32_t)c) * (uint32_t)a.spp + s;
            }
            rng_init(st, seed + g);
            p = mk(a.cam_org[0], a.cam_org[1], a.cam_org[2]);
            d = mk(a.cam[2], a.cam[6], a.cam[10]);
            if (IPT_REFILL_ABLATE == 3) {
              const float u0 = uniform(st), u1 = uniform(st);
              d = mk(2.f * ((float)((glp + q) & 511u) + u0) * a.rc_W - 1.f,
                     1.f - 2.f * ((float)((glp + q) >> 9) + u1) * a.rc_H, 1.f);
            }
          } else if (kInph) {
            float cf, rf;
            rng_init(st, entry_sample(a, q, s, cf, rf));
            camera_ray_f(a.cam, a.cam_org, st, rf, cf, a.W, a.H, a.rc_W, a.rc_H, p, d);
          } else {
            int r, c;
            item_ray_ls(a, seed, glp + q, s, st, p, d, r, c);
          }
          if (kInph) set_item((uint64_t)(((gslots >> (4 * q)) & 15u) | (s << 4)));
          else set_item((uint64_t)((gslots >> (4 * q)) & 15u) | ((uint64_t)s << 4));
          L = mk(0.f, 0.f, 0.f);
          set_le(L);
          Ld = L;
          M = mk(1.f, 1.f, 1.f);
          k = 0;
          set_ptri(-1);
          active = true;
        }
        fj += (uint32_t)__popcll(need);
        fj = fj < fn ? fj : fn;
      }
    } else if (need) {
      const uint32_t rank =
          __builtin_amdgcn_mbcnt_hi((uint32_t)(need >> 32), __builtin_amdgcn_mbcnt_lo((uint32_t)need, 0u));
      if (wants) {
        const uint64_t w = next + rank;
        if (w < end) {
          set_item(w);
          int r, c;
          item_ray(a, seed, w, st, p, d, r, c);
          L = mk(0.f, 0.f, 0.f);
          set_le(L);
          Ld = L;
          M = mk(1.f, 1.f, 1.f);
          k = 0;
          set_ptri(-1);
          if (MODE == MODE_ADJU) {
            rhi = 0;
            rslot = 0;
            if (!kSub) Mlo = mk(1.f, 1.f, 1.f);
            ctab = kNoChunks | ((uint32_t)vmax << 24);
          }
          if (MODE == MODE_GRAPH) {
            weight = 1.f;
            dst = nT;
            const uint8_t *px = target + ((size_t)r * a.W + c) * 3;
            pix = mk((float)px[0] / 255.0f, (float)px[1] / 255.0f, (float)px[2] / 255.0f);
          }
          active = true;
        }
      }
      next += (uint64_t)__popcll(need);
    }
    PHASE(0)
    PHASE_LANES(10, active && !((act0_ >> (tid & 63)) & 1ull))
    if (__ballot(active || pending()) == 0 &&
        (MODE != MODE_FWDM || (exhausted && sdone == 0 && fj >= gnp * (uint32_t)a.spp)))
      break;
#ifdef IPT_PHASE_TIMING
    tacc[6] += 1;
    tacc[7] += __popcll(__ballot(active));
#endif

    float t = 0.f;
    int hit = -1;
    if (BVH) {
      bool qn = false;
      if (active) {
        bvh_prepass<false>(bv, p, d, t, hit, -1);
        qn = coop_root_test(cv, p, d, t) && !(IPT_TREE_SKIP && tree_skip(a.src_cull, ptri(), d));
      }
      SUBPHASE_BEGIN
      coop_cast<false>(cv, qn, p, d, t, hit);
      SUBPHASE_END(8)
    } else if (active) {
      if (IPT_PATH_CULL && e3)
        hit = closest_hit_pairs_culled((const lds_f32 *)lds_pr, a.pboxes, nT, p, d, t);
      else
        hit = cast_bf(pairs, e3, nT, p, d, t);
    }
    PHASE(1)
    const bool vertex = active && hit >= 0;
    bool finished = false, escaped = false;
    if (active && hit < 0) {
      finished = true;
      escaped = (k > 0);
      if (MODE != MODE_GRAPH) {
        const V3 Le = le();
        L = mk(fmaf(M.x, Le.x + Ld.x, L.x), fmaf(M.y, Le.y + Ld.y, L.y), fmaf(M.z, Le.z + Ld.z, L.z));
      }
    }
    const int tri = hit;
    V3 nh = p, din = d, sd = d, nd = d;
    bool shadow = false, cont = false;
    bool wantc = false, refill = false;
    uint32_t nitem = 0;
    int emitter = 0;
    float ct = 0.f, coeff = 0.f, speci = 0.f, specd = 0.f;
    if (vertex) {
      const V3 q = along(p, d, t);
      if (MODE == MODE_GRAPH) {
        (void)uniform(st);
        const float wf = weight * 1.f;
        const double v[5] = {(double)weight, (double)wf, (double)(wf * pix.x), (double)(wf * pix.y),
                             (double)(wf * pix.z)};
        const size_t bin = (size_t)dst * nT + tri;
        bins_add(a.lds_edges != 0, edges, a.lds_edges ? bin * kEdgeL : bin * kEdgeW, 5, v);
      } else if (k == 0) {
        set_le(ke3(tri));
        if (kTri0Carry) {
          if (kCarryLds) *carry_at(6, tid) = (uint32_t)tri;
          else tri0_r = tri;
        }
      }
      nh = shading_normal(geom[tri], q);
      p = q;
      Ld = mk(0.f, 0.f, 0.f);
      if (nE > 0) {
        const float u = uniform(st);
        int ie = 0;
        while (ie < nE && !(emit_cdf[ie] >= u)) ++ie;
        ie = ie < nE ? ie : nE - 1;
        const float r1 = uniform(st), r2 = uniform(st);
        const double sq = dsqrt_core((double)r1);
        const float ca = (float)(1.0 - sq);
        const float cb = (float)(sq * (double)(1.f - r2));
        const float cc = (float)((double)r2 * sq);
        const TriGeom &ge = geom[emit_tri[ie]];
        const V3 pt = mk(fmaf(cc, ge.v[2][0], fmaf(cb, ge.v[1][0], ca * ge.v[0][0])),
                         fmaf(cc, ge.v[2][1], fmaf(cb, ge.v[1][1], ca * ge.v[0][1])),
                         fmaf(cc, ge.v[2][2], fmaf(cb, ge.v[1][2], ca * ge.v[0][2])));
        sd = unit(sub(pt, q));
        ct = dot3(nh, sd);
        emitter = ie;
        shadow = !(ct < 0.f);
      }
      if (!(a.max_bounces >= 0 && k == a.max_bounces)) {
        const float pr = uniform(st);
        if (kInphM) {
          wantc = pr < kPRR;
        } else if (pr < kPRR) {
          const TriMat &m = mat[tri];
          const bool spec = SPEC && (MODE != MODE_GRAPH) && (m.flags & MAT_SPECULAR);
          const float uphi = uniform(st);
          const float phi = (float)(2.0 * kPi * (double)uphi);
          const float ut = uniform(st);
          float cth, sth, psamp;
          if (!spec) {
            cth = sqrt_core(ut);
            const float omu = 1.0f - ut;
            sth = omu > 0.f ? sqrt_core(omu) : 0.f;
            psamp = kInvPiF;
          } else {
            const double cd = pow_d((double)ut, 1.0 / ((double)m.shininess + 1.0));
            cth = (float)cd;
            sth = (float)sqrt(1.0 - cd * cd);
            psamp = pow_f((m.shininess + 1.f) * cth, m.shininess);
          }
          float sp, cp;
          sincos_f(phi, sp, cp);
          const V3 h = mk(sth * cp, sth * sp, cth);
          const TriGeom &g = geom[tri];
          nd = unit(mk(fmaf(g.R[0][2], h.z, fmaf(g.R[0][1], h.y, g.R[0][0] * h.x)),
                       fmaf(g.R[1][2], h.z, fmaf(g.R[1][1], h.y, g.R[1][0] * h.x)),
                       fmaf(g.R[2][2], h.z, fmaf(g.R[2][1], h.y, g.R[2][0] * h.x))));
          if (MODE != MODE_GRAPH) {
            if (SPEC && (m.flags & MAT_HAS_KS)) speci = phong(m.shininess, nh, din, nd);
            coeff = spec ? (dot3(nd, nh) / psamp) / kPRR : div_const<1>(div_const<0>(dot3(nd, nh)));
          }
          cont = true;
        }
      }
    }
    if (kInphM) {
      const bool ends = active && !wantc;
      const uint64_t ask = __ballot(ends);
      const uint32_t fn = gnp * (uint32_t)a.spp;
      float ecf = 0.f, erf = 0.f;
      if (ask && fj < fn) {
        const uint32_t rank =
            __builtin_amdgcn_mbcnt_hi((uint32_t)(ask >> 32), __builtin_amdgcn_mbcnt_lo((uint32_t)ask, 0u));
        if (ends && fj + rank < fn) {
          const uint32_t j = fj + rank;
          const uint32_t s = (gnp & (gnp - 1u)) == 0u ? j >> __builtin_ctz(gnp) : j / gnp;
          const uint32_t q = j - s * gnp;
          rng_init(st, entry_sample(a, q, s, ecf, erf));
          nitem = ((gslots >> (4 * q)) & 15u) | (s << 4);
          if (kInphP) set_item(witem() | (uint64_t)((nitem | 0x1000u) << 16));
          refill = true;
        }
        fj += (uint32_t)__popcll(ask);
        fj = fj < fn ? fj : fn;
      }
      if (wantc || refill) {
        const float ua = uniform(st);
        const float ub = uniform(st);
        const TriMat &m = mat[refill ? 0 : tri];
        const bool spec = SPEC && !refill && (m.flags & MAT_SPECULAR);
        float psamp = kInvPiF;
        V3 h;
        if (refill) {
          h = camera_local(ua, ub, ecf, erf, a.W, a.H, a.rc_W, a.rc_H);
        } else {
          const float phi = (float)(2.0 * kPi * (double)ua);
          float cth, sth;
          if (!spec) {
            cth = sqrt_core(ub);
            const float omu = 1.0f - ub;
            sth = omu > 0.f ? sqrt_core(omu) : 0.f;
          } else {
            const double cd = pow_d((double)ub, 1.0 / ((double)m.shininess + 1.0));
            cth = (float)cd;
            sth = (float)sqrt(1.0 - cd * cd);
            psamp = pow_f((m.shininess + 1.f) * cth, m.shininess);
          }
          float sp, cp;
          sincos_f(phi, sp, cp);
          h = mk(sth * cp, sth * sp, cth);
        }
        const TriGeom &g = geom[refill ? nT : tri];
        V3 v = rotate3(g.R[0], g.R[1], g.R[2], h);
        if (refill) v = camera_w0(a.cam, v);
        nd = unit(v);
        if (wantc) {
          if (SPEC && (m.flags & MAT_HAS_KS)) speci = phong(m.shininess, nh, din, nd);
          coeff = spec ? (dot3(nd, nh) / psamp) / kPRR : div_const<1>(div_const<0>(dot3(nd, nh)));
          cont = true;
        }
      }
    }

    PHASE(2)
    PHASE_LANES(12, vertex)
    V3 lo = mk(0.f, 0.f, 0.f);
    float emit_s = 0.f;
    int emit_et = 0;
    float ts = 0.f;
    int hs = -1;
    const int et = shadow ? emit_tri[emitter] : -1;
    if (__ballot(shadow)) {
      PHASE_LANES(14, shadow)
      if (BVH) {
        bool qn = false;
        if (shadow && bvh_prepass<true>(bv, p, sd, ts, hs, et,
                                        a.big_pomask ? a.big_pomask[tri * nE + emitter] : 0xffffffffu, emitter))
          qn = coop_root_test(cv, p, sd, ts) && !(IPT_TREE_SKIP && tree_skip(a.src_cull, tri, sd));
        SUBPHASE_BEGIN
        coop_cast<true>(cv, qn, p, sd, ts, hs);
        SUBPHASE_END(9)
      } else if (shadow) {
        if (IPT_SHADOW_CULL && e3)
          hs = shadow_hit_pairs_small((const lds_f32 *)(IPT_SHADOW_PAIR1 ? lds_pr : lds_is), pairs, a.pboxes, e3, nT, p, sd, et, ts,
                                      [&]() { return po ? ((const lds_u32c *)lds_po)[tri * nE + emitter] : 0xffffffffu; });
        else
          hs = cast_bf(pairs, e3, nT, p, sd, ts);
      }
      PHASE(3)
      if (shadow && hs == et) {
        const V3 ne = shading_normal(geom[et], along(p, sd, ts));
        const float ctp = -dot3(ne, sd);
        if (!(ctp < 0.f)) {
          const double td = (double)ts;
          const TriMat &me = mat[et];
          if (MODE == MODE_GRAPH) {
            const double q = (double)((weight * ct) * ctp) / (td * td), pr = a.emit_pmfr[emitter];
            double w2d;
            if (pr != 0.0)
              w2d = q * pr;
            else
              w2d = q / (double)emit_pmf[emitter];
            const float w2 = (float)w2d;
            const float wf = w2 * kInvPiF;
            const double v[8] = {(double)w2, (double)wf, (double)(wf * pix.x), (double)(wf * pix.y),
                                 (double)(wf * pix.z), (double)(wf * me.ke[0]), (double)(wf * me.ke[1]),
                                 (double)(wf * me.ke[2])};
            const size_t bin = (size_t)tri * nT + et;
            if (a.lds_edges) {
              bins_add(true, edges, bin * kEdgeL, 5, v);
              bins_add(true, edges, (size_t)(nT + 1) * nT * kEdgeL + ((size_t)tri * nE + emitter) * 3, 3, v + 5);
            } else {
              bins_add(false, edges, bin * kEdgeW, 8, v);
            }
          } else {
            const double q = (double)(ct * ctp) / (td * td), pr = a.emit_pmfr[emitter];
            double s64;
            if (pr != 0.0)
              s64 = q * pr;
            else
              s64 = q / (double)emit_pmf[emitter];
            const float s = (float)s64;
            const V3 kee = ke3(et);
            lo = mk(kee.x * s, kee.y * s, kee.z * s);
            emit_s = s;
            emit_et = et;
            const TriMat &m = mat[tri];
            if (SPEC && (m.flags & MAT_HAS_KS)) specd = phong(m.shininess, nh, din, sd);
            const V3 kt = kd3(tri);
            if (SPEC)
              Ld = mk((kt.x + m.ks[0] * specd) * lo.x, (kt.y + m.ks[1] * specd) * lo.y,
                      (kt.z + m.ks[2] * specd) * lo.z);
            else
              Ld = mk(kt.x * lo.x, kt.y * lo.y, kt.z * lo.z);
          }
        }
      }
    }

    PHASE(4)
    PHASE_LANES(16, shadow && hs == et)
    if (MODE == MODE_ADJU) {
      const int gs = rslot - a.rec_lds;
      const int sh = 6 * (gs / kPoolSlots);
      const bool needc = vertex && gs >= 0 && (gs % kPoolSlots) == 0 && ((ctab >> sh) & 63u) == 63u;
      uint64_t want = __ballot(needc);
      if (want) {
        int got = -1;
        do {
          const int l = (int)__builtin_ctzll(want);
          want &= want - 1;
          const int c = pfree ? (int)__builtin_ctzll(pfree) : -1;
          pfree &= pfree - 1ull;
          if (lane == l) got = c;
        } while (want);
        if (needc) {
          if (got >= 0) {
            ctab = (ctab & ~(63u << sh)) | ((uint32_t)got << sh);
          } else {
            ctab = (ctab & 0x00ffffffu) | ((uint32_t)rslot << 24);
            rslot = 0;
          }
        }
      }
    }
    PHASE_LANES(18, vertex)
    if (vertex) {
      if (is_badj<MODE>()) {
        float *rec = lds_rec + (size_t)k * kBlock + tid;
        const size_t fs = (size_t)vmax * kBlock;
        rec[0] = __uint_as_float((uint32_t)tri | ((uint32_t)emit_et << 16));
        rec[fs] = emit_s;
        rec[2 * fs] = coeff;
        if (SPEC) {
          rec[kRecSD * fs] = specd;
          rec[(kRecSD + 1) * fs] = speci;
        }
      }
      if (MODE == MODE_ADJU) {
        constexpr int NF = SPEC ? kRecFieldsSpec : kRecFieldsDiffuse;
        float v[NF];
        v[0] = __uint_as_float((uint32_t)tri | ((uint32_t)emit_et << 16));
        v[1] = emit_s;
        v[2] = coeff;
        if (SPEC) {
          v[kRecSD] = specd;
          v[kRecSD + 1] = speci;
        }
        const int nl = a.rec_lds;
        if (rslot < nl) {
          float *rec = lds_rec + (size_t)rslot * kBlock + tid;
          const size_t fs = (size_t)nl * kBlock;
#pragma unroll
          for (int f = 0; f < NF; ++f) rec[f * fs] = v[f];
        } else {
          const int gs = rslot - nl;
          const uint32_t c = (ctab >> (6 * (gs / kPoolSlots))) & 63u;
          gbl_f32 *rec = upool + ((size_t)c * kPoolSlots + (size_t)(gs % kPoolSlots)) * NF;
#pragma unroll
          for (int f = 0; f < NF; ++f) rec[f] = v[f];
        }
        if (kSub > 0) {
          if (rslot % kSub == 0 && k > 0) {
            gbl_f32 *m = umr + (size_t)(rslot / kSub) * 192;
            m[0] = M.x;
            m[1] = M.y;
            m[2] = M.z;
          }
        } else if (rslot == 0) {
          if (kCarryLds) carry_put3(3, M);
          else Mlo = M;
        }
        rslot = (rslot + 1 == vcap_of()) ? 0 : rslot + 1;
      }
      if (MODE == MODE_GRAPH) {
        if (cont) {
          weight *= dot3(nd, nh);
          weight = (float)((double)weight * (((1.0 / (double)kInvPiF) / (double)kPRR) / 1.0));
          dst = tri;
        }
      } else {
        const V3 Le = le();
        L = mk(fmaf(M.x, Le.x + Ld.x, L.x), fmaf(M.y, Le.y + Ld.y, L.y), fmaf(M.z, Le.z + Ld.z, L.z));
        if (cont) {
          const V3 tp = kdpi3(tri);
          const float t0 = tp.x, t1 = tp.y, t2 = tp.z;
          if (SPEC) {
            const TriMat &m = mat[tri];
            M = mk((M.x * (t0 + m.ks[0] * speci)) * coeff, (M.y * (t1 + m.ks[1] * speci)) * coeff,
                   (M.z * (t2 + m.ks[2] * speci)) * coeff);
          } else {
            M = mk((M.x * t0) * coeff, (M.y * t1) * coeff, (M.z * t2) * coeff);
          }
        }
      }
      ++k;
      if (BVH) set_ptri(tri);
      if (cont) d = nd;
      else finished = true;
      if (MODE == MODE_ADJU && rhi > 0 && k == rhi) finished = true;
    }

    int uhi = 0, ulo = 0, urep = 0;
    bool uend = false, uesc = false;
    const bool upend = pending();
    if (upend) {
      uhi = usub;
      ulo = rhi == 0 ? k - (rslot == 0 ? vcap_of() : rslot) : rhi - vcap_of();
      if (ulo > 0) urep = ulo;
    }
    if (finished) {
      active = false;
      if (MODE == MODE_FWDM) {
        const uint64_t wi = witem();
        lds_f32 *o = fused_slots(a) + (uint32_t)(wi & 15u) * 3u * (uint32_t)a.spp +
                     (kInphP ? ((uint32_t)wi >> 4) & 0xffu : (uint32_t)(wi >> 4));
        o[0] = L.x;
        o[a.spp] = L.y;
        o[2 * a.spp] = L.z;
      } else if (MODE == MODE_FWD) {
        float *o = out_samples + witem() * 3;
        o[0] = L.x;
        o[1] = L.y;
        o[2] = L.z;
      } else if (MODE == MODE_ADJU) {
        if (rhi == 0) {
          uhi = k;
          ulo = k > 0 ? k - (rslot == 0 ? vcap_of() : rslot) : 0;
          uend = true;
          uesc = escaped;
        } else {
          uhi = rhi;
          ulo = rhi - vcap_of();
        }
        if (ulo > 0) urep = ulo;
      }
// ... 344 lines not shown
```

Before: 12160 Msamples/s.

## Stage per-triangle and emitter shading data in LDS tables for small scenes

Adds a shading-table kernel variant that copies the per-triangle shading fields (normals, flags, rotation, emission) and the per-emitter data (vertices, normals, emission, pmf, cdf) into LDS. The brute-force forward and bounded adjoint kernels then read these from LDS instead of global memory, and emitter selection becomes a vectorised CDF scan. The table is used only when it fits and does not reduce occupancy. The adjoint wide-mode check is also relaxed to ignore the table bytes. The cost is extra LDS per block, a fill at kernel start, and another kernel instance.

```diff
diff --git a/include/ipt.h b/include/ipt.h
--- a/include/ipt.h
+++ b/include/ipt.h
@@ -33,6 +33,7 @@
 int ipt_device_count(void);
 int ipt_selftest_math(uint64_t n, uint64_t seed, uint64_t *counts);
 void ipt_debug_fail_launches(int n);
+int ipt_debug_shade_launches(void);
 void ipt_debug_adju_ring(int pool_chunks, int lds_slots);
 
 void ipt_legacy_config(int width, int height, int spp, int max_bounces, int64_t seed);
diff --git a/inverse_path_tracer_amd/_native.py b/inverse_path_tracer_amd/_native.py
--- a/inverse_path_tracer_amd/_native.py
+++ b/inverse_path_tracer_amd/_native.py
@@ -63,6 +63,7 @@
     "ipt_device_count": (C.c_int, []),
     "ipt_selftest_math": (C.c_int, [C.c_uint64, C.c_uint64, C.POINTER(C.c_uint64)]),
     "ipt_debug_fail_launches": (None, [C.c_int]),
+    "ipt_debug_shade_launches": (C.c_int, []),
     "ipt_debug_adju_ring": (None, [C.c_int, C.c_int]),
     "ipt_legacy_config": (None, [C.c_int, C.c_int, C.c_int, C.c_int, C.c_int64]),
     "ipt_load_scene": (C.c_int, [C.c_int, fp, fp, fp, C.POINTER(C.c_char_p), C.POINTER(C.c_char_p), C.POINTER(vp)]),
diff --git a/inverse_path_tracer_amd/csrc/capi.cpp b/inverse_path_tracer_amd/csrc/capi.cpp
--- a/inverse_path_tracer_amd/csrc/capi.cpp
+++ b/inverse_path_tracer_amd/csrc/capi.cpp
@@ -98,6 +98,7 @@
   return gpu_status(ipt::gpu_selftest_math(n, seed, counts));
 }
 void ipt_debug_fail_launches(int n) { ipt::gpu_debug_fail_launches(n); }
+int ipt_debug_shade_launches(void) { return ipt::gpu_debug_shade_launches(); }
 void ipt_debug_adju_ring(int pool_chunks, int lds_slots) { ipt::gpu_debug_adju_ring(pool_chunks, lds_slots); }
 
 void ipt_legacy_config(int width, int height, int spp, int max_bounces, int64_t seed) {
diff --git a/inverse_path_tracer_amd/csrc/gpu_api.h b/inverse_path_tracer_amd/csrc/gpu_api.h
--- a/inverse_path_tracer_amd/csrc/gpu_api.h
+++ b/inverse_path_tracer_amd/csrc/gpu_api.h
@@ -84,6 +84,7 @@
 
 int gpu_device_count();
 int gpu_selftest_math(uint64_t n, uint64_t seed, uint64_t *counts);
+int gpu_debug_shade_launches();
 void gpu_debug_fail_launches(int n);
 void gpu_debug_adju_ring(int pool_chunks, int lds_slots);
 const char *gpu_last_error();
diff --git a/inverse_path_tracer_amd/csrc/ipt_device.h b/inverse_path_tracer_amd/csrc/ipt_device.h
--- a/inverse_path_tracer_amd/csrc/ipt_device.h
+++ b/inverse_path_tracer_amd/csrc/ipt_device.h
@@ -1100,6 +1100,27 @@
   return unit(n);
 }
 
+__device__ __forceinline__ uint32_t shade_flags_word(const uint32_t *gw, const uint32_t *mw) {
+  return gw[offsetof(TriGeom, flags) / 4] | (mw ? mw[offsetof(TriMat, flags) / 4] << 8 : 0u);
+}
+__device__ __forceinline__ uint32_t tri_shade_word(const uint32_t *gw, const uint32_t *mw, int f) {
+  if (f < TS_FLAGS) return gw[offsetof(TriGeom, vn) / 4 + f - TS_VN];
+  if (f == TS_FLAGS) return shade_flags_word(gw, mw);
+  if (f < TS_KE) return gw[offsetof(TriGeom, R) / 4 + f - TS_R];
+  return mw ? mw[offsetof(TriMat, ke) / 4 + f - TS_KE] : 0u;
+}
+__device__ __forceinline__ uint32_t emit_shade_word(const uint32_t *gw, const uint32_t *mw, int tri, float pmf, double pmfr,
+                                                    int f) {
+  if (f == ES_TRI) return (uint32_t)tri;
+  if (f < ES_VN) return gw[offsetof(TriGeom, v) / 4 + f - ES_V];
+  if (f < ES_FLAGS) return gw[offsetof(TriGeom, vn) / 4 + f - ES_VN];
+  if (f == ES_FLAGS) return shade_flags_word(gw, mw);
+  if (f < ES_PMF) return mw[offsetof(TriMat, ke) / 4 + f - ES_KE];
+  if (f == ES_PMF) return __float_as_uint(pmf);
+  const uint64_t b = (uint64_t)__double_as_longlong(pmfr);
+  return f == ES_PMFR ? (uint32_t)b : (uint32_t)(b >> 32);
+}
+
 __device__ __forceinline__ V3 camera_local(float u0, float u1, float cf, float rf, int W, int H, float rcW, float rcH) {
   const float nx = 2.f * (cf + u0), ny = 2.f * (rf + u1);
   const float x = (rcW != 0.f ? nx * rcW : div_inrange(nx, (float)W)) - 1.f;
diff --git a/inverse_path_tracer_amd/csrc/ipt_hip.hip b/inverse_path_tracer_amd/csrc/ipt_hip.hip
--- a/inverse_path_tracer_amd/csrc/ipt_hip.hip
+++ b/inverse_path_tracer_amd/csrc/ipt_hip.hip
@@ -22,6 +22,8 @@
 const char *gpu_last_error() { return g_gpu_err.c_str(); }
 static std::atomic<int> g_fail_launches{0};
 void gpu_debug_fail_launches(int n) { g_fail_launches.store(n > 0 ? n : 0); }
+static std::atomic<int> g_shade_launches{0};
+int gpu_debug_shade_launches() { return g_shade_launches.load(); }
 static std::atomic<int> g_adju_pool{0}, g_adju_lds{0};
 void gpu_debug_adju_ring(int pool_chunks, int lds_slots) {
   g_adju_pool.store(pool_chunks > 0 ? std::min(pool_chunks, 63) : 0);
@@ -295,6 +297,10 @@
 constexpr bool kInphase() {
   return IPT_INPHASE_REFILL && MODE == MODE_FWDM && !BVH;
 }
+#ifndef IPT_SHADE_TABLES
+#define IPT_SHADE_TABLES 1
+#endif
+constexpr int kSmallShade = 2;
 constexpr int kEntryWords = 4;
 static inline uint32_t fused_entry_words(uint32_t group, bool bvh) {
   return (IPT_INPHASE_REFILL && !bvh) ? kEntryWords * group : 0u;
@@ -490,6 +496,24 @@
   constexpr bool MATB = false;
   constexpr bool VIEWS = false;
   constexpr bool VSETS = false;
+  constexpr bool SHADE = false;
+  const int *const tri_emit = nullptr;
+#include "trace_body.h"
+}
+
+template <int MODE, bool SPEC, bool BVH>
+__global__ IPT_TRACE_BOUNDS void trace_shade_kernel(
+    const TraceArgs a, const TriIsect *__restrict__ isect, const TriPair *__restrict__ pairs,
+    const TriGeom *__restrict__ geom, const TriMat *__restrict__ mat, const float *__restrict__ kd,
+    const int *__restrict__ emit_tri, const float *__restrict__ emit_cdf, const float *__restrict__ emit_pmf,
+    float *__restrict__ out_samples, const float *__restrict__ adj, double *__restrict__ grad,
+    const uint8_t *__restrict__ target, double *__restrict__ edges) {
+  static_assert(!BVH, "the shading tables serve the brute-force instances");
+  constexpr bool MATG = false;
+  constexpr bool MATB = false;
+  constexpr bool VIEWS = false;
+  constexpr bool VSETS = false;
+  constexpr bool SHADE = true;
   const int *const tri_emit = nullptr;
 #include "trace_body.h"
 }
@@ -506,6 +530,7 @@
   constexpr bool MATB = true;
   constexpr bool VIEWS = false;
   constexpr bool VSETS = false;
+  constexpr bool SHADE = false;
   const int *const tri_emit = nullptr;
 #include "trace_body.h"
 }
@@ -524,6 +549,7 @@
   constexpr bool MATB = false;
   constexpr bool VIEWS = false;
   constexpr bool VSETS = false;
+  constexpr bool SHADE = false;
 #include "trace_body.h"
 }
 
@@ -541,6 +567,7 @@
   constexpr bool MATB = false;
   constexpr bool VIEWS = false;
   constexpr bool VSETS = false;
+  constexpr bool SHADE = false;
 #include "trace_body.h"
 }
 
@@ -556,6 +583,7 @@
   constexpr bool MATB = false;
   constexpr bool VIEWS = true;
   constexpr bool VSETS = false;
+  constexpr bool SHADE = false;
   const int *const tri_emit = nullptr;
 #include "trace_body.h"
 }
@@ -574,6 +602,7 @@
   constexpr bool MATB = false;
   constexpr bool VIEWS = true;
   constexpr bool VSETS = false;
+  constexpr bool SHADE = false;
 #include "trace_body.h"
 }
 
@@ -590,6 +619,7 @@
   constexpr bool MATB = false;
   constexpr bool VIEWS = true;
   constexpr bool VSETS = true;
+  constexpr bool SHADE = false;
   const int *const tri_emit = nullptr;
 #include "trace_body.h"
 }
@@ -609,6 +639,7 @@
   constexpr bool MATB = false;
   constexpr bool VIEWS = true;
   constexpr bool VSETS = true;
+  constexpr bool SHADE = false;
 #include "trace_body.h"
 }
 
@@ -628,6 +659,7 @@
   constexpr bool MATB = false;
   constexpr bool VIEWS = true;
   constexpr bool VSETS = true;
+  constexpr bool SHADE = false;
 #include "trace_body.h"
 }
 
@@ -758,8 +790,9 @@
   return r;
 }
 
-enum { KIND_TRACE = 0, KIND_MATG = 1, KIND_FWDB = 2, KIND_VFWD = 3, KIND_VMAT = 4, KIND_VBFWD = 5, KIND_VBMAT = 6 };
-constexpr int kKindLast = KIND_VBMAT;
+enum { KIND_TRACE = 0, KIND_MATG = 1, KIND_FWDB = 2, KIND_VFWD = 3, KIND_VMAT = 4, KIND_VBFWD = 5, KIND_VBMAT = 6, KIND_SHADE = 7 };
+constexpr int kKindLast = KIND_SHADE;
+constexpr bool shade_mode(int mode) { return mode == MODE_FWD || mode == MODE_FWDM || mode == MODE_ADJ || mode == MODE_ADJW; }
 constexpr bool kind_views(int kind) { return kind == KIND_VFWD || kind == KIND_VMAT; }
 constexpr bool kind_view_sets(int kind) { return kind == KIND_VBFWD || kind == KIND_VBMAT; }
 constexpr bool inst_valid(int mode, int kind) {
@@ -767,6 +800,7 @@
          : kind == KIND_MATG ? mode == MODE_ADJ || mode == MODE_ADJU
          : kind == KIND_VMAT ? mode == MODE_ADJ
          : kind == KIND_VBMAT ? mode == MODE_ADJ || mode == MODE_ADJU
+         : kind == KIND_SHADE ? shade_mode(mode)
                              : mode == MODE_FWD || mode == MODE_FWDM;
 }
 constexpr int inst_slot(int mode, bool spec, bool bvh, int kind) {
@@ -776,6 +810,7 @@
           : kind == KIND_VMAT ? 48
           : kind == KIND_VBFWD ? 52 + (mode == MODE_FWDM ? 4 : 0)
           : kind == KIND_VBMAT ? (mode == MODE_ADJU ? 64 : 60)
+          : kind == KIND_SHADE ? 68 + mode * 4
                               : mode * 4) +
          (spec ? 2 : 0) + (bvh ? 1 : 0);
 }
@@ -1039,7 +1074,10 @@
 #endif
 template <int MODE, bool SPEC, bool BVH, int KIND>
 constexpr auto kernel_of() {
-  if constexpr (KIND == KIND_VBMAT) {
+  if constexpr (KIND == KIND_SHADE) {
+    static_assert(shade_mode(MODE), "the shading tables: forwards and bounded adjoints only");
+    return &trace_shade_kernel<MODE, SPEC, BVH>;
+  } else if constexpr (KIND == KIND_VBMAT) {
     static_assert(MODE == MODE_ADJ || MODE == MODE_ADJU, "the view sets' adjoint is the material adjoint, MODE_ADJ or MODE_ADJU");
     if constexpr (MODE == MODE_ADJU) return &trace_matu_views_batch_kernel<SPEC, BVH>;
     else return &trace_mat_views_batch_kernel<SPEC, BVH>;
@@ -1064,7 +1102,8 @@
   }
 }
 constexpr const char *kernel_name(int mode, int kind) {
-  return kind == KIND_VBFWD  ? "trace_fwd_views_batch_kernel"
+  return kind == KIND_SHADE  ? "trace_shade_kernel"
+         : kind == KIND_VBFWD ? "trace_fwd_views_batch_kernel"
          : kind == KIND_VBMAT ? (mode == MODE_ADJU ? "trace_matu_views_batch_kernel" : "trace_mat_views_batch_kernel")
          : kind == KIND_VFWD ? "trace_fwd_views_kernel"
          : kind == KIND_VMAT ? "trace_mat_views_kernel"
@@ -1179,11 +1218,24 @@
   return head + (size_t)(kBlock / 64) * 8 * a.coop_stride * sizeof(uint32_t) + (lane_words ? kLaneWsBytes : 0);
 }
 
+static size_t shade_bytes(const TraceArgs &a) {
+  return (a.small_pairs & kSmallShade) ? (size_t)shade_table_words(a.nT, a.nE) * sizeof(uint32_t) : 0;
+}
+static void shade_offer(const GpuScene *s, TraceArgs &a) {
+  if (IPT_SHADE_TABLES && (a.small_pairs & 1) && !use_bvh(s) && shade_tables_fit(s->host.nT, s->host.nE))
+    a.small_pairs |= kSmallShade;
+}
+static bool shade_keeps_residency(const TraceArgs &a, size_t lds, size_t extra, size_t cap) {
+  const size_t sh = shade_bytes(a), cu = 160 * 1024;
+  return std::min(cap, cu / (lds + extra)) >= std::min(cap, cu / (lds + extra - sh));
+}
+
 static size_t table_bytes(const TraceArgs &a) {
   return (a.kd_tables ? (size_t)6 * a.nT * sizeof(float) : 0) +
          (a.small_pairs ? (size_t)kE3Floats * ((a.nT + 1) / 2) * sizeof(float) + 12 + (size_t)a.nT * kIsectLdsFloats * sizeof(float) +
                               (IPT_PATH_CULL ? (size_t)((a.nT + 1) / 2) * sizeof(TriPair) : 0) +
-                              (IPT_SHADOW_PO && a.pomask ? (size_t)a.nT * a.nE * sizeof(uint32_t) : 0)
+                              (IPT_SHADOW_PO && a.pomask ? (size_t)a.nT * a.nE * sizeof(uint32_t) : 0) +
+                              shade_bytes(a)
                         : 0);
 }
 
@@ -1405,6 +1457,19 @@
     HIP_TRY(hipGetLastError());
     a.kdpi_g = (const float *)kdpi.p;
   }
+  if (a.small_pairs & kSmallShade) {
+    bool take = KIND == KIND_SHADE;
+    if constexpr (KIND == KIND_TRACE && shade_mode(MODE))
+      take = !use_bvh(s) && shade_keeps_residency(a, lds, io.tail ? io.tail + 15 : 0, MODE == MODE_ADJW ? 6 : 5);
+    if (!take) {
+      lds -= shade_bytes(a);
+      a.small_pairs &= ~kSmallShade;
+    }
+    if constexpr (KIND == KIND_TRACE && shade_mode(MODE)) {
+      if (take) return launch<MODE, KIND_SHADE>(s, a, lds, io);
+    }
+    if (KIND == KIND_SHADE && a.n_samples > 0) g_shade_launches.fetch_add(1);
+  }
   auto run = [&](auto spec, auto bvh) {
     constexpr bool SPEC = decltype(spec)::value, BVH = decltype(bvh)::value;
     if constexpr (BVH) {
@@ -1419,13 +1484,15 @@
   constexpr std::true_type yes;
   constexpr std::false_type no;
   if constexpr (MODE == MODE_ADJW) return run(no, no);
+  else if constexpr (KIND == KIND_SHADE) return s->has_ks ? run(yes, no) : run(no, no);
   else if (use_bvh(s)) return s->has_ks ? run(yes, yes) : run(no, yes);
   else return s->has_ks ? run(yes, no) : run(no, no);
 }
 
 int gpu_render_samples(GpuScene *s, const RenderParams &p, const float *kd_dev, float *samples_dev, void *stream) {
   if (check_params(s, p)) return -1;
-  const TraceArgs a = make_args(s, p);
+  TraceArgs a = make_args(s, p);
+  shade_offer(s, a);
   LaunchIO io;
   io.kd = kd_dev, io.out = samples_dev, io.stream = (hipStream_t)stream;
   return launch<MODE_FWD>(s, a, table_bytes(a), io);
@@ -1447,6 +1514,7 @@
   if (check_params(s, p)) return -1;
   TraceArgs a = make_args(s, p);
   a.sample_major = 1;
+  if (KIND == KIND_TRACE) shade_offer(s, a);
   LaunchIO io;
   io.kd = kd_dev, io.out = samples_dev, io.mat = mat_dev, io.views = views_dev, io.nviews = nviews;
   io.stream = (hipStream_t)stream;
@@ -1519,6 +1587,7 @@
   const FusedShape fs = fused_shape(p, use_bvh(s));
   if (fs.group > 0) {
     TraceArgs a = make_args(s, p);
+    if (KIND == KIND_TRACE) shade_offer(s, a);
     a.fused = 1;
     a.group = (uint32_t)fs.group;
     a.chunk = (uint32_t)(fs.group * fs.per_grab);
@@ -2033,6 +2102,12 @@
   TraceArgs a = adjoint_args(s, p);
   const size_t fields = (size_t)(s->has_ks ? kRecFieldsSpec : kRecFieldsDiffuse);
   const size_t per = fields * kBlock * sizeof(float);
+  if (!unbounded) {
+    shade_offer(s, a);
+    if ((size_t)a.grad_slots * 3 * sizeof(double) + table_bytes(a) + (size_t)kBlock * sizeof(uint32_t) + (size_t)a.rec_cap * per >
+        160 * 1024)
+      a.small_pairs &= ~kSmallShade;
+  }
   const size_t base = (size_t)a.grad_slots * 3 * sizeof(double) + table_bytes(a) +
                       (size_t)kBlock * sizeof(uint32_t);
   if (unbounded) {
@@ -2052,6 +2127,9 @@
   bool wide = !use_bvh(s) && !s->has_ks && 6 * (lds + lane_words) <= 160 * 1024 &&
               (uint64_t)a.n_samples * (uint64_t)std::max(1, a.nscenes) >= IPT_ADJW_MIN_SAMPLES;
   if (const char *e = std::getenv("IPT_ADJW")) wide = std::atoi(e) != 0 && !use_bvh(s) && !s->has_ks;
+  if (!wide && !std::getenv("IPT_ADJW") && !use_bvh(s) && !s->has_ks && 6 * (lds - shade_bytes(a) + lane_words) <= 160 * 1024 &&
+      (uint64_t)a.n_samples * (uint64_t)std::max(1, a.nscenes) >= IPT_ADJW_MIN_SAMPLES)
+    wide = true;
   if (wide) return launch<MODE_ADJW>(s, a, lds + lane_words, io);
   return launch<MODE_ADJ>(s, a, lds, io);
 }
diff --git a/inverse_path_tracer_amd/csrc/scene_layout.h b/inverse_path_tracer_amd/csrc/scene_layout.h
--- a/inverse_path_tracer_amd/csrc/scene_layout.h
+++ b/inverse_path_tracer_amd/csrc/scene_layout.h
@@ -55,6 +55,17 @@
 };
 static_assert(sizeof(TriMat) == 32, "TriMat layout");
 
+constexpr int kTriShadeWords = 16, kTriShadeStride = 17;
+constexpr int kEmitShadeWords = 20, kEmitShadeStride = 21;
+constexpr int kShadeMaxTris = 32, kShadeMaxEmit = 16;
+enum : int { TS_VN = 0, TS_FLAGS = 3, TS_R = 4, TS_KE = 13 };
+enum : int { ES_TRI = 0, ES_V = 1, ES_VN = 10, ES_FLAGS = 13, ES_KE = 14, ES_PMF = 17, ES_PMFR = 18 };
+constexpr int kShadeCdfWords = kShadeMaxEmit;
+constexpr bool shade_tables_fit(int nT, int nE) { return nT <= kShadeMaxTris && nE > 0 && nE <= kShadeMaxEmit; }
+constexpr int shade_table_words(int nT, int nE) {
+  return (kShadeCdfWords + (nT + 1) * kTriShadeStride + nE * kEmitShadeStride + 3) & ~3;
+}
+
 struct BvhNode {
   float q[4][4];
 };
diff --git a/inverse_path_tracer_amd/csrc/trace_body.h b/inverse_path_tracer_amd/csrc/trace_body.h
--- a/inverse_path_tracer_amd/csrc/trace_body.h
+++ b/inverse_path_tracer_amd/csrc/trace_body.h
@@ -21,7 +21,10 @@
   constexpr int nthr = kBlock;
   const int nT = a.nT, nE = a.nE;
   const int vmax = a.rec_cap;
+  constexpr bool kEtEarly = !(MODE == MODE_ADJW || (MODE == MODE_FWD && SPEC));
+  float *lds_sh = reinterpret_cast<float *>(lds);
   double *lds_acc = lds;
+  if (SHADE) lds_acc += shade_table_words(nT, nE) / 2;
   int n_acc = 0;
   if (is_adj<MODE>()) {
     n_acc = a.grad_slots * 3;
@@ -29,7 +32,7 @@
   } else if (MODE == MODE_GRAPH && a.lds_edges) {
     n_acc = (int)graph_lds_doubles(nT, nE);
   }
-  float *tab = reinterpret_cast<float *>(lds + n_acc);
+  float *tab = reinterpret_cast<float *>((SHADE ? lds_acc : lds) + n_acc);
   if (a.kd_tables) {
     for (int i = tid; i < 3 * nT; i += nthr) {
       const float v = kd[i];
@@ -42,10 +45,6 @@
   auto kd3 = [&](int t) -> V3 {
     if (a.kd_tables) return mk(tab_l[3 * t], tab_l[3 * t + 1], tab_l[3 * t + 2]);
     return mk(kd_g[3 * t], kd_g[3 * t + 1], kd_g[3 * t + 2]);
-  };
-  auto ke3 = [&](int t) -> V3 {
-    const gbl_f32 *q = (const gbl_f32 *)mat + (size_t)t * (sizeof(TriMat) / sizeof(float)) + offsetof(TriMat, ke) / sizeof(float);
-    return mk(q[0], q[1], q[2]);
   };
   auto kdpi3 = [&](int t) -> V3 {
     if (a.kd_tables) return mk(tab_l[3 * nT + 3 * t], tab_l[3 * nT + 3 * t + 1], tab_l[3 * nT + 3 * t + 2]);
@@ -74,7 +73,34 @@
   const bool po = a.small_pairs && IPT_SHADOW_PO && a.pomask;
   if (po)
     for (int i = tid; i < nT * nE; i += nthr) lds_po[i] = a.pomask[i];
+  if (SHADE) {
+    uint32_t *w = reinterpret_cast<uint32_t *>(lds_sh);
+    const uint32_t *gw = reinterpret_cast<const uint32_t *>(geom), *mw = reinterpret_cast<const uint32_t *>(mat);
+    constexpr int GW = sizeof(TriGeom) / 4, MW = sizeof(TriMat) / 4;
+    for (int i = tid; i < kShadeCdfWords; i += nthr) w[i] = i < nE ? __float_as_uint(emit_cdf[i]) : 0x7fc00000u;
+    w += kShadeCdfWords;
+    for (int i = tid; i < (nT + 1) * kTriShadeWords; i += nthr) {
+      const int t = i / kTriShadeWords, f = i % kTriShadeWords;
+      w[t * kTriShadeStride + f] = tri_shade_word(gw + (size_t)t * GW, t < nT ? mw + (size_t)t * MW : nullptr, f);
+    }
+    w += (nT + 1) * kTriShadeStride;
+    for (int i = tid; i < nE * kEmitShadeWords; i += nthr) {
+      const int e = i / kEmitShadeWords, f = i % kEmitShadeWords, t = emit_tri[e];
+      w[e * kEmitShadeStride + f] = emit_shade_word(gw + (size_t)t * GW, mw + (size_t)t * MW, t, emit_pmf[e], a.emit_pmfr[e], f);
+    }
+  }
+  const lds_f32 *cdf_l = (const lds_f32 *)lds_sh;
+  const lds_f32 *tsh = cdf_l + kShadeCdfWords;
+  const lds_f32 *esh = tsh + (nT + 1) * kTriShadeStride;
   float *lds_rec = a.small_pairs ? reinterpret_cast<float *>(lds_po) + (po ? nT * nE : 0) : lds_e3;
+  auto ke3 = [&](int t) -> V3 {
+    if (SHADE) {
+      const lds_f32 *r = tsh + t * kTriShadeStride + TS_KE;
+      return mk(r[0], r[1], r[2]);
+    }
+    const gbl_f32 *q = (const gbl_f32 *)mat + (size_t)t * (sizeof(TriMat) / sizeof(float)) + offsetof(TriMat, ke) / sizeof(float);
+    return mk(q[0], q[1], q[2]);
+  };
   constexpr bool kCarryLds = MATG && MODE == MODE_ADJU && !BVH;
   lds_u32 *carry_ws = nullptr;
   if (kCarryLds) {
@@ -521,7 +547,7 @@
     bool shadow = false, cont = false;
     bool wantc = false, refill = false;
     uint32_t nitem = 0;
-    int emitter = 0;
+    int emitter = 0, et_sh = 0;
     float ct = 0.f, coeff = 0.f, speci = 0.f, specd = 0.f;
     if (vertex) {
       const V3 q = along(p, d, t);
@@ -539,23 +565,61 @@
           else tri0_r = tri;
         }
       }
-      nh = shading_normal(geom[tri], q);
+      if (SHADE) {
+        const lds_f32 *r = tsh + tri * kTriShadeStride;
+        const bool flat = (__float_as_uint(r[TS_FLAGS]) & GEOM_AXIS_FLAT) != 0u;
+        nh = mk(r[TS_VN], r[TS_VN + 1], r[TS_VN + 2]);
+        if (__ballot(!flat)) {
+          if (!flat) nh = shading_normal(geom[tri], q);
+        }
+      } else {
+        nh = shading_normal(geom[tri], q);
+      }
       p = q;
       Ld = mk(0.f, 0.f, 0.f);
       if (nE > 0) {
         const float u = uniform(st);
         int ie = 0;
-        while (ie < nE && !(emit_cdf[ie] >= u)) ++ie;
-        ie = ie < nE ? ie : nE - 1;
+        if (SHADE) {
+          ie = nE - 1;
+          bool found = false;
+          for (int i = 0; i < nE; i += 4) {
+            const v4f c = *(const lds_v4 *)(cdf_l + i);
+            const bool h0 = !found && c.x >= u;
+            ie = h0 ? i : ie;
+            found = found || h0;
+            const bool h1 = !found && c.y >= u;
+            ie = h1 ? i + 1 : ie;
+            found = found || h1;
+            const bool h2 = !found && c.z >= u;
+            ie = h2 ? i + 2 : ie;
+            found = found || h2;
+            const bool h3 = !found && c.w >= u;
+            ie = h3 ? i + 3 : ie;
+            found = found || h3;
+          }
+        } else {
+          while (ie < nE && !(emit_cdf[ie] >= u)) ++ie;
+          ie = ie < nE ? ie : nE - 1;
+        }
         const float r1 = uniform(st), r2 = uniform(st);
         const double sq = dsqrt_core((double)r1);
         const float ca = (float)(1.0 - sq);
         const float cb = (float)(sq * (double)(1.f - r2));
         const float cc = (float)((double)r2 * sq);
-        const TriGeom &ge = geom[emit_tri[ie]];
-        const V3 pt = mk(fmaf(cc, ge.v[2][0], fmaf(cb, ge.v[1][0], ca * ge.v[0][0])),
-                         fmaf(cc, ge.v[2][1], fmaf(cb, ge.v[1][1], ca * ge.v[0][1])),
-                         fmaf(cc, ge.v[2][2], fmaf(cb, ge.v[1][2], ca * ge.v[0][2])));
+        V3 pt;
+        if (SHADE) {
+          const lds_f32 *er = esh + ie * kEmitShadeStride;
+          if (kEtEarly) et_sh = (int)__float_as_uint(er[ES_TRI]);
+          const lds_f32 *ev = er + ES_V;
+          pt = mk(fmaf(cc, ev[6], fmaf(cb, ev[3], ca * ev[0])), fmaf(cc, ev[7], fmaf(cb, ev[4], ca * ev[1])),
+                  fmaf(cc, ev[8], fmaf(cb, ev[5], ca * ev[2])));
+        } else {
+          const TriGeom &ge = geom[emit_tri[ie]];
+          pt = mk(fmaf(cc, ge.v[2][0], fmaf(cb, ge.v[1][0], ca * ge.v[0][0])),
+                  fmaf(cc, ge.v[2][1], fmaf(cb, ge.v[1][1], ca * ge.v[0][1])),
+                  fmaf(cc, ge.v[2][2], fmaf(cb, ge.v[1][2], ca * ge.v[0][2])));
+        }
         sd = unit(sub(pt, q));
         ct = dot3(nh, sd);
         emitter = ie;
@@ -567,7 +631,8 @@
           wantc = pr < kPRR;
         } else if (pr < kPRR) {
           const TriMat &m = mat[tri];
-          const bool spec = SPEC && (MODE != MODE_GRAPH) && (m.flags & MAT_SPECULAR);
+          const uint32_t sflags = SPEC && SHADE ? __float_as_uint(tsh[tri * kTriShadeStride + TS_FLAGS]) >> 8 : 0u;
+          const bool spec = SPEC && (MODE != MODE_GRAPH) && ((SHADE ? sflags : m.flags) & MAT_SPECULAR);
           const float uphi = uniform(st);
           const float phi = (float)(2.0 * kPi * (double)uphi);
           const float ut = uniform(st);
@@ -586,12 +651,18 @@
           float sp, cp;
           sincos_f(phi, sp, cp);
           const V3 h = mk(sth * cp, sth * sp, cth);
-          const TriGeom &g = geom[tri];
-          nd = unit(mk(fmaf(g.R[0][2], h.z, fmaf(g.R[0][1], h.y, g.R[0][0] * h.x)),
-                       fmaf(g.R[1][2], h.z, fmaf(g.R[1][1], h.y, g.R[1][0] * h.x)),
-                       fmaf(g.R[2][2], h.z, fmaf(g.R[2][1], h.y, g.R[2][0] * h.x))));
+          if (SHADE) {
+            const lds_f32 *R = tsh + tri * kTriShadeStride + TS_R;
+            nd = unit(mk(fmaf(R[2], h.z, fmaf(R[1], h.y, R[0] * h.x)), fmaf(R[5], h.z, fmaf(R[4], h.y, R[3] * h.x)),
+                         fmaf(R[8], h.z, fmaf(R[7], h.y, R[6] * h.x))));
+          } else {
+            const TriGeom &g = geom[tri];
+            nd = unit(mk(fmaf(g.R[0][2], h.z, fmaf(g.R[0][1], h.y, g.R[0][0] * h.x)),
+                         fmaf(g.R[1][2], h.z, fmaf(g.R[1][1], h.y, g.R[1][0] * h.x)),
+                         fmaf(g.R[2][2], h.z, fmaf(g.R[2][1], h.y, g.R[2][0] * h.x))));
+          }
           if (MODE != MODE_GRAPH) {
-            if (SPEC && (m.flags & MAT_HAS_KS)) speci = phong(m.shininess, nh, din, nd);
+            if (SPEC && ((SHADE ? sflags : m.flags) & MAT_HAS_KS)) speci = phong(m.shininess, nh, din, nd);
             coeff = spec ? (dot3(nd, nh) / psamp) / kPRR : div_const<1>(div_const<0>(dot3(nd, nh)));
           }
           cont = true;
@@ -622,7 +693,8 @@
         const float ua = uniform(st);
         const float ub = uniform(st);
         const TriMat &m = mat[refill ? 0 : tri];
-        const bool spec = SPEC && !refill && (m.flags & MAT_SPECULAR);
+        const uint32_t sflags = SPEC && SHADE ? __float_as_uint(tsh[(refill ? 0 : tri) * kTriShadeStride + TS_FLAGS]) >> 8 : 0u;
+        const bool spec = SPEC && !refill && ((SHADE ? sflags : m.flags) & MAT_SPECULAR);
         float psamp = kInvPiF;
         V3 h;
         if (refill) {
@@ -644,12 +716,19 @@
           sincos_f(phi, sp, cp);
           h = mk(sth * cp, sth * sp, cth);
         }
-        const TriGeom &g = geom[refill ? nT : tri];
-        V3 v = rotate3(g.R[0], g.R[1], g.R[2], h);
+        V3 v;
+        if (SHADE) {
+          const lds_f32 *R = tsh + (refill ? nT : tri) * kTriShadeStride + TS_R;
+          v = mk(fmaf(R[2], h.z, fmaf(R[1], h.y, R[0] * h.x)), fmaf(R[5], h.z, fmaf(R[4], h.y, R[3] * h.x)),
+                 fmaf(R[8], h.z, fmaf(R[7], h.y, R[6] * h.x)));
+        } else {
+          const TriGeom &g = geom[refill ? nT : tri];
+          v = rotate3(g.R[0], g.R[1], g.R[2], h);
+        }
         if (refill) v = camera_w0(a.cam, v);
         nd = unit(v);
         if (wantc) {
-          if (SPEC && (m.flags & MAT_HAS_KS)) speci = phong(m.shininess, nh, din, nd);
+          if (SPEC && ((SHADE ? sflags : m.flags) & MAT_HAS_KS)) speci = phong(m.shininess, nh, din, nd);
           coeff = spec ? (dot3(nd, nh) / psamp) / kPRR : div_const<1>(div_const<0>(dot3(nd, nh)));
           cont = true;
         }
@@ -663,7 +742,10 @@
     int emit_et = 0;
     float ts = 0.f;
     int hs = -1;
-    const int et = shadow ? emit_tri[emitter] : -1;
+    const int et = !shadow ? -1
+                   : !SHADE   ? emit_tri[emitter]
+                   : kEtEarly ? et_sh
+                              : (int)__float_as_uint(esh[emitter * kEmitShadeStride + ES_TRI]);
     if (__ballot(shadow)) {
       PHASE_LANES(14, shadow)
       if (BVH) {
@@ -683,18 +765,37 @@
       }
       PHASE(3)
       if (shadow && hs == et) {
-        const V3 ne = shading_normal(geom[et], along(p, sd, ts));
+        V3 ne;
+        if (SHADE) {
+          const lds_f32 *er = esh + emitter * kEmitShadeStride;
+          const bool flat = (__float_as_uint(er[ES_FLAGS]) & GEOM_AXIS_FLAT) != 0u;
+          ne = mk(er[ES_VN], er[ES_VN + 1], er[ES_VN + 2]);
+          if (__ballot(!flat)) {
+            if (!flat) ne = shading_normal(geom[et], along(p, sd, ts));
+          }
+        } else {
+          ne = shading_normal(geom[et], along(p, sd, ts));
+        }
         const float ctp = -dot3(ne, sd);
         if (!(ctp < 0.f)) {
           const double td = (double)ts;
-          const TriMat &me = mat[et];
+          V3 kee_s = mk(0.f, 0.f, 0.f);
+          double pr_s = 0.0;
+          float pmf_s = 0.f;
+          if (SHADE) {
+            const lds_f32 *er = esh + emitter * kEmitShadeStride;
+            kee_s = mk(er[ES_KE], er[ES_KE + 1], er[ES_KE + 2]);
+            pmf_s = er[ES_PMF];
+            pr_s = __hiloint2double((int)__float_as_uint(er[ES_PMFR + 1]), (int)__float_as_uint(er[ES_PMFR]));
+          }
           if (MODE == MODE_GRAPH) {
-            const double q = (double)((weight * ct) * ctp) / (td * td), pr = a.emit_pmfr[emitter];
+            const TriMat &me = mat[et];
+            const double q = (double)((weight * ct) * ctp) / (td * td), pr = SHADE ? pr_s : a.emit_pmfr[emitter];
             double w2d;
             if (pr != 0.0)
               w2d = q * pr;
             else
-              w2d = q / (double)emit_pmf[emitter];
+              w2d = q / (double)(SHADE ? pmf_s : emit_pmf[emitter]);
             const float w2 = (float)w2d;
             const float wf = w2 * kInvPiF;
             const double v[8] = {(double)w2, (double)wf, (double)(wf * pix.x), (double)(wf * pix.y),
@@ -708,14 +809,14 @@
               bins_add(false, edges, bin * kEdgeW, 8, v);
             }
           } else {
-            const double q = (double)(ct * ctp) / (td * td), pr = a.emit_pmfr[emitter];
+            const double q = (double)(ct * ctp) / (td * td), pr = SHADE ? pr_s : a.emit_pmfr[emitter];
             double s64;
             if (pr != 0.0)
               s64 = q * pr;
             else
-              s64 = q / (double)emit_pmf[emitter];
+              s64 = q / (double)(SHADE ? pmf_s : emit_pmf[emitter]);
             const float s = (float)s64;
-            const V3 kee = ke3(et);
+            const V3 kee = SHADE ? kee_s : ke3(et);
             lo = mk(kee.x * s, kee.y * s, kee.z * s);
             emit_s = s;
             emit_et = et;
```

Measured after the change: 12680 Msamples/s (median of 6 runs). 4.3% higher.
